# refresh-bio/LZ-ANI

Measured on AMD Instinct MI355X. Metric: genome-pairs/sec + achieved HBM GB/s, 10k×40kbp all2all at 1/2/4/8 GPUs, higher is better.
Workload: dtype u32 (2-bit packed symbols, 64-bit lane masks; f64 only in the anchor/seed arbitration)

## Files before the change

### lz-ani_amd/csrc/lzani_core.h

```cpp
#pragma once
#include <stdint.h>
#include <type_traits>

#if defined(__HIPCC__)
#include <hip/hip_runtime.h>
#define LZ_HD __host__ __device__ __forceinline__
#else
#define LZ_HD inline
#endif

#if defined(__HIP_DEVICE_COMPILE__)
extern __device__ int g_guard_trip;
#define LZ_GUARD_TRIP(code) (g_guard_trip = (code))
#else
#define LZ_GUARD_TRIP(code) ((void)(code))
#endif

namespace lzani {

typedef uint64_t u64;
typedef uint32_t u32;

struct Params {
    int mal, msl, mrd, mqd, reg, aw, am, ar;
};

struct TextView {
    const u64* t2;
    const u64* nm;
    int len;
    int L, rc0;
    bool nfree;
};

enum { NO_RC = 0x40000000 };
LZ_HD TextView ref_view(const u64* t2, const u64* nm, int L, int mrd, bool nfree)
{ return TextView{t2, nm, 2 * L + 3 * mrd, L, L + 2 * mrd, nfree}; }
LZ_HD TextView qry_view(const u64* t2, const u64* nm, int L, int mrd, bool nfree)
{ return TextView{t2, nm, L + mrd, L, NO_RC, nfree}; }

LZ_HD bool pos_valid(const TextView& t, int p)
{
    const u32 a = (u32)p, b = (u32)(p - t.rc0);
    return (a < b ? a : b) < (u32)t.L;
}
LZ_HD int run_end(const TextView& t, int p)
{
    if (p < t.L) return (t.rc0 == t.L) ? t.rc0 + t.L : t.L;
    return (p >= t.rc0 && p < t.rc0 + t.L) ? t.rc0 + t.L : p;
}

struct IndexView {
    const u32* dirz;
    const u32* ent;
    int kb;
    int dirbits;
    int posbits;
    u32 tagmask;
    const u32* bk;
    const u32* tw;
};
enum : u32 { BK_EMPTY = 0xFFFFFFFFu, BK_OVERFLOW = 0xFFFFFFFEu, TW_OVERFLOW = 0x808080FFu };
enum { IDX_SORT_MAX = 32 };

LZ_HD u64 lowmask(int n) { return n >= 64 ? ~0ULL : (n <= 0 ? 0ULL : ((1ULL << n) - 1ULL)); }

LZ_HD int popc64(u64 x)
{
#if defined(__HIP_DEVICE_COMPILE__)
    return __popcll(x);
#else
    return __builtin_popcountll(x);
#endif
}
LZ_HD int ctz64(u64 x)
{
#if defined(__HIP_DEVICE_COMPILE__)
    return __ffsll((unsigned long long)x) - 1;
#else
    return __builtin_ctzll(x);
#endif
}
LZ_HD int clz64(u64 x)
{
#if defined(__HIP_DEVICE_COMPILE__)
    return __clzll((long long)x);
#else
    return __builtin_clzll(x);
#endif
}
LZ_HD u64 brev64(u64 x)
{
#if defined(__HIP_DEVICE_COMPILE__)
    return __brevll(x);
#else
    u64 r = 0;
    for (int k = 0; k < 64; ++k) r |= ((x >> k) & 1ULL) << (63 - k);
    return r;
#endif
}
LZ_HD int imin(int a, int b) { return a < b ? a : b; }
LZ_HD int imax(int a, int b) { return a > b ? a : b; }
LZ_HD int iabs(int a) { return a < 0 ? -a : a; }

LZ_HD u64 win2(const u64* t2, int p)
{
    const u32 w = (u32)p >> 5;
    const int s = (p & 31) * 2;
    u64 lo = t2[w];
    if (s == 0) return lo;
    return (lo >> s) | (t2[w + 1] << (64 - s));
}
LZ_HD u64 winN(const u64* nm, int p)
{
    const u32 w = (u32)p >> 6;
    const int s = p & 63;
    u64 lo = nm[w];
    if (s == 0) return lo;
    return (lo >> s) | (nm[w + 1] << (64 - s));
}
typedef u32 __attribute__((may_alias)) u32a;
LZ_HD int sym_at(const TextView& t, int p)
{
    return (int)((reinterpret_cast<const u32a*>(t.t2)[(u32)p >> 4] >> ((p & 15) * 2)) & 3u);
}
LZ_HD int isN_at(const TextView& t, int p) { return (int)((t.nm[(u32)p >> 6] >> (p & 63)) & 1ULL); }

LZ_HD int sym_match(const TextView& R, int rp, const TextView& Q, int qp)
{
    if (R.nfree && Q.nfree) {
        const bool vr = pos_valid(R, rp), vq = pos_valid(Q, qp);
        const int a = sym_at(R, vr ? rp : 0), b = sym_at(Q, vq ? qp : 0);
        return (int)(vr & vq & (a == b));
    }
    if (rp < 0 || rp >= R.len || qp < 0 || qp >= Q.len) return 0;
    if (isN_at(R, rp) | isN_at(Q, qp)) return 0;
    return sym_at(R, rp) == sym_at(Q, qp);
}

LZ_HD int equal_len(const TextView& R, int rp, const TextView& Q, int qp, int start)
{
    if (R.nfree && Q.nfree) {
        int bound = imin(run_end(R, rp) - rp, run_end(Q, qp) - qp);
        int n = start;
        while (n < bound) {
            u64 x = win2(R.t2, rp + n) ^ win2(Q.t2, qp + n);
            u64 d = (x | (x >> 1)) & 0x5555555555555555ULL;
            if (d) { n += ctz64(d) >> 1; break; }
            n += 32;
        }
        n = imin(n, bound);
        return n > start ? n : start;
    }
    int bound = imin(R.len - rp, Q.len - qp);
    int n = start;
    int guard = 0;
    while (n < bound) {
        if (++guard > (1 << 26)) { LZ_GUARD_TRIP(1); break; }
        u64 x = win2(R.t2, rp + n) ^ win2(Q.t2, qp + n);
        u64 d = (x | (x >> 1)) & 0x5555555555555555ULL;
        u32 nn = (u32)(winN(R.nm, rp + n) | winN(Q.nm, qp + n));
        int fd = d ? (ctz64(d) >> 1) : 32;
        int fn = nn ? ctz64((u64)nn) : 32;
        int f = imin(fd, fn);
        if (f < 32) { n += f; return n < bound ? n : (bound > start ? bound : start); }
        n += 32;
    }
    return n < bound ? n : (bound > start ? bound : start);
}

LZ_HD bool kmer_at(const TextView& t, int p, int k, u64& key)
{
    if (p < 0 || p + k > t.len) return false;
    if (winN(t.nm, p) & lowmask(k)) return false;
    key = win2(t.t2, p) & lowmask(2 * k);
    if (k >= 32 && (key & 2)) return false;
    return true;
}

LZ_HD u64 mix_key(u64 key, int kb)
{
    if (kb <= 32) {
        u32 m = kb >= 32 ? 0xFFFFFFFFu : ((1u << kb) - 1u);
        u32 x = (u32)key;
        x = (x * 0x9E3779B1u) & m;
        x ^= x >> ((kb + 1) >> 1);
        x = (x * 0x85EBCA6Bu) & m;
        x ^= x >> ((kb + 1) >> 1);
        x = (x * 0xC2B2AE35u) & m;
        return x;
    }
    u64 m = lowmask(kb);
    u64 x = key;
    x = (x * 0x9E3779B97F4A7C15ULL) & m;
    x ^= x >> ((kb + 1) >> 1);
    x = (x * 0xD6E8FEB86659FD93ULL) & m;
    x ^= x >> ((kb + 1) >> 1);
    x = (x * 0xC2B2AE3D27D4EB4FULL) & m;
    return x;
}
LZ_HD u32 kml_from_syms(u32 syms, int mal)
{
    return (u32)mix_key((u64)(syms & (u32)lowmask(2 * mal)), 2 * mal);
}
LZ_HD bool kmer_valid_n(const TextView& t, int p, int k, u64 nwin)
{
    return p >= 0 && p + k <= t.len && !(nwin & lowmask(k));
}
LZ_HD bool kmer_valid_nfree_head(int L, int mrd, int p, int k)
{
    return p + k <= (mrd == 0 ? 2 * L : L);
}
LZ_HD void key_slot(const IndexView& I, u64 key, u32& bucket, u32& tag)
{
    u64 h = mix_key(key, I.kb);
    int tb = I.kb - I.dirbits;
    bucket = (u32)(h >> tb);
    tag = (u32)(h & lowmask(tb)) & I.tagmask;
}

LZ_HD void anchor_lookup(const Params& P, const TextView& R, const TextView& Q, const IndexView& I,
                         u64 h, int qp, int& ap, int& al)
{
    ap = 0; al = 0;
    int tb = I.kb - I.dirbits;
    u32 b = (u32)(h >> tb);
    u32 tag = (u32)(h & lowmask(tb)) & I.tagmask;
    u32 s = I.dirz[b], e = I.dirz[b + 1];
    u32 pm = (u32)lowmask(I.posbits);
    if (e - s > (u32)R.len || e < s) { LZ_GUARD_TRIP(2); return; }
    for (u32 j = s; j < e; ++j) {
        u32 en = I.ent[j];
        if ((en >> I.posbits) != tag) continue;
        int p = (int)(en & pm);
        int m = equal_len(R, p, Q, qp, 0);
        if (m >= P.mal && (m > al || (m == al && p < ap))) { al = m; ap = p; }
    }
}

LZ_HD void best_anchor(const Params& P, const TextView& R, const TextView& Q, const IndexView& I,
                       int qp, int& ap, int& al)
{
    ap = 0; al = 0;
    u64 key;
    if (!kmer_at(Q, qp, P.mal, key)) return;
    anchor_lookup(P, R, Q, I, mix_key(key, I.kb), qp, ap, al);
}

LZ_HD void seed_consider(int p, int m, int ref_pred, int& sp, int& sl)
{
    if (m >= sl) {
        if (m == sl) { if (iabs(p - ref_pred) < iabs(sp - ref_pred)) sp = p; }
        else { sl = m; sp = p; }
    }
}

LZ_HD double pow_not_chance(int len, u32 e)
{
    if (len >= 27) return 1.0;
    double base = 1.0 - __builtin_ldexp(1.0, -2 * len);
    double r = 1.0;
    while (e) {
        if (e & 1u) r *= base;
        base *= base;
        e >>= 1;
    }
    return r;
}

LZ_HD void arbitrate(const Params& P, int T, int lit, int ap, int al, int& sp, int& sl)
{
    if (!ap) return;
    if (!sp) { sp = ap; sl = al; return; }
    if (sp == ap && sl == al) return;
    u32 ea = (u32)(int)(2 * ((u64)T + 1 - (u64)(int64_t)al));
    u32 ec = (u32)(lit + P.mrd + 1 - sl);
    double anchor_prob = pow_not_chance(al, ea);
    double close_prob = pow_not_chance(sl, ec);
    if (anchor_prob > close_prob) { sp = ap; sl = al; }
}

LZ_HD void seed_search_window(const Params& P, const TextView& R, const TextView& Q,
                              int qp, int r_end, int lit, int& sp, int& sl)
{
    sp = 0; sl = 0;
    u64 qk;
    if (!kmer_at(Q, qp, P.msl, qk)) return;
    int ref_pred = r_end + lit;
    int hi = imin(ref_pred + P.mrd, R.len - P.msl + 1);
    const int step = 33 - P.msl;
    const u64 km = lowmask(2 * P.msl), nk = lowmask(P.msl);
    for (int p0 = r_end; p0 < hi; p0 += step) {
        u64 w2 = win2(R.t2, p0), wn = winN(R.nm, p0);
        int cnt = imin(step, hi - p0);
        for (int o = 0; o < cnt; ++o) {
            if (((w2 >> (2 * o)) & km) != qk || ((wn >> o) & nk)) continue;
            seed_consider(p0 + o, equal_len(R, p0 + o, Q, qp, P.msl), ref_pred, sp, sl);
        }
    }
}

LZ_HD void eval_step(const Params& P, const TextView& R, const TextView& Q, const IndexView& I,
                     int qp, bool trk, int r_end, int lit, int& bp, int& bl)
{
    int ap, al;
    best_anchor(P, R, Q, I, qp, ap, al);
    if (!trk) { bp = ap; bl = al; return; }
    int sp, sl;
    seed_search_window(P, R, Q, qp, r_end, lit, sp, sl);
    arbitrate(P, R.len, lit, ap, al, sp, sl);
    bp = sp; bl = sl;
}

struct Regions {
    int cl, clit, nl;
    int tm, tl, tc;
    int reg;
    LZ_HD void init(int r) { cl = clit = nl = tm = tl = tc = 0; reg = r; }
    LZ_HD void finalize()
    {
        if (cl && cl + clit >= reg) { tm += cl; tl += clit; ++tc; }
        cl = clit = nl = 0;
    }
    LZ_HD void discard() { cl = clit = nl = 0; }
    LZ_HD void seg(u64 M, int n)
    {
        if (M) {
            int hi = 63 - clz64(M);
            int c = popc64(M);
            cl += c;
            clit += nl + (hi + 1 - c);
            nl = n - 1 - hi;
        } else nl += n;
    }
    LZ_HD void seg_match_run(int n) { if (n > 0) { cl += n; clit += nl; nl = 0; } }
};

struct RegionCoords {
    int ref_start, ref_end, seq_start, seq_end, nm, nmm, buf;
    bool fresh;
    LZ_HD void clear() { ref_start = ref_end = seq_start = seq_end = -1; nm = nmm = buf = 0; fresh = true; }
    LZ_HD int length() const { return seq_end - seq_start; }
    LZ_HD void touch(int dp, int off, int len)
    {
        if (seq_start < 0 || dp < seq_start) seq_start = dp;
        if (seq_end < 0 || dp + len > seq_end) seq_end = dp + len;
        if (ref_start < 0 || off < ref_start) ref_start = off;
        if (ref_end < 0 || off + len > ref_end) ref_end = off + len;
    }
    LZ_HD void match(int dp, int off, int len)
    {
        if (fresh) { clear(); fresh = false; }
        else { ref_end += buf; seq_end += buf; nmm += buf; }
        buf = 0;
        touch(dp, off, len);
        nm += len;
    }
    LZ_HD void lit(int len) { buf += len; }
};

struct ExtMasks { u64 brk, qual; };

LZ_HD void ext_lane(u64 prevB, u64 B, int j, int n, int aw, int am, int ar, bool& brk, bool& qual)
{
    u64 W = (B << (63 - j)) | ((prevB >> 1) >> j);
    int a = ar < 1 ? 1 : ar;
    bool in = j < n;
    brk = in && popc64(W >> (64 - aw)) > am;
    qual = in && (W >> (64 - a)) == 0;
}

LZ_HD u64 compress_even(u64 x)
{
    x &= 0x5555555555555555ULL;
    x = (x | (x >> 1)) & 0x3333333333333333ULL;
    x = (x | (x >> 2)) & 0x0F0F0F0F0F0F0F0FULL;
    x = (x | (x >> 4)) & 0x00FF00FF00FF00FFULL;
    x = (x | (x >> 8)) & 0x0000FFFF0000FFFFULL;
    x = (x | (x >> 16)) & 0x00000000FFFFFFFFULL;
    return x;
}
LZ_HD u64 bits_below(int n) { return lowmask(n < 0 ? 0 : n); }
LZ_HD u64 bits_range(int a, int b) { return bits_below(b) & ~bits_below(a); }
LZ_HD u64 valid_bits(const TextView& t, int p0)
{
    u64 v = bits_range(-p0, t.L - p0);
    if (t.rc0 != NO_RC) v |= bits_range(t.rc0 - p0, t.rc0 + t.L - p0);
    return v;
}
LZ_HD u64 win2f(const u64* t2, int p)
{
    const u32 w = (u32)p >> 5;
    const int s = (p & 31) * 2;
    return (t2[w] >> s) | ((t2[w + 1] << 1) << (63 - s));
}
LZ_HD u64 winNf(const u64* nm, int p)
{
    const u32 w = (u32)p >> 6;
    const int s = p & 63;
    return (nm[w] >> s) | ((nm[w + 1] << 1) << (63 - s));
}
LZ_HD u32 lane_mism32(const TextView& R, const TextView& Q, int q0, int r0)
{
    const u64 x = win2f(R.t2, r0) ^ win2f(Q.t2, q0);
    const u32 mm = (u32)compress_even(x | (x >> 1));
    u32 valid;
    if (R.nfree && Q.nfree) valid = (u32)(valid_bits(R, r0) & valid_bits(Q, q0));
    else valid = (u32)(~(winNf(R.nm, r0) | winNf(Q.nm, q0)) & bits_below(R.len - r0) & bits_below(Q.len - q0));
    return mm | ~valid;
}
LZ_HD u32 win16f(const u64* t2, int p)
{
    const u32* t32 = reinterpret_cast<const u32*>(t2);
    const u32 w = (u32)p >> 4;
    const u32 s = ((u32)p & 15u) * 2u;
    const u32 d0 = t32[w], d1 = t32[w + 1];
#if defined(__HIP_DEVICE_COMPILE__)
    return __builtin_amdgcn_alignbit(d1, d0, s);
#else
    return (u32)((((u64)d1 << 32) | d0) >> s);
#endif
}
LZ_HD u32 compress_even16(u32 x)
{
    x &= 0x55555555u;
    x = (x | (x >> 1)) & 0x33333333u;
    x = (x | (x >> 2)) & 0x0F0F0F0Fu;
    x = (x | (x >> 4)) & 0x00FF00FFu;
    x = (x | (x >> 8)) & 0x0000FFFFu;
    return x;
}
LZ_HD int clamp16(int n) { return imax(0, imin(n, 16)); }
LZ_HD u32 bits_range16(int a, int b)
{
    const int l = clamp16(a), h = imax(clamp16(b), l);
    return (1u << h) - (1u << l);
}
LZ_HD u32 valid_bits16(const TextView& t, int p0)
{
    u32 v = bits_range16(-p0, t.L - p0);
    if (t.rc0 != NO_RC) v |= bits_range16(t.rc0 - p0, t.rc0 + t.L - p0);
    return v;
}
LZ_HD u32 lane_mism16(const TextView& R, const TextView& Q, int q0, int r0)
{
    const u32 x = win16f(R.t2, r0) ^ win16f(Q.t2, q0);
    const u32 mm = compress_even16(x | (x >> 1));
    u32 valid;
    if (R.nfree && Q.nfree) valid = valid_bits16(R, r0) & valid_bits16(Q, q0);
    else valid = (u32)(~(winNf(R.nm, r0) | winNf(Q.nm, q0)) & bits_below(R.len - r0) & bits_below(Q.len - q0)) & 0xFFFFu;
    return mm | ~valid;
}
LZ_HD u32 brev32(u32 x)
{
#if defined(__HIP_DEVICE_COMPILE__)
    return __brev(x);
#else
    u32 r = 0;
    for (int k = 0; k < 32; ++k) r |= ((x >> k) & 1u) << (31 - k);
    return r;
#endif
}
LZ_HD int popc32(u32 x) { return popc64((u64)x); }

enum : u32 { EXT_REC_NONE = 0x3FFFFFFFu, EXT_REC_FWDK = 0x20000000u, EXT_REC_BRKB = 0x40000000u, EXT_REC_NULLF = 0x80000000u };
LZ_HD u32 ext_rec_none(int aw) { return aw <= 15 ? 0x00007FFFu : (u32)EXT_REC_NONE; }
LZ_HD u32 ext_qual32(u32 B, int ar)
{
    const int a = ar < 1 ? 1 : ar;
    const u32 Z = ~B;
    u32 acc = Z;
    for (int k = 1; k < a && k < 32; ++k) acc &= (Z << k) | (u32)lowmask(k);
    return acc;
}
LZ_HD u32 ext_record_bwd(const Params& P, u32 Bb)
{
    const u32 wm = (u32)lowmask(P.aw);
    const u32 qb = ext_qual32(Bb, P.ar) & wm;
    if (popc32(Bb & wm) <= P.am) return qb;
    if (P.aw > 15) return qb | EXT_REC_BRKB;
    u32 x = Bb & wm;
    for (int k = 0; k < P.am; ++k) x &= x - 1u;
    const u32 q = qb & (u32)lowmask((int)__builtin_ctz(x) + 1);
    const int b = q ? 32 - (int)__builtin_clz(q) : 0;
    return (u32)b | ((u32)(b - popc32(Bb & (u32)lowmask(b))) << 4) | EXT_REC_BRKB;
}
LZ_HD u32 ext_record_fwd(const Params& P, u32 Bf)
{
    const u32 wm = (u32)lowmask(P.aw);
    if (popc32(Bf & wm) <= P.am) return 0u;
    u32 x = Bf & wm;
    for (int k = 0; k < P.am; ++k) x &= x - 1u;
    const u32 qf = ext_qual32(Bf, P.ar) & (u32)lowmask((int)__builtin_ctz(x) + 1);
    if (qf == 0) return EXT_REC_NULLF | (P.aw <= 15 ? (u32)EXT_REC_FWDK : 0u);
    if (P.aw > 15) return 0u;
    const int e = 32 - (int)__builtin_clz(qf);
    return EXT_REC_FWDK | ((u32)e << 24) | ((u32)popc32(Bf & (u32)lowmask(e)) << 20);
}
LZ_HD u32 null_ext_record(const Params& P, const TextView& R, const TextView& Q, int qp, int pos, int al, bool narrow = true)
{
    if (P.aw > 30) return EXT_REC_NONE;
    u32 rec = ext_rec_none(P.aw);
    if (qp >= 32 && pos >= 32)
        rec = ext_record_bwd(P, (narrow && P.aw <= 15) ? (brev32(lane_mism16(R, Q, qp - 16, pos - 16)) >> 16) | 0xFFFF0000u
                                                       : brev32(lane_mism32(R, Q, qp - 32, pos - 32)));
    const int fq = qp + al, fr = pos + al;
    if (imin(Q.len - fq, R.len - fr) >= P.aw)
        rec |= ext_record_fwd(P, (narrow && P.aw <= 15) ? lane_mism16(R, Q, fq, fr) : lane_mism32(R, Q, fq, fr));
    return rec;
}

struct TextWords5 { u32 m, a, b, c, d; };
LZ_HD u32 funnel32(u32 hi, u32 lo, u32 s)
{
// ... 554 lines not shown
```

### lz-ani_amd/csrc/lzani_kernels_index.h

```cpp
#pragma once
#include "lzani_block.h"

namespace lzani {

__global__ void k_kmers(GenomeTab G, u32* __restrict__ kmL, u32* __restrict__ kmS, int mal, int msl, int mrd, int Tmax)
{
    u32 g = blockIdx.y;
    int p = blockIdx.x * blockDim.x + threadIdx.x;
    int T = ref_text_len(G.L[g], mrd);
    if (p >= Tmax || p >= T) return;
    u64 o = G.nmoff[g];
    TextView R = ref_view(G.t2 + 2 * o, G.nm + o, G.L[g], mrd, false);
    u64 key;
    u32 a = KM_INVALID, b = KM_INVALID;
    if (kmer_at(R, p, mal, key)) a = kml_from_syms((u32)key, mal);
    if (kmer_at(R, p, msl, key)) {
        b = (u32)key;
        if (msl == 8 || msl == 9) {
            u32 h = (b * 0x9E3779B1u) >> 18;
            h = h == 0x3FFFu ? 0x3FFEu : h;
            b |= h << (2 * msl);
        }
    }
    kmL[64 * o + p] = a;
    kmS[64 * o + p] = b;
}

__global__ void __launch_bounds__(256) k_join_keys(GenomeTab G, const u64* __restrict__ koff, unsigned long long* __restrict__ keys,
                                                   u32* __restrict__ valid_cnt, int shift_g, int posbits, int Lmax, u32 g_base)
{
    enum { PER_THREAD = 16 };
    __shared__ u32 s_cnt;
    const u32 g = blockIdx.y;
    const int L = G.L[g];
    if (threadIdx.x == 0) s_cnt = 0;
    __syncthreads();
    const u32* km = G.kmL + 64 * G.nmoff[g];
    unsigned long long* out = keys + koff[g];
    u32 mine = 0;
    for (int k = 0; k < PER_THREAD; ++k) {
        const int p = (blockIdx.x * PER_THREAD + k) * 256 + threadIdx.x;
        if (p >= L) break;
        const u32 h = km[p];
        const bool ok = h != KM_INVALID;
        out[p] = ok ? ((unsigned long long)(g_base + g) << shift_g) | ((unsigned long long)h << posbits) | (unsigned long long)p : ~0ULL;
        mine += ok;
    }
    for (int d = 32; d >= 1; d >>= 1) mine += __shfl_xor(mine, d);
    if ((threadIdx.x & 63) == 0 && mine) atomicAdd(&s_cnt, mine);
    __syncthreads();
    if (threadIdx.x == 0 && s_cnt) atomicAdd(&valid_cnt[g], s_cnt);
    (void)Lmax;
}

__global__ void k_pack(const uint8_t* __restrict__ codes, const u64* __restrict__ codeoff,
                       u64* __restrict__ t2, u64* __restrict__ nm, const u64* __restrict__ nmoff,
                       const int* __restrict__ Ls, int* __restrict__ hasN, int mrd, u32 n)
{
    u32 g = blockIdx.y;
    if (g >= n) return;
    int L = Ls[g];
    int T = ref_text_len(L, mrd);
    size_t nblk = text_wordsN(T);
    size_t blk = (size_t)blockIdx.x * blockDim.x + threadIdx.x;
    if (blk >= nblk) return;
    const uint8_t* c = codes + codeoff[g];
    u64 w0 = 0, w1 = 0, nw = 0;
    int rc0 = L + 2 * mrd;
    for (int j = 0; j < 64; ++j) {
        long p = (long)blk * 64 + j;
        int s = 4;
        if (p < L) { int v = c[p]; s = v < 4 ? v : 4; if (v >= 4) hasN[g] = 1; }
        else if (p >= rc0 && p < rc0 + L) { int v = c[L - 1 - (p - rc0)]; s = v < 4 ? 3 - v : 4; }
        if (s < 4) {
            if (j < 32) w0 |= (u64)s << (2 * j);
            else w1 |= (u64)s << (2 * (j - 32));
        } else nw |= 1ULL << j;
    }
    size_t o = nmoff[g] + blk;
    nm[o] = nw;
    t2[2 * o] = w0;
    t2[2 * o + 1] = w1;
}

struct IdxArgs {
    GenomeTab G;
    const u32* ref_ids;
    u32* dirz;
    u32* ent;
    u64 dir_stride, ent_stride;
    int mal, mrd;
    IndexGeom geo;
    const u32* todo;
};

__device__ __forceinline__ bool idx_slot_key(const IdxArgs& a, u32 slot, int p, u32& bucket, u32& entry)
{
    u32 g = a.ref_ids[slot];
    int T = ref_text_len(a.G.L[g], a.mrd);
    if (p + a.mal > T) return false;
    u64 o = a.G.nmoff[g];
    u64 h;
    if (a.G.kmL) {
        u32 v = a.G.kmL[64 * o + p];
        if (v == KM_INVALID) return false;
        h = (u64)v;
    } else {
        TextView R = ref_view(a.G.t2 + 2 * o, a.G.nm + o, a.G.L[g], a.mrd, false);
        u64 key;
        if (!kmer_at(R, p, a.mal, key)) return false;
        h = mix_key(key, a.geo.kb);
    }
    int tb = a.geo.kb - a.geo.dirbits;
    bucket = (u32)(h >> tb);
    u32 tag = (u32)(h & lowmask(tb)) & a.geo.tagmask;
    entry = (tag << a.geo.posbits) | (u32)p;
    return true;
}

__global__ void __launch_bounds__(256) k_idx_keys(IdxArgs a, unsigned long long* __restrict__ keys, u32* __restrict__ cnt,
                                                  int Tmax, int shift_slot)
{
    enum { PER_THREAD = 16 };
    __shared__ u32 s_cnt;
    const u32 slot = blockIdx.y;
    const u32 g = a.ref_ids[slot];
    const int T = ref_text_len(a.G.L[g], a.mrd);
    if (threadIdx.x == 0) s_cnt = 0;
    __syncthreads();
    const u32* km = a.G.kmL + 64 * a.G.nmoff[g];
    unsigned long long* out = keys + (u64)slot * (u64)Tmax;
    u32 mine = 0;
    for (int k = 0; k < PER_THREAD; ++k) {
        const int p = (blockIdx.x * PER_THREAD + k) * 256 + threadIdx.x;
        if (p >= Tmax) break;
        const u32 h = p < T ? km[p] : KM_INVALID;
        const bool ok = h != KM_INVALID;
        out[p] = ok ? ((unsigned long long)h << a.geo.posbits) | (unsigned long long)p : ~0ULL;
        mine += ok;
    }
    (void)shift_slot;
    block_sum(mine, &s_cnt);
    if (threadIdx.x == 0 && s_cnt) atomicAdd(&cnt[slot], s_cnt);
}

__global__ void k_idx_base(const u32* __restrict__ cnt, u64* __restrict__ base, u32 rows, u32 group, u64 Tmax)
{
    for (u32 s = blockIdx.x * blockDim.x + threadIdx.x; s < rows; s += gridDim.x * blockDim.x) {
        const u32 g0 = s / group * group;
        u64 at = (u64)g0 * Tmax;
        for (u32 t = g0; t < s; ++t) at += cnt[t];
        base[s] = at;
    }
}

__global__ void __launch_bounds__(256) k_idx_from_sorted(IdxArgs a, const unsigned long long* __restrict__ sorted,
                                                         const u32* __restrict__ cnt, const u64* __restrict__ base,
                                                         u32* __restrict__ bk, u32* __restrict__ tw, u64 bk_stride, u64 tw_stride)
{
    const u32 slot = blockIdx.y;
    const u32 n = cnt[slot], nb = 1u << a.geo.dirbits;
    const int tb = a.geo.kb - a.geo.dirbits, posbits = a.geo.posbits;
    const u32 hmask = (u32)lowmask(a.geo.kb), pmask = (u32)lowmask(posbits), tagm = (u32)lowmask(tb) & a.geo.tagmask;
    u32* dirz = a.dirz + slot * a.dir_stride;
    u32* ent = a.ent + slot * a.ent_stride;
    uint4* bks = bk ? reinterpret_cast<uint4*>(bk + slot * bk_stride) : nullptr;
    u32* tws = tw ? tw + slot * tw_stride : nullptr;
    const uint4 empty4 = {BK_EMPTY, BK_EMPTY, BK_EMPTY, BK_EMPTY};
    if (n == 0) {
        for (u32 b = blockIdx.x * blockDim.x + threadIdx.x; b <= nb; b += gridDim.x * blockDim.x) {
            dirz[b] = 0;
            if (b < nb) { if (bks) bks[b] = empty4; if (tws) tws[b] = 0; }
        }
        return;
    }
    const unsigned long long* S = sorted + base[slot];
    for (u32 k = blockIdx.x * blockDim.x + threadIdx.x; k < n; k += gridDim.x * blockDim.x) {
        const unsigned long long e = S[k];
        const u32 h = ((u32)(e >> posbits)) & hmask, b = h >> tb;
        const u32 en = ((h & tagm) << posbits) | ((u32)e & pmask);
        ent[k] = en;
        const long long pb = k ? (long long)((((u32)(S[k - 1] >> posbits)) & hmask) >> tb) : -1;
        if ((long long)b != pb) {
            for (long long bb = pb + 1; bb <= (long long)b; ++bb) dirz[bb] = k;
            for (long long bb = pb + 1; bb < (long long)b; ++bb) { if (bks) bks[bb] = empty4; if (tws) tws[bb] = 0; }
            if (bks) {
                u32 o[4] = {en, BK_EMPTY, BK_EMPTY, BK_EMPTY};
                u32 w = 0x80u | (en >> posbits);
                u32 m = 1;
                for (; m < 5 && k + m < n; ++m) {
                    const unsigned long long e2 = S[k + m];
                    const u32 h2 = ((u32)(e2 >> posbits)) & hmask;
                    if ((h2 >> tb) != b) break;
                    if (m < 4) { o[m] = ((h2 & tagm) << posbits) | ((u32)e2 & pmask); w |= (0x80u | (o[m] >> posbits)) << (8 * m); }
                }
                if (m > 4) { o[3] = BK_OVERFLOW; w = TW_OVERFLOW; }
                bks[b] = uint4{o[0], o[1], o[2], o[3]};
                if (tws) tws[b] = w;
            }
        }
        if (k == n - 1) {
            for (long long bb = (long long)b + 1; bb <= (long long)nb; ++bb) dirz[bb] = n;
            for (long long bb = (long long)b + 1; bb < (long long)nb; ++bb) { if (bks) bks[bb] = empty4; if (tws) tws[bb] = 0; }
        }
    }
}

__global__ void k_idx_filter(IdxArgs a, u32* __restrict__ fl, u64 fl_stride, u32 fmask, int Tmax)
{
    const u32 slot = blockIdx.y;
    const u32 g = a.ref_ids[slot];
    const int T = ref_text_len(a.G.L[g], a.mrd);
    const u64 o = a.G.nmoff[g];
    for (int p = blockIdx.x * blockDim.x + threadIdx.x; p + a.mal <= T && p < Tmax; p += gridDim.x * blockDim.x) {
        const u32 v = a.G.kmL[64 * o + p];
        if (v != KM_INVALID) atomicOr(&fl[slot * fl_stride + ((v & fmask) >> 5)], 1u << (v & 31));
    }
}

__global__ void k_idx_count(IdxArgs a, int Tmax)
{
    u32 slot = blockIdx.y;
    if (a.todo && !a.todo[slot]) return;
    for (int p = blockIdx.x * blockDim.x + threadIdx.x; p < Tmax; p += gridDim.x * blockDim.x) {
        u32 b, e;
        if (idx_slot_key(a, slot, p, b, e)) atomicAdd(&a.dirz[slot * a.dir_stride + 1 + b], 1u);
    }
}

__global__ void k_idx_zero(u32* dirz, u64 dir_stride, u32 nb, const u32* todo)
{
    u32 slot = blockIdx.y;
    if (!todo[slot]) return;
    for (u32 b = blockIdx.x * blockDim.x + threadIdx.x; b <= nb; b += gridDim.x * blockDim.x) dirz[slot * dir_stride + b] = 0;
}

__global__ void __launch_bounds__(1024) k_idx_scan(u32* dirz, u64 dir_stride, u32 nb, const u32* todo)
{
    __shared__ u32 wsum[16];
    __shared__ u32 carry_s;
    if (todo && !todo[blockIdx.x]) return;
    u32* cnt = dirz + (u64)blockIdx.x * dir_stride + 1;
    if (threadIdx.x == 0) carry_s = 0;
    __syncthreads();
    for (u32 base = 0; base < nb; base += 1024) {
        const u32 idx = base + threadIdx.x;
        const u32 before = block_scan_step<u32>(idx < nb ? cnt[idx] : 0, wsum, &carry_s);
        if (idx < nb) cnt[idx] = before;
    }
}

__global__ void k_idx_fill(IdxArgs a, int Tmax)
{
    u32 slot = blockIdx.y;
    if (a.todo && !a.todo[slot]) return;
    for (int p = blockIdx.x * blockDim.x + threadIdx.x; p < Tmax; p += gridDim.x * blockDim.x) {
        u32 b, e;
        if (idx_slot_key(a, slot, p, b, e)) {
            u32 at = atomicAdd(&a.dirz[slot * a.dir_stride + 1 + b], 1u);
            a.ent[slot * a.ent_stride + at] = e;
        }
    }
}

#ifndef LZANI_IDX_RANGE
#define LZANI_IDX_RANGE 16384
#define LZANI_IDX_STAGE 24576
#endif
enum { IDX_RANGE = LZANI_IDX_RANGE, IDX_STAGE = LZANI_IDX_STAGE };

__global__ void __launch_bounds__(1024) k_idx_build(IdxArgs a, u32* __restrict__ bk, u32* __restrict__ tw,
                                                    u64 bk_stride, u64 tw_stride, u32* __restrict__ status)
{
    extern __shared__ u32 lds[];
    u32* cnt = lds;
    u32* stage = lds + IDX_RANGE / 2;
    __shared__ u32 wsum[16];
    __shared__ u32 carry_s, ovf_s;
    const u32 slot = blockIdx.x, tid = threadIdx.x;
    const int lane = tid & 63, wv = tid >> 6;
    const u32 g = a.ref_ids[slot];
    const int T = ref_text_len(a.G.L[g], a.mrd);
    const u32* km = a.G.kmL + 64 * a.G.nmoff[g];
    const u32 nb = 1u << a.geo.dirbits;
    const u32 rb = nb < (u32)IDX_RANGE ? nb : (u32)IDX_RANGE, rw = rb >> 1;
    const int tb = a.geo.kb - a.geo.dirbits, posbits = a.geo.posbits;
    const u32 tagm = (u32)lowmask(tb) & a.geo.tagmask;
    u32* dirz = a.dirz + slot * a.dir_stride;
    u32* ent = a.ent + slot * a.ent_stride;
    u32* bks = bk ? bk + slot * bk_stride : nullptr;
    u32* tws = tw ? tw + slot * tw_stride : nullptr;
    enum { U = 8 };
    if (tid == 0) ovf_s = 0;
    u32 base = 0;
    for (u32 r0 = 0; r0 < nb; r0 += rb) {
        for (u32 k = tid; k < rw; k += 1024) cnt[k] = 0;
        if (tid == 0) carry_s = 0;
        __syncthreads();
        for (int p0 = (int)tid; p0 < T; p0 += U * 1024) {
            u32 v[U];
#pragma unroll
            for (int k = 0; k < U; ++k) { const int p = p0 + k * 1024; v[k] = p < T ? km[p] : KM_INVALID; }
#pragma unroll
            for (int k = 0; k < U; ++k) {
                const u32 b = (v[k] >> tb) - r0;
                if (v[k] == KM_INVALID || b >= rb) continue;
                const u32 sh = (b & 1) * 16;
                const u32 old = atomicAdd(&cnt[b >> 1], 1u << sh);
                if (((old >> sh) & 0xFFFFu) == 0xFFFFu) ovf_s = 1;
            }
        }
        __syncthreads();
        for (u32 w0 = 0; w0 < rw; w0 += 1024) {
            const u32 idx = w0 + tid;
            const u32 w = idx < rw ? cnt[idx] : 0;
            const u32 c0 = w & 0xFFFFu, c1 = w >> 16;
            const u32 v = c0 + c1;
            u32 x = v;
            for (int d = 1; d < 64; d <<= 1) {
                u32 y = __shfl_up(x, d);
// ... 114 lines not shown
```

### lz-ani_amd/csrc/lzani_kernels_pairs.h

```cpp
#pragma once

namespace lzani {

enum { SEED_BM_BITS = 14, SEED_BM_WORDS = 1 << (SEED_BM_BITS - 5), NQUEUES = 8 };
enum { AQ_CAP = 64, AQ_MAXCHUNKS = 32, AQ_LANE_CAP = 32, AQ_LDS_CAND = 128,
       SEED_PAD = 96,
       SEED_LDS_WORDS = SEED_BM_WORDS + SEED_PAD };
static_assert(2 * AQ_LDS_CAND <= SEED_BM_WORDS, "the candidate buffers of refill live in the seed bitmap");
enum : u32 { AQ_COMPLEX = 0x80000000u, AQ_LONG = 0x40000000u, AQ_POS = 0x3FFFFFFFu };
enum { AQ_NONE = 0x7FFFFFFF };

__device__ __forceinline__ u64 wballot(bool b) { return __builtin_amdgcn_ballot_w64(b); }
__device__ __forceinline__ u32 rep4(u32 b) { return __builtin_amdgcn_perm(b, b, 0u); }

#if defined(LZANI_RTC)
#define LZ_RTC_PARAMS Params{LZANI_P_MAL, LZANI_P_MSL, LZANI_P_MRD, LZANI_P_MQD, LZANI_P_REG, LZANI_P_AW, LZANI_P_AM, LZANI_P_AR}
#else
#define LZ_RTC_PARAMS Params{11, 7, 40, 40, 35, 15, 7, 3}
#endif
LZ_HD constexpr Params folded_params(int defp)
{
    return defp == 2 ? Params{15, 9, 40, 40, 60, 15, 7, 3} : defp == 9 ? LZ_RTC_PARAMS : Params{11, 7, 40, 40, 35, 15, 7, 3};
}
LZ_HD constexpr bool chain_params_ok(const Params& p)
{
    return p.mal >= 1 && p.mal <= 15 && p.msl >= 1 && p.msl <= 9 && p.mqd >= 0 && p.mqd <= 62 && p.mrd >= 1 &&
           p.mqd + p.mrd >= 64 && p.mqd + p.mrd <= 127 && p.aw >= 2 && p.aw <= 15 && p.ar <= p.aw && p.am >= 0 && p.reg >= 0 && p.reg < (1 << 20);
}
LZ_HD constexpr int chain_of(int defp, bool nfree)
{
    return defp == 1 ? (nfree ? 3 : 1) : defp == 2 ? 2 : defp == 9 ? (chain_params_ok(folded_params(9)) ? (nfree ? 10 : 9) : 0) : 0;
}
template <int CHAIN> struct ChainP {
    static constexpr Params P = folded_params(CHAIN == 2 ? 2 : CHAIN >= 9 ? 9 : 1);
    static constexpr bool NF = CHAIN == 3 || CHAIN == 10;
    enum { MAL = P.mal, MSL = P.msl, MRD = P.mrd, MQD = P.mqd, REG = P.reg, AW = P.aw, AM = P.am > 16 ? 16 : P.am, AR = P.ar < 1 ? 1 : P.ar,
           NT = MQD + 1, WIN = MQD + MRD };
};

#ifndef LZANI_STRETCH_DENSE
#define LZANI_STRETCH_DENSE 0
#endif
template <bool FAST, bool BK = false, bool JOIN = false, int CHAIN = 0, bool LFLT = false, bool SPLITW = false>
struct DevWave {
    static constexpr bool NULL_CHAIN = CHAIN != 0;
    const Params& P;
    TextView R, Q;
    IndexView I;
    int lane;
    u32* bitmap;
    const u32* rkS;
    const u32* qkL;
    const u32* qkS;
    lzani_region* reg_out;
    unsigned long long* reg_count;
    unsigned long long reg_cap, pair_e;
    int iend = 0;
    int scan_pos = 0, q_head = 0, q_cnt = 0;
    int last_src = -1;
    int stop_i = 0x7FFFFFFF;
    __device__ __forceinline__ void split_limit(int at) { stop_i = at; }
    bool split_taint = false;
    __device__ __forceinline__ void split_taint_set(bool t) { split_taint = t; }
    static __device__ __forceinline__ int uniform(int v) { return __builtin_amdgcn_readfirstlane(v); }
    enum { SPLIT_MARGIN = 256 };
    u32 a_ext = EXT_REC_NONE;
    unsigned long long* cand_bits = nullptr;
    int a_pos = AQ_NONE, a_len = 0;
    u32 a_ref = 0;
#ifdef LZANI_CHAIN_STATS
    unsigned st[8] = {0, 0, 0, 0, 0, 0, 0, 0};
    unsigned sw[8] = {0, 0, 0, 0, 0, 0, 0, 0};
    unsigned sr[4] = {0, 0, 0, 0};
    unsigned long long stc[4] = {0, 0, 0, 0}, stc_t0 = 0;
    int stc_open = -2;
#define LZ_CHAIN_SLOTS(X) \
    X(0, "chain_calls") X(1, "commits") X(2, "exit_nothing") X(3, "exit_seed") X(4, "exit_not_plain") X(5, "exit_event") \
    X(6, "events_general") X(7, "refills") \
    X(8, "cycles after exit_nothing") X(9, "cycles after round_done") X(10, "cycles after exit_event") X(11, "cycles inside the chain") \
    X(12, "not null: close") X(13, "not null: region kept or none open") X(14, "not null: no forward record") X(15, "not null: backward side") \
    X(16, "exit_seed: anchor's own step") X(17, "exit_seed: no window position") X(18, "exit_seed: several") X(19, "exit_seed: text end") \
    X(20, "exit_seed: long seed") X(21, "exit_seed: other") X(22, "event known, commit left") X(23, "-")
    template <class Acc> __device__ __forceinline__ void flush_chain_stats(Acc* g, int ln) const
    {
        for (int k = 0; k < 8; ++k) atomicAdd(&g[k], ln == 0 ? (unsigned long long)st[k] : 0ULL);
        for (int k = 0; k < 4; ++k) atomicAdd(&g[8 + k], ln == 0 ? stc[k] : 0ULL);
        for (int k = 0; k < 4; ++k) atomicAdd(&g[12 + k], ln == 0 ? (unsigned long long)sr[k] : 0ULL);
        for (int k = 0; k < 8; ++k) atomicAdd(&g[16 + k], ln == 0 ? (unsigned long long)sw[k] : 0ULL);
    }
    __device__ __forceinline__ void cycles_mark(int code)
    {
        unsigned long long t;
        asm volatile("s_memtime %0\n\ts_waitcnt lgkmcnt(0)" : "=s"(t) :: "memory");
        if (stc_open == 0) stc[0] += t - stc_t0; else if (stc_open == 1) stc[1] += t - stc_t0; else if (stc_open == 2) stc[2] += t - stc_t0; else if (stc_open == 3) stc[3] += t - stc_t0;
        stc_open = code < 0 ? 3 : code;
        stc_t0 = t;
    }
#endif
#ifdef LZANI_PATH_STATS
    unsigned ps[24] = {0};
    unsigned pw[12] = {0};
#define LZ_PATH_SLOTS(X) \
    X(0, "find_event calls") X(1, "fe: seed straight from the chain's round") X(2, "fe: common call, plain candidate") X(3, "fe: light rounds") \
    X(4, "fe: light round hit") X(5, "fe: light round without a hit") X(6, "fe: merge loop hit") X(7, "fe: jump to a plain candidate") \
    X(8, "stretch calls") X(9, "stretch: not applicable") X(10, "stretch: no seed step") X(11, "stretch: anchor before the seed") \
    X(12, "stretch: seed event") X(13, "stretch: ... with the masks") X(14, "stretch: sum of seed steps") \
    X(15, "refills") X(16, "chain: nothing") X(17, "chain: round done") X(18, "chain: event found") X(19, "chain: seed event known") \
    X(20, "events") X(21, "close events") X(22, "extension chunks") X(23, "stretch chain: events committed") \
    X(24, "-") X(25, "text end") X(26, "no seed step") X(27, "several window positions") X(28, "seed bounds") X(29, "match of 64+") \
    X(30, "anchor before the seed") X(31, "tag in two slots / overflow") X(32, "anchor elsewhere") X(33, "extension runs on") \
    X(34, "-") X(35, "-")
    template <class Acc> __device__ __forceinline__ void flush_path_stats(Acc* g, int ln) const
    {
        for (int k = 0; k < 24; ++k) atomicAdd(&g[k], ln == 0 ? (unsigned long long)ps[k] : 0ULL);
        for (int k = 0; k < 12; ++k) atomicAdd(&g[24 + k], ln == 0 ? (unsigned long long)pw[k] : 0ULL);
    }
#define LZ_PS(k) (ps[k] += 1)
#define LZ_PSN(k, n) (ps[k] += (unsigned)(n))
#else
#define LZ_PS(k) ((void)0)
#define LZ_PSN(k, n) ((void)0)
#endif
#ifdef LZANI_PHASE_TIME
    unsigned long long pt_chain = 0, pt_refill = 0;
    static __device__ __forceinline__ unsigned long long pt_now()
    {
        unsigned long long t;
        asm volatile("s_memtime %0\n\ts_waitcnt lgkmcnt(0)" : "=s"(t) :: "memory");
        return t;
    }
#endif
    bool refill_only = false;
    int restart_at = -1;
    bool round_no_seed = false;
    bool pre_round = false;
    u64 pre_seed = 0;
    u32 pre_rk0 = KM_INVALID, pre_rk1 = KM_INVALID, pre_qk = KM_INVALID;
    const u32* flt = nullptr;
    u32 fmask = 31;
    __device__ __forceinline__ void emit_region(const RegionCoords& c) const
    {
        unsigned long long old, saved;
        const unsigned long long one = 1ULL;
        asm volatile("s_mov_b64 %[sv], exec\n\t"
                     "s_mov_b64 exec, 1\n\t"
                     "global_atomic_add_x2 %[old], %[addr], %[one], off sc0\n\t"
                     "s_waitcnt vmcnt(0)\n\t"
                     "s_mov_b64 exec, %[sv]"
                     : [old] "=&v"(old), [sv] "=&s"(saved)
                     : [addr] "v"(reg_count), [one] "v"(one)
                     : "memory");
        const u32 lo = __builtin_amdgcn_readfirstlane((u32)old), hi = __builtin_amdgcn_readfirstlane((u32)(old >> 32));
        const unsigned long long slot = ((unsigned long long)hi << 32) | lo;
        if (slot < reg_cap) {
            lzani_region* o = reg_out + slot;
            o->pair = pair_e;
            o->ref_start = c.ref_start; o->ref_end = c.ref_end; o->seq_start = c.seq_start; o->seq_end = c.seq_end;
            o->num_matches = c.nm; o->num_mismatches = c.nmm;
        }
    }
#ifdef LZANI_STAMPS
    mutable unsigned long long t0;
    mutable unsigned long long acc[8];
    mutable int cur;
    __device__ __forceinline__ void stamp(int k) const
    {
        unsigned long long t;
        asm volatile("s_memtime %0\n\ts_waitcnt lgkmcnt(0)" : "=s"(t) :: "memory");
        acc[cur] += t - t0; cur = k; t0 = t;
    }
#else
    __device__ __forceinline__ void stamp(int) const {}
#endif

    struct SymReq { u32 wr, wq; int sr, sq; bool ok; };
    __device__ __forceinline__ SymReq sym_request(int rp, int qp) const
    {
        const bool vr = pos_valid(R, rp), vq = pos_valid(Q, qp);
        const int a = vr ? rp : 0, b = vq ? qp : 0;
        SymReq x;
        x.wr = reinterpret_cast<const u32a*>(R.t2)[(u32)a >> 4];
        x.wq = reinterpret_cast<const u32a*>(Q.t2)[(u32)b >> 4];
        x.sr = (a & 15) * 2; x.sq = (b & 15) * 2; x.ok = vr & vq;
        return x;
    }
    static __device__ __forceinline__ bool sym_differs(const SymReq& x)
    {
        return !(x.ok & ((((x.wr >> x.sr) ^ (x.wq >> x.sq)) & 3u) == 0));
    }
    __device__ __forceinline__ bool lane_mismatch(int rp, int qp) const
    {
        if (R.nfree && Q.nfree) {
            SymReq x = sym_request(rp, qp);
            asm volatile("" : "+v"(x.wr), "+v"(x.wq));
            return sym_differs(x);
        }
        return !sym_match(R, rp, Q, qp);
    }
    __device__ __forceinline__ u64 mism_fwd(int q0, int r0, int n) const
    {
        return wballot((lane < n) & lane_mismatch(r0 + lane, q0 + lane));
    }
    __device__ __forceinline__ u64 mism_bwd(int q0, int r0, int n) const
    {
        return wballot((lane < n) & lane_mismatch(r0 - 1 - lane, q0 - 1 - lane));
    }
    __device__ __forceinline__ void mism2(int qa, int ra, int da, int na, int qb, int rb, int db, int nb, u64& A, u64& B) const
    {
        const int rpa = ra + da * lane, qpa = qa + da * lane, rpb = rb + db * lane, qpb = qb + db * lane;
        bool ma, mb;
        if (R.nfree && Q.nfree) {
            SymReq x = sym_request(rpa, qpa), y = sym_request(rpb, qpb);
            asm volatile("" : "+v"(x.wr), "+v"(x.wq), "+v"(y.wr), "+v"(y.wq));
            ma = sym_differs(x); mb = sym_differs(y);
        } else {
            ma = !sym_match(R, rpa, Q, qpa);
            mb = !sym_match(R, rpb, Q, qpb);
        }
        A = wballot((lane < na) & ma);
        B = wballot((lane < nb) & mb);
    }
    static constexpr bool HAS_MISM3 = true;
    __device__ __forceinline__ void mism3(int qa, int ra, int na, int qb, int rb, int nb, int qc, int rc, int nc, u64& A, u64& B, u64& C) const
    {
        bool ma, mb, mc;
        if (R.nfree && Q.nfree) {
            SymReq x = sym_request(ra + lane, qa + lane), y = sym_request(rb + lane, qb + lane), z = sym_request(rc + lane, qc + lane);
            asm volatile("" : "+v"(x.wr), "+v"(x.wq), "+v"(y.wr), "+v"(y.wq), "+v"(z.wr), "+v"(z.wq));
            ma = sym_differs(x); mb = sym_differs(y); mc = sym_differs(z);
        } else {
            ma = !sym_match(R, ra + lane, Q, qa + lane);
            mb = !sym_match(R, rb + lane, Q, qb + lane);
            mc = !sym_match(R, rc + lane, Q, qc + lane);
        }
        A = wballot((lane < na) & ma);
        B = wballot((lane < nb) & mb);
        C = wballot((lane < nc) & mc);
    }
    __device__ __forceinline__ u32 bm_hash(u32 k) const
    {
        return P.msl <= 7 ? k : P.msl <= 9 ? k >> (2 * P.msl) : (k * 0x9E3779B1u) >> (32 - SEED_BM_BITS);
    }
    __device__ __forceinline__ bool seed_prefilter(u32 rk0, u32 rk1, u32 qk) const
    {
        const u32 scratch = (u32)lane;
        const u32 b0 = bm_hash(rk0), b1 = bm_hash(rk1), bq = bm_hash(qk);
        const bool v0 = rk0 != KM_INVALID, v1 = rk1 != KM_INVALID, vq = qk != KM_INVALID;
        const u32 w0 = v0 ? b0 >> 5 : scratch, w1 = v1 ? b1 >> 5 : scratch, wq = vq ? bq >> 5 : scratch;
        atomicOr(&bitmap[w0], v0 ? 1u << (b0 & 31) : 0u);
        atomicOr(&bitmap[w1], v1 ? 1u << (b1 & 31) : 0u);
        __builtin_amdgcn_fence(__ATOMIC_ACQ_REL, "wavefront");
        __builtin_amdgcn_wave_barrier();
        const bool hit = vq & ((bitmap[wq] >> (bq & 31)) & 1u);
        __builtin_amdgcn_fence(__ATOMIC_ACQ_REL, "wavefront");
        __builtin_amdgcn_wave_barrier();
        bitmap[w0] = 0;
        bitmap[w1] = 0;
        return hit;
    }
    __device__ __forceinline__ void seed_candidates(u32 qkl, int lim, u32 rk0, u32 rk1, u64& d0, u64& d1) const
    {
        d0 = wballot(rk0 == qkl) & lowmask(lim);
        d1 = wballot(rk1 == qkl) & lowmask(lim - 64);
    }

    __device__ __forceinline__ u64 bcast64(u64 v, int l) const
    {
        const u32 lo = (u32)__builtin_amdgcn_readlane((int)(u32)v, l), hi = (u32)__builtin_amdgcn_readlane((int)(u32)(v >> 32), l);
        return ((u64)hi << 32) | lo;
    }
    __device__ __forceinline__ int wave_equal_len(int rp, int qp, int start) const
    {
        const int bound = imin(R.len - rp, Q.len - qp);
        int n = start;
        while (n < bound) {
            u64 B = mism_fwd(qp + n, rp + n, imin(64, bound - n));
            if (B) { n += ctz64(B); break; }
            n += 64;
        }
        n = imin(n, bound);
        return n > start ? n : start;
    }

    __device__ __forceinline__ bool find_event_generic(int i, int n, bool trk, int r_end, int lit,
                                                       int& ev_lane, int& bpos, int& blen) const
    {
        int bp = 0, bl = 0;
        if (lane < n)
            eval_step(P, R, Q, I, i + lane, trk && (lit + lane <= P.mqd), r_end, lit + lane, bp, bl);
        u64 hit = wballot(lane < n && bl >= P.msl);
        if (!hit) { ev_lane = n; return false; }
        ev_lane = ctz64(hit);
        bpos = __builtin_amdgcn_readlane(bp, ev_lane);
        blen = __builtin_amdgcn_readlane(bl, ev_lane);
        return true;
    }

    __device__ __forceinline__ void walk_bucket(u32 b, u32 tag, int qp, int& ap, int& al) const
    {
        const u32 pm = (u32)lowmask(I.posbits);
        u32 s = I.dirz[b], e = I.dirz[b + 1];
        if (e - s > (u32)R.len || e < s) { LZ_GUARD_TRIP(2); e = s; }
        for (u32 j = s; j < e; ++j) {
            const u32 x = (u32)__builtin_amdgcn_readfirstlane((int)I.ent[j]);
            if ((x >> I.posbits) != tag) continue;
            const int p = (int)(x & pm);
            const int m = wave_equal_len(p, qp, 0);
            if (m >= P.mal && (m > al || (m == al && p < ap))) { al = m; ap = p; }
        }
    }

    __device__ __forceinline__ void anchor_by_wave(u32 hql, int qp, int& ap, int& al) const
    {
        const int tb = I.kb - I.dirbits;
        const u32 pm = (u32)lowmask(I.posbits), tag = hql & I.tagmask;
        typedef u32 u32x4 __attribute__((ext_vector_type(4)));
        u32x4 bq;
        const u64 baddr = (u64)(I.bk + 4 * (u64)(hql >> tb));
        const u64 bsgpr = ((u64)(u32)__builtin_amdgcn_readfirstlane((int)(u32)(baddr >> 32)) << 32) |
                          (u32)__builtin_amdgcn_readfirstlane((int)(u32)baddr);
        asm volatile("s_load_dwordx4 %0, %1, 0x0\n\ts_waitcnt lgkmcnt(0)" : "=s"(bq) : "s"(bsgpr) : "memory");
        const u32 en[4] = {bq.x, bq.y, bq.z, bq.w};
        if (__builtin_expect(en[3] == BK_OVERFLOW, 0)) {
            walk_bucket(hql >> tb, tag, qp, ap, al);
        } else {
#pragma unroll
            for (int k = 0; k < 4; ++k) {
                if ((en[k] >> I.posbits) != tag) continue;
                const int p = (int)(en[k] & pm);
                const int m = wave_equal_len(p, qp, 0);
                if (m >= P.mal && m > al) { al = m; ap = p; }
            }
        }
    }

    __device__ __forceinline__ bool find_event_round(int i, int n, bool trk, int r_end, int lit,
                                                     int& ev_lane, int& bpos, int& blen) const
    {
        n = imin(n, 64);
        ev_lane = n;
        const int nt = trk ? imin(n, P.mqd - lit + 1) : 0;
        const int W = nt > 0 ? imin(lit + nt - 1 + P.mrd, R.len - P.msl + 1 - r_end) : 0;
        const int tb = I.kb - I.dirbits;
        if (__builtin_expect(!FAST || W > 128 || (!BK && I.tagmask != (u32)lowmask(tb)), 0))
            return find_event_generic(i, n, trk, r_end, lit, ev_lane, bpos, blen);

        u32 hq = qkL[(u32)(i + lane)], rk0 = KM_INVALID, rk1 = KM_INVALID, qk = KM_INVALID;
        hq = lane < n ? hq : KM_INVALID;
        if (W > 0) {
            const int w0 = imin(lane, W - 1), w1 = imin(lane + 64, W - 1);
            qk = qkS[(u32)(i + lane)];
            rk0 = rkS[(u32)(r_end + w0)];
            rk1 = rkS[(u32)(r_end + w1)];
            qk = lane < nt ? qk : KM_INVALID;
            rk0 = lane < W ? rk0 : KM_INVALID;
            rk1 = lane + 64 < W ? rk1 : KM_INVALID;
        }
        u32 ac = 0;
        uint4 bkv = {BK_EMPTY, BK_EMPTY, BK_EMPTY, BK_EMPTY};
        bool viadir = !BK && I.bk == nullptr;
        if constexpr (BK) {
            const bool valid = hq != KM_INVALID;
            const u32 w = I.tw[valid ? hq >> tb : 0u];
            const u32 x = w ^ rep4(0x80u | (hq & I.tagmask));
            ac = (u32)(valid & ((((x - 0x01010101u) & ~x & 0x80808080u) != 0) | (w == TW_OVERFLOW)));
        } else if (hq != KM_INVALID) {
            const u32 b = hq >> tb, tag = hq & I.tagmask;
            if (I.bk) {
                bkv = reinterpret_cast<const uint4*>(I.bk)[b];
                viadir = bkv.w == BK_OVERFLOW;
                if (!viadir)
                    ac = (u32)((bkv.x >> I.posbits) == tag) + (u32)((bkv.y >> I.posbits) == tag) +
                         (u32)((bkv.z >> I.posbits) == tag) + (u32)((bkv.w >> I.posbits) == tag);
            }
            if (viadir) {
                u32 s = I.dirz[b], e = I.dirz[b + 1];
                if (e - s > (u32)R.len || e < s) { LZ_GUARD_TRIP(2); e = s; }
                for (u32 j = s; j < e; ++j) ac += (I.ent[j] >> I.posbits) == tag;
            }
        }
        stamp(2);
        bool shit = false;
        if (W > 0) shit = seed_prefilter(rk0, rk1, qk);
        u64 todo = wballot(ac != 0 || shit);
        stamp(7);
        const u32 pm = (u32)lowmask(I.posbits);
        while (todo) {
            const int l = ctz64(todo);
            todo &= todo - 1;
            const int qp = i + l;
            int ap = 0, al = 0;
            const u32 cnt = __builtin_amdgcn_readlane(ac, l);
            if (BK && cnt) {
                anchor_by_wave((u32)__builtin_amdgcn_readlane((int)hq, l), qp, ap, al);
            } else if (cnt) {
                const u32 hql = (u32)__builtin_amdgcn_readlane((int)hq, l), tag = hql & I.tagmask;
                if (__builtin_amdgcn_readlane((int)viadir, l)) {
                    walk_bucket(hql >> tb, tag, qp, ap, al);
                } else {
                    const u32 en[4] = {(u32)__builtin_amdgcn_readlane((int)bkv.x, l), (u32)__builtin_amdgcn_readlane((int)bkv.y, l),
                                       (u32)__builtin_amdgcn_readlane((int)bkv.z, l), (u32)__builtin_amdgcn_readlane((int)bkv.w, l)};
#pragma unroll
                    for (int k = 0; k < 4; ++k) {
                        if ((en[k] >> I.posbits) != tag) continue;
                        const int p = (int)(en[k] & pm);
                        const int m = wave_equal_len(p, qp, 0);
                        if (m >= P.mal && m > al) { al = m; ap = p; }
                    }
                }
            }
            int bp = ap, bl = al;
            if (l < nt) {
                int sp = 0, sl = 0;
                const int ref_pred = r_end + lit + l;
                u64 d0 = 0, d1 = 0;
                const u32 qkl = (u32)__builtin_amdgcn_readlane((int)qk, l);
                if (qkl != KM_INVALID) seed_candidates(qkl, lit + l + P.mrd, rk0, rk1, d0, d1);
                while (d0 | d1) {
                    int idx;
                    if (d0) { idx = ctz64(d0); d0 &= d0 - 1; }
                    else { idx = 64 + ctz64(d1); d1 &= d1 - 1; }
                    seed_consider(r_end + idx, wave_equal_len(r_end + idx, qp, P.msl), ref_pred, sp, sl);
                }
                arbitrate(P, R.len, lit + l, ap, al, sp, sl);
                bp = sp; bl = sl;
            }
            if (__builtin_expect(bl >= P.msl, 1)) { ev_lane = l; bpos = bp; blen = bl; return true; }
        }
        return false;
    }
    static __device__ __forceinline__ int wave_incl_scan(int v)
    {
        v += __builtin_amdgcn_update_dpp(0, v, 0x111, 0xF, 0xF, false);
        v += __builtin_amdgcn_update_dpp(0, v, 0x112, 0xF, 0xF, false);
        v += __builtin_amdgcn_update_dpp(0, v, 0x114, 0xF, 0xF, false);
        v += __builtin_amdgcn_update_dpp(0, v, 0x118, 0xF, 0xF, false);
        v += __builtin_amdgcn_update_dpp(0, v, 0x142, 0xA, 0xF, false);
        v += __builtin_amdgcn_update_dpp(0, v, 0x143, 0xC, 0xF, false);
        return v;
    }
    __device__ __forceinline__ void lds_order() const
    {
        __builtin_amdgcn_fence(__ATOMIC_ACQ_REL, "wavefront");
        __builtin_amdgcn_wave_barrier();
    }
    __device__ __forceinline__ void refill(int from)
    {
#ifdef LZANI_CHAIN_STATS
        st[7] += 1;
#endif
#ifdef LZANI_STAMPS
        const int stamp_sv = cur;
        stamp(2);
#endif
#ifdef LZANI_PHASE_TIME
        const unsigned long long pt_r0 = pt_now();
#endif
        LZ_PS(15);
        u32* const cq = bitmap;
        const int tb = I.kb - I.dirbits;
        scan_pos = imax(scan_pos, from);
        int ncand = 0;
        if (JOIN && scan_pos < iend) {
            const u32 w0 = (u32)scan_pos >> 6;
            const int p_lo = (int)((w0 + (u32)lane) << 6), p_hi = p_lo + 4096;
            unsigned long long x = cand_bits[p_lo < iend ? w0 + (u32)lane : w0];
            unsigned long long x2 = cand_bits[p_hi < iend ? w0 + 64u + (u32)lane : w0];
            x &= ~lowmask(scan_pos - p_lo) & lowmask(iend - p_lo);
            x2 = p_hi < iend ? x2 & lowmask(iend - p_hi) : 0ULL;
            int blocks = 1, base = 0;
            for (;;) {
                const int cnt = popc64(x);
                const int incl = wave_incl_scan(cnt);
                int at = base + incl - cnt;
                ncand = base + __builtin_amdgcn_readlane(incl, 63);
                int p0 = blocks == 1 ? p_lo : p_hi;
                while (wballot((x != 0) & (at <= AQ_CAP)) != 0) {
                    const bool has = (x != 0) & (at <= AQ_CAP);
                    const u32 lo = (u32)x, hi = (u32)(x >> 32);
                    const int b = lo ? (int)__builtin_ctz(lo) : 32 + (int)__builtin_ctz(hi | 0x80000000u);
                    cq[has ? at : AQ_LDS_CAND - 1] = (u32)(p0 + b);
                    x &= x - 1;
                    at += 1;
                }
                if (blocks == 2 || ncand >= AQ_CAP || (int)((w0 + 64u) << 6) >= iend) break;
                blocks = 2; base = ncand; x = x2;
            }
            scan_pos = imin((int)((w0 + 64u * (u32)blocks) << 6), iend);
        }
        for (int turn = 0; !JOIN && turn < AQ_MAXCHUNKS / 4 && scan_pos < iend && ncand < AQ_CAP; ++turn) {
            u32 hq[4], w[4];
            bool valid[4];
#pragma unroll
            for (int c = 0; c < 4; ++c) hq[c] = qkL[(u32)imin(scan_pos + 64 * c + lane, iend + 63)];
            asm volatile("" : "+v"(hq[0]), "+v"(hq[1]), "+v"(hq[2]), "+v"(hq[3]));
#pragma unroll
            for (int c = 0; c < 4; ++c) {
                valid[c] = (scan_pos + 64 * c + lane < iend) & (hq[c] != KM_INVALID);
                if (LFLT) valid[c] &= (bool)((flt[(hq[c] & fmask) >> 5] >> (hq[c] & 31u)) & 1u);
                w[c] = I.tw[valid[c] ? hq[c] >> tb : 0u];
            }
            asm volatile("" : "+v"(w[0]), "+v"(w[1]), "+v"(w[2]), "+v"(w[3]));
#ifdef LZANI_PROBE2X
            {
                u32 d[4];
#pragma unroll
                for (int c = 0; c < 4; ++c) d[c] = I.tw[valid[c] ? ((hq[c] * 0x9E3779B1u) >> (32 - I.dirbits)) : 0u];
                asm volatile("" :: "v"(d[0]), "v"(d[1]), "v"(d[2]), "v"(d[3]));
            }
#endif
#pragma unroll
            for (int c = 0; c < 4; ++c) {
                if (scan_pos >= iend || ncand >= AQ_CAP) break;
                const int p = scan_pos + lane;
                const u32 x = w[c] ^ rep4(0x80u | (hq[c] & I.tagmask));
                const u32 z = (x - 0x01010101u) & ~x & 0x80808080u;
                const bool ovf = w[c] == TW_OVERFLOW;
                const bool cnd = valid[c] & ((z != 0) | ovf);
                const u64 bal = wballot(cnd);
                {
                    const int at = cnd ? ncand + (int)__builtin_amdgcn_mbcnt_hi((u32)(bal >> 32), __builtin_amdgcn_mbcnt_lo((u32)bal, 0u)) : AQ_LDS_CAND - 1;
                    const bool cplx = ovf | ((z & (z - 1)) != 0);
                    cq[at] = (u32)p;
                    cq[AQ_LDS_CAND + at] = cplx ? (u32)AQ_COMPLEX : 4u * (hq[c] >> tb) + ((u32)__builtin_ctz(z | 0x80000000u) >> 3);
                    ncand += popc64(bal);
                }
                scan_pos = imin(scan_pos + 64, iend);
            }
        }
        lds_order();
        q_head = 0;
        q_cnt = imin(ncand, AQ_CAP);
        if (__builtin_expect(ncand > AQ_CAP, 0))
            scan_pos = (int)__builtin_amdgcn_readfirstlane(cq[AQ_CAP]);
        const bool live = lane < q_cnt;
        const int qp = live ? (int)cq[lane] : 0;
        u32 slot = live ? cq[AQ_LDS_CAND + lane] : (u32)AQ_COMPLEX;
        lds_order();
#pragma unroll
        for (int k = 0; k < 2 * AQ_LDS_CAND; k += 64) cq[k + lane] = 0;
        lds_order();
        bool simple, dead = false;
        int pos;
        const u32* const pq = reinterpret_cast<const u32*>(Q.t2) + ((u32)qp >> 4);
        const u32 sq = ((u32)qp & 15u) * 2u;
        const u32 q0 = pq[0], q1 = pq[1];
        const u32 qlo = __builtin_amdgcn_alignbit(q1, q0, sq);
        u64 qn = 0;
        bool qvalid = true;
        if (JOIN) {
            const TextView QR = ref_view(Q.t2, Q.nm, Q.L, P.mrd, Q.nfree);
            if (R.nfree && Q.nfree) qvalid = kmer_valid_nfree_head(Q.L, P.mrd, qp, P.mal);
            else { qn = winN(Q.nm, qp); qvalid = kmer_valid_n(QR, qp, P.mal, qn); }
        }
        if (JOIN) {
            const u32 hq = kml_from_syms(qlo, P.mal);
            const bool ok = live & qvalid;
            const uint4 bkv = reinterpret_cast<const uint4*>(I.bk)[ok ? hq >> tb : 0u];
            const u32 tag = hq & I.tagmask;
            const bool m0 = (bkv.x >> I.posbits) == tag, m1 = (bkv.y >> I.posbits) == tag, m2 = (bkv.z >> I.posbits) == tag,
                       m3 = (bkv.w >> I.posbits) == tag;
            const int cnt = (int)m0 + (int)m1 + (int)m2 + (int)m3;
            const bool ovf = bkv.w == BK_OVERFLOW;
            simple = ok & !ovf & (cnt == 1);
            dead = !ok | (!ovf & (cnt == 0));
            const u32 en = m0 ? bkv.x : m1 ? bkv.y : m2 ? bkv.z : bkv.w;
            pos = simple ? (int)(en & (u32)lowmask(I.posbits)) : 0;
        } else {
            simple = !(slot & AQ_COMPLEX);
            pos = simple ? (int)(I.bk[simple ? slot : 0u] & (u32)lowmask(I.posbits)) : 0;
        }
        int qp2 = qp;
        asm volatile("" : "+v"(qp2));
        ResolveDiff df = resolve_diff(text_words5(R.t2, pos), pos, text_words5(Q.t2, qp2), qp);
        asm volatile("" : "+v"(df.back), "+v"(df.d0), "+v"(df.d1), "+v"(df.d2));
        int same = diff_same32(df);
        int bound;
        if (R.nfree && Q.nfree) bound = imin(run_end(R, pos) - pos, run_end(Q, qp) - qp);
        else {
            bound = imin(R.len - pos, Q.len - qp);
            if (!JOIN) qn = winN(Q.nm, qp);
            const u32 nn = (u32)(winN(R.nm, pos) | qn);
            same = imin(same, nn ? (int)__builtin_ctz(nn) : AQ_LANE_CAP);
        }
        const bool lng = (same == AQ_LANE_CAP) & (bound > AQ_LANE_CAP);
        a_pos = live ? qp : (int)AQ_NONE;
        a_ref = simple ? ((u32)pos | (lng ? (u32)AQ_LONG : 0u)) : (u32)AQ_COMPLEX;
        const int al0 = simple ? imin(same, bound) : 0;
        const bool plain = simple & !lng & (al0 >= P.mal) & (al0 >= P.msl) & (pos != 0);
        a_len = plain ? al0 : -1 - al0;
        a_ext = ext_rec_none(P.aw);
        if (R.nfree && Q.nfree && P.aw <= 15) a_ext = (simple & !lng) ? null_ext_record_diff(P, R, Q, df, qp, pos, al0) : a_ext;
        else if (simple & !lng) a_ext = null_ext_record(P, R, Q, qp, pos, al0);
        const bool kept = live & !dead & !(simple & !lng & (al0 < P.mal));
        const u64 keep = wballot(kept);
        if (keep != lowmask(q_cnt)) {
            const int to = 4 * (kept ? (int)__builtin_amdgcn_mbcnt_hi((u32)(keep >> 32), __builtin_amdgcn_mbcnt_lo((u32)keep, 0u)) : 63);
            q_cnt = popc64(keep);
            const int mp = __builtin_amdgcn_ds_permute(to, a_pos), ml = __builtin_amdgcn_ds_permute(to, a_len);
            const int mr = __builtin_amdgcn_ds_permute(to, (int)a_ref), mx = __builtin_amdgcn_ds_permute(to, (int)a_ext);
            a_pos = lane < q_cnt ? mp : (int)AQ_NONE;
            a_len = ml; a_ref = (u32)mr; a_ext = (u32)mx;
        }
        if constexpr (CHAIN) chain_classes();
#ifdef LZANI_PHASE_TIME
        asm volatile("s_waitcnt vmcnt(0) lgkmcnt(0)" ::: "memory");
        pt_refill += pt_now() - pt_r0;
#endif
#ifdef LZANI_STAMPS
        stamp(stamp_sv);
#endif
    }
    __device__ __forceinline__ int len_at(int k) const
    {
        const int v = __builtin_amdgcn_readlane(a_len, k);
        return CHAIN ? (int)(signed char)(v & 0xFF) : v;
    }
    __device__ __forceinline__ void chain_classes()
    {
        typedef ChainP<CHAIN> CP;
        enum { MQD = CP::MQD, MRD = CP::MRD, MSL = CP::MSL, REG = CP::REG, AW = CP::AW, NT = CP::NT, WIN = CP::WIN };
        constexpr bool nf = CP::NF;
        int ilim = imin(imin(scan_pos, iend) - NT, nf ? Q.L - MSL + 1 - 64 : iend);
        const int rlim = R.len - MSL + 1 - WIN;
        if constexpr (SPLITW) ilim = imin(ilim, stop_i - (int)SPLIT_MARGIN);
        const int len = a_len;
        const bool plain = len > 0;
        const u32 rec = a_ext;
        const int pos = (int)(a_ref & AQ_POS);
        const int t2 = len + (int)((rec >> 24) & 31u);
        const int end = a_pos + t2, rend = pos + t2;
        const bool both = (rec & (EXT_REC_FWDK | EXT_REC_BRKB)) == (u32)(EXT_REC_FWDK | EXT_REC_BRKB);
        const bool cap = plain & both & (imin(a_pos, pos) >= AW);
        const bool rwin = !nf | (rend + WIN <= R.L - MSL + 1) | ((rend >= R.rc0) & (rend + WIN <= R.rc0 + R.L - MSL + 1));
        const bool pred = plain & both & (end <= ilim) & (rend <= rlim) & rwin & (t2 + (int)(rec & 15u) < REG);
        const int mine = (int)((u32)pos | (cap ? 0x80000000u : 0u));
        int succ = 64, s_pos = 0, s_u = 0;
#pragma unroll
        for (int d = 3; d >= 1; --d) {
            const int l = lane + d;
            const int p = __builtin_amdgcn_ds_bpermute(4 * l, a_pos), u = __builtin_amdgcn_ds_bpermute(4 * l, mine);
            const bool ok = (l < 64) & (p >= end);
            succ = ok ? l : succ; s_pos = ok ? p : s_pos; s_u = ok ? u : s_u;
        }
        const int gap = s_pos - end;
        const bool distant = (gap > MQD) | (iabs((s_u & 0x7FFFFFFF) - (rend + gap)) > MRD);
        bool go = pred & (succ < q_cnt) & (s_u < 0) & distant;
        if constexpr (SPLITW) go &= s_pos <= ilim;
        a_len = (len & 0xFF) | (succ << 8) | (go ? 0x8000 : 0) | (cap ? 0x10000 : 0) | ((t2 & 0xFF) << 17);
    }
    __device__ __forceinline__ bool ext_record(u32& x) const
    {
        if (last_src < 0) return false;
        x = (u32)__builtin_amdgcn_readlane((int)a_ext, last_src);
        return true;
    }
    __device__ __forceinline__ void note_src(int k, int ap, int al, int bpos, int blen)
    {
        const u32 ref = (u32)__builtin_amdgcn_readlane((int)a_ref, k);
        last_src = (!(ref & (AQ_COMPLEX | AQ_LONG)) && al >= P.mal && bpos == ap && blen == al) ? k : -1;
    }
    __device__ __forceinline__ void drop_before(int pos)
    {
        const u64 m = wballot((lane >= q_head) & (a_pos >= pos));
        q_head = m ? ctz64(m) : 64;
    }
    __device__ __forceinline__ void anchor_of(int k, int qp, int& ap, int& al) const
    {
        const u32 ref = (u32)__builtin_amdgcn_readlane((int)a_ref, k);
        ap = 0; al = 0;
        if (__builtin_expect((ref & AQ_COMPLEX) != 0, 0)) {
            anchor_by_wave((u32)__builtin_amdgcn_readfirstlane((int)qkL[(u32)qp]), qp, ap, al);
            return;
        }
        ap = (int)(ref & AQ_POS);
        al = len_at(k);
        al = al < 0 ? -1 - al : al;
        if (__builtin_expect((ref & AQ_LONG) != 0, 0)) al = wave_equal_len(ap, qp, AQ_LANE_CAP);
        if (__builtin_expect(al < P.mal, 0)) { ap = 0; al = 0; }
    }

    __device__ __forceinline__ u64 detect_steps(int i, int nt, int from = 0) const
    {
        if (JOIN) {
            const int sh = i & 63;
            const unsigned long long wd = cand_bits[((u32)i >> 6) + (u32)imin(lane, 1)];
            return ((bcast64(wd, 0) >> sh) | ((bcast64(wd, 1) << 1) << (63 - sh))) & lowmask(nt) & ~lowmask(from);
        }
        const int tb = I.kb - I.dirbits;
        const u32 hq = qkL[(u32)(i + lane)];
        const bool valid = (lane >= from) & (lane < nt) & (hq != KM_INVALID);
        const u32 w = I.tw[valid ? hq >> tb : 0u];
        const u32 x = w ^ rep4(0x80u | (hq & I.tagmask));
        const u32 z = (x - 0x01010101u) & ~x & 0x80808080u;
        return wballot(valid & ((z != 0) | (w == TW_OVERFLOW)));
    }

    __device__ __forceinline__ u64 track_round(int i, int nt, int r_end, int lit, u32& rk0, u32& rk1, u32& qk) const
    {
        rk0 = rk1 = qk = KM_INVALID;
        const int W = imin(lit + nt - 1 + P.mrd, R.len - P.msl + 1 - r_end);
        if (W <= 0) return 0;
        const int w0 = imin(lane, W - 1), w1 = imin(lane + 64, W - 1);
#ifdef LZANI_PRIO
        __builtin_amdgcn_s_setprio(LZANI_PRIO);
#endif
        qk = qkS[(u32)(i + lane)];
        rk0 = rkS[(u32)(r_end + w0)];
        rk1 = rkS[(u32)(r_end + w1)];
#ifdef LZANI_PRIO
        asm volatile("" : "+v"(qk), "+v"(rk0), "+v"(rk1));
        __builtin_amdgcn_s_setprio(0);
#endif
        qk = lane < nt ? qk : KM_INVALID;
        rk0 = lane < W ? rk0 : KM_INVALID;
        rk1 = lane + 64 < W ? rk1 : KM_INVALID;
        return wballot(seed_prefilter(rk0, rk1, qk));
    }


    static __device__ __forceinline__ const u32* uniform_ptr(const u32* p)
    {
        const u64 a = (u64)p;
        const u32 lo = (u32)__builtin_amdgcn_readfirstlane((int)(u32)a), hi = (u32)__builtin_amdgcn_readfirstlane((int)(u32)(a >> 32));
        return (const u32*)(((u64)hi << 32) | lo);
    }
    __device__ __forceinline__ bool chain_covers(int i) const { return scan_pos >= i; }
    __device__ __forceinline__ int null_chain(int& i, int& r_end, int& prev_rs, int& prev_re, int& pre_lit, int& last_cl,
                                              int& last_clit, int& adv, int& bpos, int& blen, int open_cl, int open_clit,
                                              int& add_tm, int& add_tl, int& add_tc)
    {
        static_assert(!CHAIN || (FAST && BK), "the null chain reads the anchor queue");
        typedef ChainP<CHAIN> CP;
        enum { MQD = CP::MQD, MRD = CP::MRD, MSL = CP::MSL, REG = CP::REG, AW = CP::AW, AM = CP::AM, AR = CP::AR, NT = CP::NT, WIN = CP::WIN };
        static_assert(!CHAIN || chain_params_ok(CP::P), "the null chain is not written for these parameters");
        const int ilim_q = imin(scan_pos, iend) - NT;
        const int ilim = SPLITW ? imin(ilim_q, stop_i - (int)SPLIT_MARGIN) : ilim_q;
        const int rlim = R.len - MSL + 1 - WIN;
        const u32 ldsb = (u32)(size_t)bitmap;
        const u32 zero = 0, one = 1;
        const u32* const qks = uniform_ptr(qkS);
        const u32* const rks = uniform_ptr(rkS);
        int code, ap, rec, t0, t1, t2, kb, kc, qh = q_head;
        u64 m, seed;
#if defined(LZANI_STAMPS) || defined(LZANI_PATH_STATS)
        constexpr bool unify = true;
#else
        constexpr bool unify = SPLITW;
#endif
        int qc_u = q_cnt, ilim_u = ilim, rlim_u = rlim;
        [[maybe_unused]] const int tnt_u = SPLITW ? __builtin_amdgcn_readfirstlane((int)split_taint) : 0;
        if constexpr (unify) {
            i = __builtin_amdgcn_readfirstlane(i); r_end = __builtin_amdgcn_readfirstlane(r_end); qh = __builtin_amdgcn_readfirstlane(qh);
            prev_rs = __builtin_amdgcn_readfirstlane(prev_rs); prev_re = __builtin_amdgcn_readfirstlane(prev_re);
            pre_lit = __builtin_amdgcn_readfirstlane(pre_lit);
            qc_u = __builtin_amdgcn_readfirstlane(q_cnt); ilim_u = __builtin_amdgcn_readfirstlane(ilim); rlim_u = __builtin_amdgcn_readfirstlane(rlim);
        }
        u32 rk0, rk1, qk, a0, a1, aq, t, bq, w1, dumv, qkb, rk0b, rk1b;
#ifdef LZANI_CHAIN_STATS
        int ncnt = 0;
#define LZ_NC_COUNT "s_add_i32 %[ncnt], %[ncnt], 1\n\t"
        int why = 0;
#define LZ_NC_COUNT_OPERAND [ncnt] "+s"(ncnt), [why] "+s"(why),
#define LZ_NC_WHY(n) "s_mov_b32 %[why], " #n "\n\t"
#else
#define LZ_NC_COUNT
#define LZ_NC_COUNT_OPERAND
#define LZ_NC_WHY(n)
#endif
#if defined(LZANI_EXP) && LZANI_EXP == 4
#define LZ_NC_NOSEED "s_cmp_lg_u32 0, 0\n\t"
#else
#define LZ_NC_NOSEED
#endif
#define LZ_NC_LOADS_X(I, R, QK, K0, K1) \
            "v_add_lshl_u32 %[a0], %[lane], %[" I "], 2\n\t" \
            "v_add_lshl_u32 %[a1], %[lane], %[" R "], 2\n\t" \
            "v_add_lshl_u32 %[aq], %[w1], %[" R "], 2\n\t" \
            "global_load_dword %[" QK "], %[a0], %[qks]\n\t" \
            "global_load_dword %[" K0 "], %[a1], %[rks]\n\t" \
            "global_load_dword %[" K1 "], %[aq], %[rks]\n\t"
#define LZ_NC_LOADS_F LZ_NC_LOADS_X("i", "rend", "qk", "rk0", "rk1")
#define LZ_NC_WORD7(A, T, K) \
            "v_lshrrev_b32_e32 %[" A "], 5, %[" K "]\n\t" \
            "v_lshlrev_b32_e32 %[" T "], %[" K "], %[one]\n\t" \
            "v_min_u32_e32 %[" A "], %[dumv], %[" A "]\n\t" \
            "v_lshl_add_u32 %[" A "], %[" A "], 2, %[ldsb]\n\t"
#define LZ_NC_WORD7N(A, T, K) \
            "v_lshrrev_b32_e32 %[" A "], 5, %[" K "]\n\t" \
            "v_lshlrev_b32_e32 %[" T "], %[" K "], %[one]\n\t" \
            "v_lshl_add_u32 %[" A "], %[" A "], 2, %[ldsb]\n\t"
#define LZ_NC_WORD9(A, T, K) \
            "v_lshrrev_b32_e32 %[" A "], 23, %[" K "]\n\t" \
            "v_lshrrev_b32_e32 %[" T "], 18, %[" K "]\n\t" \
            "v_lshlrev_b32_e32 %[" T "], %[" T "], %[one]\n\t" \
            "v_lshl_add_u32 %[" A "], %[" A "], 2, %[ldsb]\n\t"
#define LZ_NC_WORD8(A, T, K)                 \
            "v_bfe_u32 %[" A "], %[" K "], %[KS5], 9\n\t" \
            "v_lshrrev_b32_e32 %[" T "], %[KS], %[" K "]\n\t" \
            "v_lshlrev_b32_e32 %[" T "], %[" T "], %[one]\n\t" \
            "v_lshl_add_u32 %[" A "], %[" A "], 2, %[ldsb]\n\t"
#define LZ_NC_ROUND_X(WORD, WAIT, QK, K0, K1) \
            WAIT "\n\t" \
            WORD("a0", "t", K0) \
            "ds_or_b32 %[a0], %[t]\n\t" \
            WORD("a1", "bq", K1) \
            "ds_or_b32 %[a1], %[bq]\n\t" \
            WORD("aq", "t", QK) \
            "ds_read_b32 %[aq], %[aq]\n\t" \
            "ds_write_b32 %[a0], %[zero]\n\t" \
            "ds_write_b32 %[a1], %[zero]\n\t" \
            "s_waitcnt lgkmcnt(2)\n\t" \
            "v_and_b32_e32 %[aq], %[aq], %[t]\n\t" \
            "v_cmp_ne_u32_e64 %[seed], 0, %[aq]\n\t"
#define LZ_NC_ROUND_F(WORD) LZ_NC_ROUND_X(WORD, "s_waitcnt vmcnt(0)", "qk", "rk0", "rk1")
#define LZ_NC_FTURN(WORDF, P, N, IC, IN, RN, CQ, C0, C1, NQ, N0, N1, SFX) \
            "Lnc_fturn" SFX "_%=:\n\t" \
            "s_bitcmp0_b32 %[" P "], 15\n\t" \
            "s_cbranch_scc1 Lnc_fnogo" SFX "_%=\n\t" \
            "s_bfe_u32 %[qh], %[" P "], 0x70008\n\t"         \
            "v_readlane_b32 %[" N "], %[alen], %[qh]\n\t"    \
            "v_readlane_b32 %[ap], %[apos], %[qh]\n\t" \
            "v_readlane_b32 %[bpos], %[aref], %[qh]\n\t" \
            "s_bfe_u32 %[t0], %[" N "], 0x80011\n\t" \
            "s_sub_i32 %[gap], %[ap], %[" IC "]\n\t" \
            "s_add_i32 %[" IN "], %[ap], %[t0]\n\t" \
            "s_add_i32 %[" RN "], %[bpos], %[t0]\n\t" \
            LZ_NC_LOADS_X(IN, RN, NQ, N0, N1) \
            LZ_NC_ROUND_X(WORDF, "s_waitcnt vmcnt(3)", CQ, C0, C1) \
            LZ_NC_SEEDS \
            "s_cbranch_scc1 Lnc_frec" SFX "_%=\n\t"          \
            "s_mov_b32 %[t2], %[qh]\n\t" \
            LZ_NC_COUNT
#define LZ_NC_FIX \
            "s_bfm_b64 %[m2], %[NT], 0\n\t" \
            "s_and_b64 %[seed], %[seed], %[m2]\n\t" \
            "v_cmp_gt_u32_e64 %[m2], %[NR1], %[lane]\n\t" \
            "v_cmp_gt_u32_e32 vcc, %[NT], %[lane]\n\t" \
            "s_nop 1\n\t" \
            "v_cndmask_b32_e64 %[rk1], -1, %[rk1], %[m2]\n\t" \
            "v_cndmask_b32_e32 %[qk], -1, %[qk], vcc\n\t" \
            "v_cmp_ne_u32_e32 vcc, -1, %[qk]\n\t"           \
            "s_and_b64 %[seed], %[seed], vcc\n\t" \
            "s_and_b64 %[m], %[m], vcc\n"
#define LZ_NC_SEEDS \
            "s_add_i32 %[t0], %[gap], 1\n\t" \
            "s_min_u32 %[t0], %[t0], %[NT]\n\t" \
            "s_bfm_b64 %[m], %[t0], 0\n\t" \
            "s_and_b64 %[m], %[m], %[seed]\n\t" LZ_NC_NOSEED
#define LZ_NC_COMMIT \
            "s_sub_i32 %[plit], %[t1], %[kb]\n\t"            \
            "s_sub_i32 %[prs], %[ap], %[kb]\n\t"             \
            "s_bfe_u32 %[t0], %[rec], 0x50018\n\t"           \
            "s_bfe_u32 %[lastlit], %[rec], 0x40014\n\t"      \
            "s_add_i32 %[t2], %[blen], %[t0]\n\t" \
            "s_sub_i32 %[lastb], %[t2], %[lastlit]\n\t"      \
            "s_add_i32 %[lastb], %[lastb], %[kc]\n\t" \
            "s_add_i32 %[lastlit], %[lastlit], %[kb]\n\t"    \
            "s_sub_i32 %[lastlit], %[lastlit], %[kc]\n\t" \
            "s_add_i32 %[i], %[ap], %[t2]\n\t" \
            "s_add_i32 %[rend], %[bpos], %[t2]\n\t" \
            "s_mov_b32 %[pre], %[i]\n\t" \
            "s_add_i32 %[qh], %[qh], 1\n\t" \
            LZ_NC_COUNT
        int gap, cls, fok;
        u64 m2;
        const u32* const rt2 = uniform_ptr(reinterpret_cast<const u32*>(R.t2));
        const u32* const qt2 = uniform_ptr(reinterpret_cast<const u32*>(Q.t2));
        const int qend = __builtin_amdgcn_readfirstlane((R.nfree && Q.nfree) ? iend : -(1 << 30));
        const int ocl_u = __builtin_amdgcn_readfirstlane(open_cl), oclit_u = __builtin_amdgcn_readfirstlane(open_clit);
#ifdef LZANI_CHAIN_PRIO
#define LZ_NC_PRIO_ON "s_setprio 2\n\t"
#define LZ_NC_PRIO_OFF "s_setprio 0\n\t"
#else
#define LZ_NC_PRIO_ON
#define LZ_NC_PRIO_OFF
#endif
#define LZ_NC_SPLITCHK \
            "v_readlane_b32 %[t0], %[apos], %[qh]\n\t" \
            "s_cmp_gt_i32 %[t0], %[ilim]\n\t" \
            "s_cbranch_scc1 Lnc_end_%=\n\t"
#define LZ_NC_SPLITGEN \
            "s_cmp_lg_u32 %[tnt], 0\n\t" \
            "s_cbranch_scc1 Lnc_chk_%=\n\t"
#define LZ_NC_SPLITIN , [tnt] "s"(tnt_u)
#define LZ_NC_ASM(WORD, WORDF) LZ_NC_ASM_X(WORD, WORDF, "", "", )
#define LZ_NC_ASM_X(WORD, WORDF, SPLCHK, SPLGEN, SPLIN) \
        asm volatile( \
            LZ_NC_PRIO_ON \
            "s_mov_b32 %[code], 0\n\t" \
            "s_mov_b32 %[lastb], 0\n\t" \
            "s_mov_b32 %[lastlit], 0\n\t" \
            "s_mov_b32 %[atm], 0\n\t" \
            "s_mov_b32 %[atl], 0\n\t" \
            "s_mov_b32 %[atc], 0\n\t" \
            "s_mov_b64 %[m2], -1\n\t"                       \
             \
             \
            "v_add_u32_e32 %[w1], 64, %[lane]\n\t" \
            "v_subrev_u32_e32 %[dumv], %[WIN], %[w1]\n\t" \
            "v_min_u32_e32 %[w1], %[w1], %[dumv]\n\t" \
            "v_add_u32_e32 %[dumv], %[wdum], %[lane]\n\t"   \
            "s_nop 3\n" \
            "Lnc_top_%=:\n\t" \
             \
            "s_cmp_ge_i32 %[qh], %[qc]\n\t" \
            "s_cbranch_scc1 Lnc_end_%=\n\t" \
            "v_readlane_b32 %[t0], %[apos], %[qh]\n\t" \
            "s_cmp_ge_i32 %[t0], %[i]\n\t" \
            "s_cbranch_scc1 Lnc_nodrop_%=\n\t" \
            "v_cmp_le_i32_e32 vcc, %[qh], %[lane]\n\t" \
            "v_cmp_le_i32_e64 %[m], %[i], %[apos]\n\t" \
            "s_and_b64 %[m], %[m], vcc\n\t" \
            "s_ff1_i32_b64 %[qh], %[m]\n\t" \
            "s_min_u32 %[qh], %[qh], 64\n\t" \
            "s_cmp_ge_i32 %[qh], %[qc]\n\t" \
            "s_cbranch_scc1 Lnc_end_%=\n" \
            "Lnc_nodrop_%=:\n\t" \
            "s_cmp_gt_i32 %[i], %[ilim]\n\t" \
            "s_cbranch_scc1 Lnc_end_%=\n\t" \
            "s_cmp_gt_i32 %[rend], %[rlim]\n\t" \
            "s_cbranch_scc1 Lnc_end_%=\n\t" \
            SPLCHK \
            LZ_NC_LOADS_F \
             \
             \
            "v_readlane_b32 %[blen], %[alen], %[qh]\n\t" \
            "v_readlane_b32 %[ap], %[apos], %[qh]\n\t" \
            "v_readlane_b32 %[bpos], %[aref], %[qh]\n\t" \
            "v_readlane_b32 %[rec], %[aext], %[qh]\n\t" \
            "s_mov_b32 %[t2], 0\n\t" \
            "s_mov_b32 %[cls], 0\n\t"                         \
            "s_bfe_u32 %[code], %[blen], 0x10010\n\t"        \
            "s_sext_i32_i8 %[blen], %[blen]\n\t"             \
            "s_sub_i32 %[gap], %[ap], %[i]\n\t" \
            "s_cmp_lt_i32 %[blen], 1\n\t" \
            "s_cbranch_scc1 Lnc_chk_%=\n\t" \
            "s_cmp_le_i32 %[gap], %[MQD]\n\t" \
            "s_cbranch_scc1 Lnc_close_%=\n" \
            "Lnc_distant_%=:\n\t" \
            "s_cmp_lt_i32 %[prs], 0\n\t" \
            "s_cbranch_scc1 Lnc_kept_%=\n\t" \
            "s_sub_i32 %[t1], %[pre], %[prs]\n\t" \
            "s_cmp_ge_i32 %[t1], %[REG]\n\t" \
            "s_cbranch_scc1 Lnc_kept_%=\n\t" \
            "s_sub_i32 %[t1], %[ap], %[prs]\n\t" \
            "s_add_i32 %[t1], %[t1], %[plit]\n"              \
            "Lnc_avail_%=:\n\t" \
             \
             \
            "s_cmp_eq_u32 %[code], 0\n\t" \
            "s_cbranch_scc1 Lnc_gen_%=\n\t" \
            "s_cmp_lt_i32 %[t1], %[AW]\n\t" \
            "s_cbranch_scc1 Lnc_gen_%=\n\t" \
            "s_and_b32 %[kb], %[rec], 15\n\t" \
            "s_bfe_u32 %[kc], %[rec], 0x40004\n\t" \
            "s_mov_b32 %[fok], 1\n\t" \
            "s_branch Lnc_ok_%=\n" \
            "Lnc_gen_%=:\n\t" \
            SPLGEN \
            "s_bitcmp0_b32 %[rec], 29\n\t"                   \
            "s_cbranch_scc1 Lnc_chk_%=\n\t" \
            "s_min_i32 %[t0], %[t1], %[ap]\n\t" \
            "s_min_i32 %[t0], %[t0], %[bpos]\n\t"            \
            "s_mov_b32 %[kb], 0\n\t"                           \
            "s_mov_b32 %[kc], 0\n\t" \
            "s_mov_b32 %[fok], 0\n\t" \
            "s_cmp_lt_i32 %[t0], 1\n\t" \
            "s_cbranch_scc1 Lnc_ok_%=\n\t" \
            "s_bitcmp1_b32 %[rec], 30\n\t" \
            "s_cbranch_scc1 Lnc_brkb_%=\n\t" \
            "s_min_i32 %[code], %[t0], %[AW]\n\t"            \
            "s_bfm_b32 %[code], %[code], 0\n\t"              \
            "s_and_b32 %[code], %[code], %[rec]\n\t" \
            "s_cbranch_scc1 Lnc_chk_%=\n\t" \
            "s_cmp_le_i32 %[t0], %[AW]\n\t" \
            "s_cbranch_scc1 Lnc_ok_%=\n\t" \
            "s_branch Lnc_chk_%=\n" \
            "Lnc_brkb_%=:\n\t"                                \
            "s_cmp_lt_i32 %[t0], %[AW]\n\t"                  \
            "s_cbranch_scc1 Lnc_chk_%=\n\t" \
            "s_and_b32 %[kb], %[rec], 15\n\t" \
            "s_bfe_u32 %[kc], %[rec], 0x40004\n\t" \
            "s_mov_b32 %[fok], 1\n"                           \
            "Lnc_ok_%=:\n\t" \
            "s_mov_b32 %[t2], 1\n" \
            "Lnc_chk_%=:\n\t" \
            LZ_NC_ROUND_F(WORD) \
            "s_mov_b32 %[code], 1\n\t" \
            LZ_NC_SEEDS \
            "s_cbranch_scc1 Lnc_sseed_%=\n"                  \
            "Lnc_noseed_%=:\n\t" \
            "s_cmp_lt_i32 %[blen], 1\n\t" \
            "s_cbranch_scc1 Lnc_npl_%=\n\t"                  \
            "s_mov_b32 %[code], 2\n\t" \
            "s_cmp_eq_u32 %[t2], 0\n\t" \
            "s_cbranch_scc1 Lnc_end_%=\n\t"                  \
            "s_cmp_eq_u32 %[cls], 0\n\t" \
            "s_cbranch_scc1 Lnc_commit_%=\n\t" \
             \
             \
             \
            "s_cmp_lg_u32 %[lastb], 0\n\t" \
            "s_cselect_b32 %[t0], %[lastb], %[ocl]\n\t" \
            "s_cselect_b32 %[t2], %[lastlit], %[oclit]\n\t" \
            "s_cmp_eq_u32 %[t0], 0\n\t" \
            "s_cbranch_scc1 Lnc_commit_%=\n\t" \
            "s_add_i32 %[t2], %[t2], %[t0]\n\t" \
            "s_cmp_lt_i32 %[t2], %[REG]\n\t" \
            "s_cbranch_scc1 Lnc_commit_%=\n\t" \
            "s_sub_i32 %[t2], %[t2], %[t0]\n\t" \
            "s_add_i32 %[atm], %[atm], %[t0]\n\t" \
            "s_add_i32 %[atl], %[atl], %[t2]\n\t" \
            "s_add_i32 %[atc], %[atc], 1\n" \
            "Lnc_commit_%=:\n\t" \
            LZ_NC_COMMIT \
            "s_mov_b32 %[code], 0\n\t" \
            "s_cmp_eq_u32 %[fok], 0\n\t" \
            "s_cbranch_scc1 Lnc_top_%=\n" \
             \
             \
             \
            "Lnc_fast_%=:\n\t" \
             \
             \
             \
             \
            "s_sub_i32 %[fok], %[prs], %[plit]\n\t" \
            "s_sub_i32 %[t2], %[qh], 1\n\t"                 \
            "v_readlane_b32 %[cls], %[alen], %[t2]\n"       \
            "Lnc_fstart_%=:\n\t" \
            LZ_NC_LOADS_F \
             \
             \
             \
             \
             \
            LZ_NC_FTURN(WORDF, "cls", "blen", "i", "t1", "kb", "qk", "rk0", "rk1", "qkb", "rk0b", "rk1b", "") \
            LZ_NC_FTURN(WORDF, "blen", "cls", "t1", "i", "rend", "qkb", "rk0b", "rk1b", "qk", "rk0", "rk1", "2") \
            "s_branch Lnc_fturn_%=\n" \
            "Lnc_fnogo2_%=:\n\t" \
            "s_mov_b32 %[i], %[t1]\n\t" \
            "s_mov_b32 %[rend], %[kb]\n\t" \
            "s_mov_b32 %[cls], %[blen]\n\t" \
            "s_branch Lnc_fnogo_%=\n" \
            "Lnc_frec2_%=:\n\t" \
            "s_mov_b32 %[i], %[t1]\n\t" \
            "s_mov_b32 %[rend], %[kb]\n\t" \
            "s_mov_b32 %[t0], %[cls]\n\t" \
            "s_mov_b32 %[cls], %[blen]\n\t" \
            "s_mov_b32 %[blen], %[t0]\n\t" \
            "s_waitcnt vmcnt(0)\n\t"                         \
            "v_mov_b32_e32 %[qk], %[qkb]\n\t" \
            "v_mov_b32_e32 %[rk0], %[rk0b]\n\t" \
            "v_mov_b32_e32 %[rk1], %[rk1b]\n\t" \
            "s_branch Lnc_frec_%=\n" \
             \
            "Lnc_fcont_%=:\n\t" \
            "s_bfe_u32 %[t0], %[blen], 0x80011\n\t" \
            "s_add_i32 %[i], %[ap], %[t0]\n\t" \
            "s_add_i32 %[rend], %[bpos], %[t0]\n\t" \
            "s_mov_b32 %[t2], %[qh]\n\t" \
            "s_mov_b32 %[cls], %[blen]\n\t" \
            LZ_NC_COUNT \
            "s_branch Lnc_fstart_%=\n" \
            "Lnc_fnogo_%=:\n\t"                             \
            "s_add_i32 %[qh], %[t2], 1\n" \
             \
            "Lnc_frec_%=:\n\t" \
            "v_readlane_b32 %[t0], %[apos], %[t2]\n\t" \
            "v_readlane_b32 %[t1], %[alen], %[t2]\n\t" \
            "v_readlane_b32 %[kc], %[aext], %[t2]\n\t" \
            "s_sext_i32_i8 %[t1], %[t1]\n\t" \
            "s_and_b32 %[kb], %[kc], 15\n\t" \
            "s_sub_i32 %[prs], %[t0], %[kb]\n\t" \
            "s_sub_i32 %[plit], %[t0], %[fok]\n\t" \
            "s_sub_i32 %[plit], %[plit], %[kb]\n\t" \
            "s_bfe_u32 %[lastlit], %[kc], 0x40014\n\t" \
            "s_bfe_u32 %[t0], %[kc], 0x50018\n\t" \
            "s_add_i32 %[t1], %[t1], %[t0]\n\t" \
            "s_sub_i32 %[lastb], %[t1], %[lastlit]\n\t" \
            "s_bfe_u32 %[t0], %[kc], 0x40004\n\t" \
            "s_add_i32 %[lastb], %[lastb], %[t0]\n\t" \
            "s_add_i32 %[lastlit], %[lastlit], %[kb]\n\t" \
            "s_sub_i32 %[lastlit], %[lastlit], %[t0]\n\t" \
            "s_mov_b32 %[pre], %[i]\n\t" \
            "s_bitcmp0_b32 %[cls], 15\n\t" \
            "s_cbranch_scc1 Lnc_top_%=\n"                    \
            "Lnc_fseed_%=:\n\t"                              \
            "s_mov_b32 %[code], 1\n\t" \
            LZ_NC_FIX \
            "s_cmp_eq_u64 %[m], 0\n\t"                       \
            "s_cbranch_scc1 Lnc_snone_%=\n" \
             \
             \
             \
             \
             \
             \
            "Lnc_seedev_%=:\n\t" \
            "s_ff1_i32_b64 %[t0], %[m]\n"                    \
            "Lnc_sdl_%=:\n\t" \
            "v_readlane_b32 %[t1], %[qk], %[t0]\n\t"         \
            "s_add_i32 %[t2], %[t0], %[MRD]\n\t"             \
            "s_sub_i32 %[kc], %[t2], 64\n\t" \
            "s_max_i32 %[kc], %[kc], 0\n\t" \
            "s_min_u32 %[kb], %[t2], 64\n\t" \
            "s_sub_i32 %[kb], 64, %[kb]\n\t"                 \
            "v_cmp_eq_u32_e32 vcc, %[t1], %[rk1]\n\t" \
            "s_bfm_b64 %[m2], %[kc], 0\n\t" \
            "s_and_b64 %[m2], %[m2], vcc\n\t" \
            "v_cmp_eq_u32_e32 vcc, %[t1], %[rk0]\n\t" \
            "s_bcnt1_i32_b64 %[kc], %[m2]\n\t" \
            "s_lshl_b64 vcc, vcc, %[kb]\n\t" \
            "s_bcnt1_i32_b64 %[t1], vcc\n\t" \
            "s_add_i32 %[t2], %[t1], %[kc]\n\t" \
            LZ_NC_WHY(2) \
            "s_cmp_eq_u32 %[t2], 0\n\t" \
            "s_cbranch_scc1 Lnc_sfalse_%=\n\t"               \
            "s_cmp_lg_u32 %[t2], 1\n\t" \
            "s_cbranch_scc1 Lnc_end_%=\n\t"                  \
            "s_ff1_i32_b64 %[t2], vcc\n\t" \
            "s_sub_i32 %[t2], %[t2], %[kb]\n\t" \
            "s_ff1_i32_b64 %[kc], %[m2]\n\t" \
            "s_add_i32 %[kc], %[kc], 64\n\t" \
            "s_cmp_lg_u32 %[t1], 0\n\t" \
            "s_cselect_b32 %[t2], %[t2], %[kc]\n\t"          \
            "s_add_i32 %[rec], %[rend], %[t2]\n\t"           \
            "s_add_i32 %[cls], %[i], %[t0]\n\t"              \
             \
             \
             \
             \
            LZ_NC_WHY(1) \
            "s_cmp_lg_u32 %[t0], %[gap]\n\t" \
            "s_cbranch_scc1 Lnc_snoq_%=\n\t" \
            "s_cmp_lt_i32 %[blen], 1\n\t" \
            "s_cbranch_scc1 Lnc_end_%=\n\t" \
            "s_cmp_lg_u32 %[bpos], %[rec]\n\t" \
            "s_cbranch_scc1 Lnc_end_%=\n" \
            "Lnc_snoq_%=:\n\t" \
             \
             \
             \
            "s_sub_i32 %[t1], %[qend], %[CQ64]\n\t" \
            LZ_NC_WHY(3) \
            "s_cmp_gt_i32 %[cls], %[t1]\n\t" \
            "s_cbranch_scc1 Lnc_end_%=\n\t" \
            "s_sub_i32 %[t1], %[rlim], %[C41M]\n\t" \
            "s_lshr_b32 %[t1], %[t1], 1\n\t" \
            "s_add_i32 %[t2], %[rec], %[MSL64]\n\t" \
            "s_cmp_le_i32 %[t2], %[t1]\n\t" \
            "s_cbranch_scc1 Lnc_sok_%=\n\t" \
            "s_add_i32 %[kb], %[t1], %[C2MRD]\n\t"                 \
            "s_cmp_lt_i32 %[rec], %[kb]\n\t" \
            "s_cbranch_scc1 Lnc_end_%=\n\t"                  \
            "s_add_i32 %[kb], %[kb], %[t1]\n\t" \
            "s_cmp_gt_i32 %[t2], %[kb]\n\t" \
            "s_cbranch_scc1 Lnc_end_%=\n" \
            "Lnc_sok_%=:\n\t" \
            "s_add_i32 %[t1], %[rec], %[MSL]\n\t" \
            "s_add_i32 %[t2], %[cls], %[MSL]\n\t" \
            "v_add_u32_e32 %[a0], %[t1], %[lane]\n\t" \
            "v_add_u32_e32 %[a1], %[t2], %[lane]\n\t" \
            "v_lshrrev_b32_e32 %[aq], 4, %[a0]\n\t" \
            "v_lshrrev_b32_e32 %[t], 4, %[a1]\n\t" \
            "v_lshlrev_b32_e32 %[aq], 2, %[aq]\n\t" \
            "v_lshlrev_b32_e32 %[t], 2, %[t]\n\t" \
            "global_load_dword %[aq], %[aq], %[rt2]\n\t" \
            "global_load_dword %[t], %[t], %[qt2]\n\t" \
            "v_and_b32_e32 %[a0], 15, %[a0]\n\t" \
            "v_and_b32_e32 %[a1], 15, %[a1]\n\t" \
            "v_lshlrev_b32_e32 %[a0], 1, %[a0]\n\t" \
            "v_lshlrev_b32_e32 %[a1], 1, %[a1]\n\t" \
            "s_waitcnt vmcnt(0)\n\t" \
            "v_lshrrev_b32_e32 %[aq], %[a0], %[aq]\n\t" \
            "v_lshrrev_b32_e32 %[t], %[a1], %[t]\n\t" \
            "v_xor_b32_e32 %[aq], %[aq], %[t]\n\t" \
            "v_and_b32_e32 %[aq], 3, %[aq]\n\t" \
            "v_cmp_ne_u32_e64 %[m], 0, %[aq]\n\t" \
            "s_nop 0\n\t" \
            LZ_NC_WHY(4) \
            "s_cmp_eq_u64 %[m], 0\n\t" \
            "s_cbranch_scc1 Lnc_end_%=\n\t"                  \
            "s_ff1_i32_b64 %[blen], %[m]\n\t" \
            "s_add_i32 %[blen], %[blen], %[MSL]\n\t" \
            "s_mov_b32 %[ap], %[t0]\n\t" \
            "s_mov_b32 %[bpos], %[rec]\n\t" \
            LZ_NC_WHY(5) \
            "s_mov_b32 %[code], 4\n\t"                       \
             \
             \
             \
             \
             \
             \
            "s_add_i32 %[t1], %[cls], %[blen]\n\t" \
            "s_add_i32 %[t2], %[t1], 64\n\t" \
            "s_sub_i32 %[kb], %[qend], %[C40M]\n\t"               \
            "s_cmp_gt_i32 %[t2], %[kb]\n\t" \
            "s_cbranch_scc1 Lnc_end_%=\n\t" \
            "s_add_i32 %[fok], %[rec], %[blen]\n\t" \
            "s_add_i32 %[t2], %[fok], 64\n\t"                \
            "s_sub_i32 %[kb], %[rlim], %[C41M]\n\t" \
            "s_lshr_b32 %[kb], %[kb], 1\n\t"                 \
            "s_cmp_le_i32 %[t2], %[kb]\n\t" \
            "s_cbranch_scc1 Lnc_hull_%=\n\t" \
            "s_add_i32 %[kc], %[kb], %[C2MRD]\n\t"                 \
            "s_cmp_lt_i32 %[rend], %[kc]\n\t" \
            "s_cbranch_scc1 Lnc_end_%=\n\t" \
            "s_add_i32 %[kc], %[kc], %[kb]\n\t" \
            "s_cmp_gt_i32 %[t2], %[kc]\n\t" \
            "s_cbranch_scc1 Lnc_end_%=\n" \
            "Lnc_hull_%=:\n\t" \
             \
            "s_sub_i32 %[kb], %[fok], %[rend]\n\t" \
            "s_min_i32 %[kb], %[kb], %[t0]\n\t"              \
            "s_sub_i32 %[kc], %[t0], %[kb]\n\t" \
            "s_sub_i32 %[gap], %[fok], %[kb]\n\t"            \
            "s_add_i32 %[kc], %[kc], %[i]\n\t"               \
             \
            "v_add_u32_e32 %[rk0], %[rend], %[lane]\n\t" \
            "v_add_u32_e32 %[rk1], %[i], %[lane]\n\t" \
            "v_add_u32_e32 %[qk], %[gap], %[lane]\n\t" \
            "v_add_u32_e32 %[a0], %[kc], %[lane]\n\t" \
            "v_add_u32_e32 %[a1], %[fok], %[lane]\n\t" \
            "v_add_u32_e32 %[aq], %[t1], %[lane]\n\t" \
            "v_lshrrev_b32_e32 %[rk0], 4, %[rk0]\n\t" \
            "v_lshrrev_b32_e32 %[rk1], 4, %[rk1]\n\t" \
            "v_lshrrev_b32_e32 %[qk], 4, %[qk]\n\t" \
            "v_lshrrev_b32_e32 %[a0], 4, %[a0]\n\t" \
            "v_lshrrev_b32_e32 %[a1], 4, %[a1]\n\t" \
            "v_lshrrev_b32_e32 %[aq], 4, %[aq]\n\t" \
            "v_lshlrev_b32_e32 %[rk0], 2, %[rk0]\n\t" \
            "v_lshlrev_b32_e32 %[rk1], 2, %[rk1]\n\t" \
            "v_lshlrev_b32_e32 %[qk], 2, %[qk]\n\t" \
            "v_lshlrev_b32_e32 %[a0], 2, %[a0]\n\t" \
            "v_lshlrev_b32_e32 %[a1], 2, %[a1]\n\t" \
            "v_lshlrev_b32_e32 %[aq], 2, %[aq]\n\t" \
            "s_nop 0\n\t" \
            "global_load_dword %[rk0], %[rk0], %[rt2]\n\t" \
            "global_load_dword %[rk1], %[rk1], %[qt2]\n\t" \
            "global_load_dword %[qk], %[qk], %[rt2]\n\t" \
            "global_load_dword %[a0], %[a0], %[qt2]\n\t" \
            "global_load_dword %[a1], %[a1], %[rt2]\n\t" \
            "global_load_dword %[aq], %[aq], %[qt2]\n\t" \
            "s_bfm_b64 %[seed], %[kb], 0\n\t"                \
            "s_waitcnt vmcnt(0)\n\t" \
             \
            "v_add_u32_e32 %[t], %[rend], %[lane]\n\t" \
            "v_add_u32_e32 %[bq], %[i], %[lane]\n\t" \
            "v_lshlrev_b32_e32 %[t], 1, %[t]\n\t" \
            "v_lshlrev_b32_e32 %[bq], 1, %[bq]\n\t" \
            "v_and_b32_e32 %[t], 30, %[t]\n\t" \
            "v_and_b32_e32 %[bq], 30, %[bq]\n\t" \
            "v_lshrrev_b32_e32 %[rk0], %[t], %[rk0]\n\t" \
            "v_lshrrev_b32_e32 %[rk1], %[bq], %[rk1]\n\t" \
            "v_xor_b32_e32 %[rk0], %[rk0], %[rk1]\n\t" \
            "v_and_b32_e32 %[rk0], 3, %[rk0]\n\t" \
            "v_cmp_eq_u32_e64 %[m], 0, %[rk0]\n\t" \
             \
            "v_add_u32_e32 %[t], %[gap], %[lane]\n\t" \
            "v_add_u32_e32 %[bq], %[kc], %[lane]\n\t" \
            "v_lshlrev_b32_e32 %[t], 1, %[t]\n\t" \
            "v_lshlrev_b32_e32 %[bq], 1, %[bq]\n\t" \
            "v_and_b32_e32 %[t], 30, %[t]\n\t" \
            "v_and_b32_e32 %[bq], 30, %[bq]\n\t" \
            "v_lshrrev_b32_e32 %[qk], %[t], %[qk]\n\t" \
            "v_lshrrev_b32_e32 %[a0], %[bq], %[a0]\n\t" \
            "v_xor_b32_e32 %[qk], %[qk], %[a0]\n\t" \
            "v_and_b32_e32 %[qk], 3, %[qk]\n\t" \
            "v_cmp_eq_u32_e64 %[m2], 0, %[qk]\n\t" \
             \
            "v_add_u32_e32 %[t], %[fok], %[lane]\n\t" \
            "v_add_u32_e32 %[bq], %[t1], %[lane]\n\t" \
            "v_lshlrev_b32_e32 %[t], 1, %[t]\n\t" \
            "v_lshlrev_b32_e32 %[bq], 1, %[bq]\n\t" \
            "v_and_b32_e32 %[t], 30, %[t]\n\t" \
            "v_and_b32_e32 %[bq], 30, %[bq]\n\t" \
            "v_lshrrev_b32_e32 %[a1], %[t], %[a1]\n\t" \
            "v_lshrrev_b32_e32 %[aq], %[bq], %[aq]\n\t" \
            "v_xor_b32_e32 %[a1], %[a1], %[aq]\n\t" \
            "v_and_b32_e32 %[a1], 3, %[a1]\n\t" \
            "v_cmp_ne_u32_e32 vcc, 0, %[a1]\n\t" \
            "s_and_b64 %[m], %[m], %[seed]\n\t"              \
            "s_and_b64 %[m2], %[m2], %[seed]\n\t"            \
            "s_mov_b64 %[seed], vcc\n\t"                     \
             \
            "s_bcnt1_i32_b64 %[t2], %[m2]\n\t" \
            "s_mov_b64 vcc, %[m]\n\t" \
            "s_nop 0\n\t" \
            "v_mbcnt_lo_u32_b32 %[t], vcc_lo, 0\n\t" \
            "v_mbcnt_hi_u32_b32 %[t], vcc_hi, %[t]\n\t" \
            "s_mov_b64 vcc, %[m2]\n\t" \
            "s_nop 0\n\t" \
            "v_mbcnt_lo_u32_b32 %[bq], vcc_lo, 0\n\t" \
            "v_mbcnt_hi_u32_b32 %[bq], vcc_hi, %[bq]\n\t" \
            "v_add_u32_e32 %[t], %[t2], %[t]\n\t" \
            "v_sub_u32_e32 %[t], %[t], %[bq]\n\t" \
            "v_cmp_ge_u32_e32 vcc, %[kb], %[lane]\n\t" \
            "s_nop 1\n\t" \
            "v_cndmask_b32_e32 %[t], 0, %[t], vcc\n\t"       \
            "s_nop 1\n\t" \
            "v_max_u32_dpp %[t], %[t], %[t] row_shr:1 row_mask:0xf bank_mask:0xf bound_ctrl:0\n\t" \
            "s_nop 1\n\t" \
            "v_max_u32_dpp %[t], %[t], %[t] row_shr:2 row_mask:0xf bank_mask:0xf bound_ctrl:0\n\t" \
            "s_nop 1\n\t" \
            "v_max_u32_dpp %[t], %[t], %[t] row_shr:4 row_mask:0xf bank_mask:0xf bound_ctrl:0\n\t" \
            "s_nop 1\n\t" \
            "v_max_u32_dpp %[t], %[t], %[t] row_shr:8 row_mask:0xf bank_mask:0xf bound_ctrl:0\n\t" \
            "s_nop 1\n\t" \
            "v_max_u32_dpp %[t], %[t], %[t] row_bcast:15 row_mask:0xa bank_mask:0xf\n\t" \
            "s_nop 1\n\t" \
            "v_max_u32_dpp %[t], %[t], %[t] row_bcast:31 row_mask:0xc bank_mask:0xf\n\t" \
            "s_nop 1\n\t" \
            "v_readlane_b32 %[t2], %[t], 63\n\t"             \
             \
             \
             \
            "s_mov_b64 vcc, %[seed]\n\t" \
            "s_lshl_b32 %[gap], vcc_lo, %[AW1]\n\t" \
            "s_lshr_b32 %[kb], vcc_lo, %[AW1C]\n\t" \
            "s_lshl_b32 %[kc], vcc_hi, %[AW1]\n\t" \
            "s_or_b32 %[kc], %[kc], %[kb]\n\t" \
            "s_lshr_b32 %[kb], vcc_hi, %[AW1C]\n\t" \
            "v_mov_b32_e32 %[rk0], %[gap]\n\t" \
            "v_mov_b32_e32 %[rk1], %[kc]\n\t" \
            "v_mov_b32_e32 %[qk], %[kb]\n\t" \
            "v_cmp_gt_u32_e32 vcc, 32, %[lane]\n\t" \
            "v_alignbit_b32 %[a0], %[rk1], %[rk0], %[lane]\n\t" \
            "v_alignbit_b32 %[a1], %[qk], %[rk1], %[lane]\n\t" \
            "v_cndmask_b32_e32 %[a0], %[a1], %[a0], vcc\n\t" \
            "v_and_b32_e32 %[a0], %[AWM], %[a0]\n\t" \
            "v_bcnt_u32_b32 %[a1], %[a0], 0\n\t" \
            "v_and_b32_e32 %[a0], %[ARM], %[a0]\n\t" \
            "v_cmp_lt_u32_e32 vcc, %[AM], %[a1]\n\t"             \
            "v_cmp_eq_u32_e64 %[m], 0, %[a0]\n\t"            \
            "s_nop 0\n\t" \
            "s_cmp_eq_u64 vcc, 0\n\t" \
            "s_cbranch_scc1 Lnc_end_%=\n\t"                  \
            "s_ff1_i32_b64 %[kb], vcc\n\t" \
            "s_cmp_ge_u32 %[kb], 63\n\t" \
            "s_cbranch_scc1 Lnc_end_%=\n\t" \
            "s_add_i32 %[kb], %[kb], 1\n\t" \
            "s_bfm_b64 %[m2], %[kb], 0\n\t" \
            "s_and_b64 %[m], %[m], %[m2]\n\t"                \
            "s_mov_b32 %[kb], 0\n\t"                          \
            "s_mov_b32 %[kc], 0\n\t"                          \
            "s_cbranch_scc0 Lnc_sext_%=\n\t" \
            "s_flbit_i32_b64 %[kb], %[m]\n\t" \
            "s_sub_i32 %[kb], 64, %[kb]\n\t"                 \
            "s_bfm_b64 %[m2], %[kb], 0\n\t" \
            "s_and_b64 %[m2], %[m2], %[seed]\n\t" \
            "s_bcnt1_i32_b64 %[kc], %[m2]\n"                  \
            "Lnc_sext_%=:\n\t" \
             \
            "s_cmp_lg_u32 %[lastb], 0\n\t" \
            "s_cselect_b32 %[gap], %[lastb], %[ocl]\n\t" \
            "s_cselect_b32 %[rec], %[lastlit], %[oclit]\n\t" \
            "s_add_i32 %[gap], %[gap], %[t2]\n\t"            \
            "s_add_i32 %[gap], %[gap], %[blen]\n\t" \
            "s_add_i32 %[gap], %[gap], %[kb]\n\t" \
            "s_sub_i32 %[lastb], %[gap], %[kc]\n\t"          \
            "s_add_i32 %[rec], %[rec], %[t0]\n\t" \
            "s_sub_i32 %[rec], %[rec], %[t2]\n\t" \
            "s_add_i32 %[lastlit], %[rec], %[kc]\n\t"        \
            "s_add_i32 %[i], %[t1], %[kb]\n\t" \
            "s_add_i32 %[rend], %[fok], %[kb]\n\t" \
            "s_mov_b32 %[pre], %[i]\n\t" \
            "s_mov_b32 %[code], 0\n\t" \
            "s_mov_b64 %[m2], -1\n\t" \
            LZ_NC_COUNT \
            "s_branch Lnc_top_%=\n" \
             \
             \
            "Lnc_sfalse_%=:\n\t" \
            "s_bitset0_b64 %[m], %[t0]\n\t" \
            "s_cmp_eq_u64 %[m], 0\n\t" \
            "s_cbranch_scc1 Lnc_snone_%=\n\t" \
            "s_ff1_i32_b64 %[t0], %[m]\n\t" \
            "s_branch Lnc_sdl_%=\n" \
            "Lnc_snone_%=:\n\t" \
            "s_mov_b32 %[code], 0\n\t" \
            "s_mov_b64 %[m2], -1\n\t" \
            "s_bitcmp1_b32 %[cls], 15\n\t" \
            "s_cbranch_scc1 Lnc_fcont_%=\n\t" \
            "s_mov_b64 %[m2], 0\n\t" \
            "s_branch Lnc_top_%=\n" \
            "Lnc_sseed_%=:\n\t"                             \
            "s_cmp_eq_u64 %[m2], 0\n\t" \
            "s_mov_b64 %[m2], -1\n\t" \
            "s_cbranch_scc1 Lnc_noseed_%=\n\t" \
            "s_branch Lnc_fseed_%=\n" \
            "Lnc_kept_%=:\n\t"                               \
            "s_mov_b32 %[cls], 1\n\t"                         \
            "s_mov_b32 %[t1], %[gap]\n\t" \
            "s_branch Lnc_avail_%=\n" \
            "Lnc_close_%=:\n\t"                              \
            "s_add_i32 %[t1], %[rend], %[gap]\n\t" \
            "s_sub_i32 %[t1], %[bpos], %[t1]\n\t" \
            "s_abs_i32 %[t1], %[t1]\n\t" \
            "s_cmp_le_i32 %[t1], %[MRD]\n\t" \
            "s_cbranch_scc1 Lnc_chk_%=\n\t" \
            "s_branch Lnc_distant_%=\n" \
            "Lnc_npl_%=:\n\t" \
            LZ_NC_FIX \
            "Lnc_end_%=:\n\t" \
            "s_waitcnt vmcnt(0) lgkmcnt(0)\n\t" \
            LZ_NC_PRIO_OFF \
            "s_nop 4" \
            : LZ_NC_COUNT_OPERAND [i] "+s"(i), [rend] "+s"(r_end), [qh] "+s"(qh), [prs] "+s"(prev_rs), [pre] "+s"(prev_re), [plit] "+s"(pre_lit), \
              [code] "=&s"(code), [ap] "=&s"(ap), [bpos] "=&s"(bpos), [blen] "=&s"(blen), [lastb] "=&s"(last_cl), [lastlit] "=&s"(last_clit), [rec] "=&s"(rec), \
              [t0] "=&s"(t0), [t1] "=&s"(t1), [t2] "=&s"(t2), [kb] "=&s"(kb), [kc] "=&s"(kc), [m] "=&s"(m), [seed] "=&s"(seed), \
              [gap] "=&s"(gap), [cls] "=&s"(cls), [fok] "=&s"(fok), [atm] "=&s"(add_tm), [atl] "=&s"(add_tl), [atc] "=&s"(add_tc), [m2] "=&s"(m2), \
              [rk0] "=&v"(rk0), [rk1] "=&v"(rk1), [qk] "=&v"(qk), [a0] "=&v"(a0), [a1] "=&v"(a1), [aq] "=&v"(aq), [t] "=&v"(t), [bq] "=&v"(bq), [w1] "=&v"(w1), [dumv] "=&v"(dumv), [qkb] "=&v"(qkb), [rk0b] "=&v"(rk0b), [rk1b] "=&v"(rk1b) \
            : [qc] "s"(qc_u), [ilim] "s"(ilim_u), [rlim] "s"(rlim_u), [qks] "s"(qks), [rks] "s"(rks), [ocl] "s"(ocl_u), [oclit] "s"(oclit_u), \
              [rt2] "s"(rt2), [qt2] "s"(qt2), [qend] "s"(qend), [wdum] "s"((int)SEED_BM_WORDS) SPLIN, \
              [apos] "v"(a_pos), [alen] "v"(a_len), [aref] "v"(a_ref), [aext] "v"(a_ext), [lane] "v"(lane), \
              [ldsb] "v"(ldsb), [zero] "v"(zero), [one] "v"(one), \
              [MQD] "n"(MQD), [MRD] "n"(MRD), [REG] "n"(REG), [AW] "n"(AW), [NT] "n"(NT), [WIN] "s"((int)WIN), [NR1] "n"(WIN - 64), [MSL] "n"(MSL), [MSL64] "n"(MSL + 64), [C41M] "n"(3 * MRD + 1 - WIN - MSL), [C40M] "n"(MRD - MSL), [CQ64] "n"(MRD + 64), [C2MRD] "n"(2 * MRD), \
              [AW1] "n"(AW - 1), [AW1C] "n"(33 - AW), [AWM] "n"((1 << AW) - 1), [ARM] "n"(((1 << AR) - 1) << (AW - AR)), [AM] "n"(AM), [KS5] "n"(2 * MSL + 5), [KS] "n"(2 * MSL) \
            : "vcc", "scc", "memory");
#ifdef LZANI_PHASE_TIME
        const unsigned long long pt_t0 = pt_now();
#endif
        if constexpr (SPLITW) {
            if constexpr (MSL == 9) { LZ_NC_ASM_X(LZ_NC_WORD9, LZ_NC_WORD9, LZ_NC_SPLITCHK, LZ_NC_SPLITGEN, LZ_NC_SPLITIN) }
            else if constexpr (MSL == 8) { LZ_NC_ASM_X(LZ_NC_WORD8, LZ_NC_WORD8, LZ_NC_SPLITCHK, LZ_NC_SPLITGEN, LZ_NC_SPLITIN) }
            else if constexpr (CP::NF) { LZ_NC_ASM_X(LZ_NC_WORD7, LZ_NC_WORD7N, LZ_NC_SPLITCHK, LZ_NC_SPLITGEN, LZ_NC_SPLITIN) }
            else { LZ_NC_ASM_X(LZ_NC_WORD7, LZ_NC_WORD7, LZ_NC_SPLITCHK, LZ_NC_SPLITGEN, LZ_NC_SPLITIN) }
        } else
        if constexpr (MSL == 9) { LZ_NC_ASM(LZ_NC_WORD9, LZ_NC_WORD9) }
        else if constexpr (MSL == 8) { LZ_NC_ASM(LZ_NC_WORD8, LZ_NC_WORD8) }
        else if constexpr (CP::NF) { LZ_NC_ASM(LZ_NC_WORD7, LZ_NC_WORD7N) }
        else { LZ_NC_ASM(LZ_NC_WORD7, LZ_NC_WORD7) }
#ifdef LZANI_PHASE_TIME
        pt_chain += pt_now() - pt_t0;
#endif
        q_head = qh;
        if constexpr (JOIN) {
            if (code == 0 && scan_pos >= i && scan_pos < iend && (qh >= q_cnt || (i > ilim_q && restart_at != i))) refill_only = true;
        }
        pre_round = code == 1;
        if (code == 0) LZ_PS(16); else if (code == 1) LZ_PS(17); else if (code == 2) LZ_PS(18); else LZ_PS(19);
        pre_seed = seed; pre_rk0 = rk0; pre_rk1 = rk1; pre_qk = qk;
        if (code == 2) { adv = ap - i; last_src = q_head++; }
        if (code == 4) { adv = ap; last_src = -1; }
#ifdef LZANI_CHAIN_STATS
        st[0] += 1; st[1] += ncnt; st[2] += code == 0; st[3] += code == 1 && seed != 0; st[4] += code == 1 && seed == 0; st[5] += code == 2;
        if (code == 2) {
            const int g2 = ap - i;
            const bool close = g2 <= MQD && iabs(bpos - (r_end + g2)) <= MRD;
            const bool kept = prev_rs < 0 || prev_re - prev_rs >= REG;
            const bool nofwd = !((u32)rec & EXT_REC_FWDK);
            sr[0] += close; sr[1] += !close && kept; sr[2] += !close && !kept && nofwd; sr[3] += !close && !kept && !nofwd;
        }
        if (code == 1 && seed != 0) {
            sw[0] += why == 1; sw[2] += why == 2; sw[3] += why == 3; sw[4] += why == 4; sw[5] += why == 0;
        }
        if (code == 4) sw[6] += 1;
#endif
        return code;
    }

    static constexpr bool HAS_STRETCH_CHAIN = CHAIN != 0 && (ChainP<CHAIN>::MQD <= ChainP<CHAIN>::MRD) &&
                                              (!JOIN || ChainP<CHAIN>::MAL >= 13 || LZANI_STRETCH_DENSE);
    __device__ __forceinline__ int stretch_chain(int& i, int& r_end, int& cl, int& clit, int& kind, u64& Bf, int& adv, u32& hqa)
    {
        typedef ChainP<CHAIN> CP;
        enum { MQD = CP::MQD, MRD = CP::MRD, MSL = CP::MSL, AW = CP::AW, AM = CP::AM, AR = CP::AR, NT = CP::NT, WIN = CP::WIN };
        const int ilim = SPLITW ? imin(iend - NT, stop_i - (int)SPLIT_MARGIN) : iend - NT, rlim = R.len - MSL + 1 - WIN;
        const u32 ldsb = (u32)(size_t)bitmap;
        const u32 zero = 0, one = 1;
        const u32* const qks = uniform_ptr(qkS);
        const u32* const rks = uniform_ptr(rkS);
        const u32* const qkl = uniform_ptr(qkL);
        const u32* const rt2 = uniform_ptr(reinterpret_cast<const u32*>(R.t2));
        const u32* const qt2 = uniform_ptr(reinterpret_cast<const u32*>(Q.t2));
        const u32* const twp = uniform_ptr(I.tw);
        const u32* const bkp = uniform_ptr(I.bk);
        const int qend = __builtin_amdgcn_readfirstlane((R.nfree && Q.nfree) ? iend : -(1 << 30));
        const int tbits = __builtin_amdgcn_readfirstlane(I.kb - I.dirbits), pbits = __builtin_amdgcn_readfirstlane(I.posbits);
        const u32 tagm = (u32)__builtin_amdgcn_readfirstlane((int)I.tagmask);
        int ncm, t0, t1, t2, kb, kc, gap, rec, cls, fok, blen, anc, aent;
        u64 m, seed, m2, pmk;
        u32 rk0, rk1, qk, hq, a0, a1, aq, t, bq, w1, dumv;
        [[maybe_unused]] u64 cwa, cwb;
        [[maybe_unused]] u32 e0, e1, e2, e3, tagl;
        [[maybe_unused]] const unsigned long long* const cbp = JOIN ? reinterpret_cast<const unsigned long long*>(uniform_ptr(reinterpret_cast<const u32*>(cand_bits))) : nullptr;
#if defined(LZANI_STAMPS) || defined(LZANI_PATH_STATS)
        constexpr bool unify = true;
#else
        constexpr bool unify = SPLITW;
#endif
        int ilim_u = ilim, rlim_u = rlim;
        if constexpr (unify) {
            i = __builtin_amdgcn_readfirstlane(i); r_end = __builtin_amdgcn_readfirstlane(r_end);
            cl = __builtin_amdgcn_readfirstlane(cl); clit = __builtin_amdgcn_readfirstlane(clit);
            ilim_u = __builtin_amdgcn_readfirstlane(ilim); rlim_u = __builtin_amdgcn_readfirstlane(rlim);
        }
#ifdef LZANI_PATH_STATS
        int why = 0;
#define LZ_SC_WHY(n) "s_mov_b32 %[why], " #n "\n\t"
#define LZ_SC_WHY_OPERAND [why] "=&s"(why),
#else
#define LZ_SC_WHY(n)
#define LZ_SC_WHY_OPERAND
#endif
#define LZ_SC_P_CANDLOAD
#define LZ_SC_P_TWADDR \
            "v_lshrrev_b32_e32 %[bq], %[TB], %[hq]\n\t"      \
            "v_cmp_ge_u32_e32 vcc, %[t0], %[lane]\n\t"
#define LZ_SC_P_TWADDR2 \
            "v_lshlrev_b32_e32 %[bq], 2, %[bq]\n\t" \
            "v_cndmask_b32_e32 %[bq], 0, %[bq], vcc\n\t"
#define LZ_SC_P_TWLOAD \
            "s_mov_b64 %[pmk], vcc\n\t" \
            "s_nop 0\n\t" \
            "global_load_dword %[bq], %[bq], %[twp]\n\t"
#define LZ_SC_P_VWAIT "s_waitcnt vmcnt(0)\n\t"
#define LZ_SC_P_TWSWAR \
            "v_and_b32_e32 %[a0], %[TAGM], %[hq]\n\t" \
            "v_or_b32_e32 %[a0], 0x80, %[a0]\n\t" \
            "v_perm_b32 %[a0], %[a0], %[a0], %[zero]\n\t" \
            "v_xor_b32_e32 %[a0], %[a0], %[bq]\n\t"          \
            "v_subrev_u32_e32 %[a1], 0x01010101, %[a0]\n\t" \
            "v_not_b32_e32 %[a0], %[a0]\n\t" \
            "v_and_b32_e32 %[a1], %[a1], %[a0]\n\t" \
            "v_and_b32_e32 %[a1], 0x80808080, %[a1]\n\t"
#define LZ_SC_P_CANDMASK \
            "v_cmp_ne_u32_e32 vcc, 0, %[a1]\n\t" \
            "s_mov_b64 %[m2], vcc\n\t" \
            "v_cmp_eq_u32_e32 vcc, 0x808080ff, %[bq]\n\t"    \
            "s_or_b64 %[m2], %[m2], vcc\n\t" \
            "s_and_b64 %[m2], %[m2], %[pmk]\n\t"
#define LZ_SC_P_ANCENTRY \
             \
            "v_readlane_b32 %[kc], %[a1], %[t0]\n\t"         \
            "v_readlane_b32 %[t1], %[bq], %[t0]\n\t"         \
            "v_readlane_b32 %[t2], %[hq], %[t0]\n\t" \
            "s_cmp_eq_u32 %[t1], 0x808080ff\n\t" \
            LZ_SC_WHY(7) "s_cbranch_scc1 Lsc_end_%=\n\t" \
            "s_sub_u32 %[t1], %[kc], 1\n\t" \
            "s_and_b32 %[t1], %[t1], %[kc]\n\t" \
            "s_cmp_lg_u32 %[t1], 0\n\t" \
            "s_cbranch_scc1 Lsc_end_%=\n\t"                  \
            "s_ff1_i32_b32 %[kc], %[kc]\n\t" \
            "s_lshr_b32 %[kc], %[kc], 3\n\t"                 \
            "s_lshr_b32 %[t2], %[t2], %[TB]\n\t" \
            "s_lshl_b32 %[t2], %[t2], 2\n\t" \
            "s_add_u32 %[t2], %[t2], %[kc]\n\t" \
            "s_lshl_b32 %[t2], %[t2], 2\n\t" \
            "s_load_dword %[aent], %[bkp], %[t2]\n\t" \
            "s_mov_b32 %[anc], 1\n"
#define LZ_SC_P_ANCCHECK \
            "s_bfm_b32 %[anc], %[PB], 0\n\t" \
            "s_and_b32 %[aent], %[aent], %[anc]\n\t" \
            LZ_SC_WHY(8) "s_cmp_lg_u32 %[aent], %[rec]\n\t" \
            "s_cbranch_scc1 Lsc_end_%=\n"
#define LZ_SC_P_XOUT
#define LZ_SC_P_XIN , [twp] "s"(twp)
#define LZ_SC_J_CANDLOAD \
            "s_lshr_b32 %[t1], %[i], 6\n\t" \
            "s_lshl_b32 %[t1], %[t1], 3\n\t" \
            "s_add_u32 %[t2], %[t1], 8\n\t" \
            "s_waitcnt lgkmcnt(0)\n\t" \
            "s_load_dwordx2 %[cwa], %[cbp], %[t1]\n\t" \
            "s_load_dwordx2 %[cwb], %[cbp], %[t2]\n\t"
#define LZ_SC_J_TWADDR
#define LZ_SC_J_TWADDR2
#define LZ_SC_J_TWLOAD
#define LZ_SC_J_VWAIT "s_waitcnt vmcnt(0) lgkmcnt(0)\n\t"
#define LZ_SC_J_TWSWAR
#define LZ_SC_J_CANDMASK \
            "s_and_b32 %[t1], %[i], 63\n\t" \
            "s_lshr_b64 %[m2], %[cwa], %[t1]\n\t" \
            "s_sub_i32 %[t1], 63, %[t1]\n\t" \
            "s_lshl_b64 %[pmk], %[cwb], 1\n\t" \
            "s_lshl_b64 %[pmk], %[pmk], %[t1]\n\t" \
            "s_or_b64 %[m2], %[m2], %[pmk]\n\t"              \
            "s_add_i32 %[t1], %[t0], 1\n\t" \
            "s_bfm_b64 %[pmk], %[t1], 0\n\t" \
            "s_and_b64 %[m2], %[m2], %[pmk]\n\t"
#define LZ_SC_J_ANCENTRY \
            "v_readlane_b32 %[t2], %[hq], %[t0]\n\t" \
            "s_lshr_b32 %[t1], %[t2], %[TB]\n\t" \
            "s_lshl_b32 %[t1], %[t1], 4\n\t" \
            "s_and_b32 %[tagl], %[t2], %[TAGM]\n\t"          \
            "s_load_dword %[e0], %[bkp], %[t1]\n\t" \
            "s_add_u32 %[t2], %[t1], 4\n\t" \
            "s_load_dword %[e1], %[bkp], %[t2]\n\t" \
            "s_add_u32 %[anc], %[t1], 8\n\t" \
            "s_load_dword %[e2], %[bkp], %[anc]\n\t" \
            "s_add_u32 %[aent], %[t1], 12\n\t" \
            "s_load_dword %[e3], %[bkp], %[aent]\n\t" \
            "s_mov_b32 %[anc], 1\n"
#define LZ_SC_J_ANCCHECK \
             \
            "s_cmp_eq_u32 %[e3], 0xfffffffe\n\t" \
            LZ_SC_WHY(7) "s_cbranch_scc1 Lsc_end_%=\n\t" \
            "s_mov_b32 %[anc], 0\n\t" \
            "s_mov_b32 %[aent], 0\n\t" \
            "s_lshr_b32 %[t2], %[e0], %[PB]\n\t" \
            "s_cmp_eq_u32 %[t2], %[tagl]\n\t" \
            "s_cselect_b32 %[aent], %[e0], %[aent]\n\t" \
            "s_addc_u32 %[anc], %[anc], 0\n\t" \
            "s_lshr_b32 %[t2], %[e1], %[PB]\n\t" \
            "s_cmp_eq_u32 %[t2], %[tagl]\n\t" \
            "s_cselect_b32 %[aent], %[e1], %[aent]\n\t" \
            "s_addc_u32 %[anc], %[anc], 0\n\t" \
            "s_lshr_b32 %[t2], %[e2], %[PB]\n\t" \
            "s_cmp_eq_u32 %[t2], %[tagl]\n\t" \
            "s_cselect_b32 %[aent], %[e2], %[aent]\n\t" \
            "s_addc_u32 %[anc], %[anc], 0\n\t" \
            "s_lshr_b32 %[t2], %[e3], %[PB]\n\t" \
            "s_cmp_eq_u32 %[t2], %[tagl]\n\t" \
            "s_cselect_b32 %[aent], %[e3], %[aent]\n\t" \
            "s_addc_u32 %[anc], %[anc], 0\n\t" \
            "s_cmp_lg_u32 %[anc], 1\n\t" \
            "s_cbranch_scc1 Lsc_end_%=\n\t" \
            "s_bfm_b32 %[anc], %[PB], 0\n\t" \
            "s_and_b32 %[aent], %[aent], %[anc]\n\t" \
            LZ_SC_WHY(8) "s_cmp_lg_u32 %[aent], %[rec]\n\t" \
            "s_cbranch_scc1 Lsc_end_%=\n"
#define LZ_SC_J_XOUT , [cwa] "=&s"(cwa), [cwb] "=&s"(cwb), [e0] "=&s"(e0), [e1] "=&s"(e1), [e2] "=&s"(e2), [e3] "=&s"(e3), [tagl] "=&s"(tagl)
#define LZ_SC_J_XIN , [cbp] "s"(cbp)
#define LZ_SC_CAT(F, X) LZ_SC_##F##_##X
#define LZ_SC_ASM(WORD, F) \
        asm volatile( \
            "s_mov_b32 %[ncm], 0\n\t" "s_mov_b32 %[kind], 0\n\t" LZ_SC_WHY(10) \
            "v_add_u32_e32 %[w1], 64, %[lane]\n\t" \
            "v_subrev_u32_e32 %[dumv], %[WIN], %[w1]\n\t" \
            "v_min_u32_e32 %[w1], %[w1], %[dumv]\n\t" \
            "v_add_u32_e32 %[dumv], %[wdum], %[lane]\n\t" \
            "s_nop 3\n" \
            "Lsc_top_%=:\n\t" \
            LZ_SC_WHY(1) "s_cmp_gt_i32 %[i], %[ilim]\n\t" \
            "s_cbranch_scc1 Lsc_end_%=\n\t" \
            LZ_SC_WHY(1) "s_cmp_gt_i32 %[rend], %[rlim]\n\t" \
            "s_cbranch_scc1 Lsc_end_%=\n\t" \
            LZ_NC_LOADS_F \
            "global_load_dword %[hq], %[a0], %[qkl]\n\t"     \
            "s_mov_b32 %[gap], %[NT]\n\t"                    \
            LZ_NC_ROUND_F(WORD) \
            LZ_NC_SEEDS \
            LZ_SC_WHY(2) "s_cbranch_scc0 Lsc_noseed_%=\n\t"               \
            LZ_NC_FIX \
            LZ_SC_WHY(2) "s_cmp_eq_u64 %[m], 0\n\t" \
            "s_cbranch_scc1 Lsc_noseed_%=\n\t" \
            LZ_SC_CAT(F, CANDLOAD) \
            "s_ff1_i32_b64 %[t0], %[m]\n"                    \
            "Lsc_sdl_%=:\n\t" \
            "v_readlane_b32 %[t1], %[qk], %[t0]\n\t"         \
            "s_add_i32 %[t2], %[t0], %[MRD]\n\t"             \
            "s_sub_i32 %[kc], %[t2], 64\n\t" \
            "s_max_i32 %[kc], %[kc], 0\n\t" \
            "s_min_u32 %[kb], %[t2], 64\n\t" \
            "s_sub_i32 %[kb], 64, %[kb]\n\t" \
            "v_cmp_eq_u32_e32 vcc, %[t1], %[rk1]\n\t" \
            "s_bfm_b64 %[m2], %[kc], 0\n\t" \
            "s_and_b64 %[m2], %[m2], vcc\n\t" \
            "v_cmp_eq_u32_e32 vcc, %[t1], %[rk0]\n\t" \
            "s_bcnt1_i32_b64 %[kc], %[m2]\n\t" \
            "s_lshl_b64 vcc, vcc, %[kb]\n\t" \
            "s_bcnt1_i32_b64 %[t1], vcc\n\t" \
            "s_add_i32 %[t2], %[t1], %[kc]\n\t" \
            "s_cmp_eq_u32 %[t2], 0\n\t" \
            "s_cbranch_scc1 Lsc_sfalse_%=\n\t"               \
            "s_cmp_lg_u32 %[t2], 1\n\t" \
            LZ_SC_WHY(3) "s_cbranch_scc1 Lsc_end_%=\n\t"                  \
            "s_ff1_i32_b64 %[t2], vcc\n\t" \
            "s_sub_i32 %[t2], %[t2], %[kb]\n\t" \
            "s_ff1_i32_b64 %[kc], %[m2]\n\t" \
            "s_add_i32 %[kc], %[kc], 64\n\t" \
            "s_cmp_lg_u32 %[t1], 0\n\t" \
            "s_cselect_b32 %[t2], %[t2], %[kc]\n\t"          \
            "s_add_i32 %[rec], %[rend], %[t2]\n\t"           \
            "s_add_i32 %[cls], %[i], %[t0]\n\t"              \
             \
            "s_sub_i32 %[t1], %[qend], %[CQ64]\n\t" \
            LZ_SC_WHY(4) "s_cmp_gt_i32 %[cls], %[t1]\n\t" \
            "s_cbranch_scc1 Lsc_end_%=\n\t" \
            "s_sub_i32 %[t1], %[rlim], %[C41M]\n\t" \
            "s_lshr_b32 %[t1], %[t1], 1\n\t"                 \
            "s_add_i32 %[t2], %[rec], %[MSL64]\n\t" \
            "s_cmp_le_i32 %[t2], %[t1]\n\t" \
            "s_cbranch_scc1 Lsc_sok_%=\n\t" \
            "s_add_i32 %[kb], %[t1], %[C2MRD]\n\t"           \
            "s_cmp_lt_i32 %[rec], %[kb]\n\t" \
            "s_cbranch_scc1 Lsc_end_%=\n\t" \
            "s_add_i32 %[kb], %[kb], %[t1]\n\t" \
            "s_cmp_gt_i32 %[t2], %[kb]\n\t" \
            "s_cbranch_scc1 Lsc_end_%=\n" \
            "Lsc_sok_%=:\n\t" \
             \
            "s_add_i32 %[t1], %[rec], %[MSL]\n\t" \
            "s_add_i32 %[t2], %[cls], %[MSL]\n\t" \
            "v_add_u32_e32 %[a0], %[t1], %[lane]\n\t" \
            "v_add_u32_e32 %[a1], %[t2], %[lane]\n\t" \
            "v_lshrrev_b32_e32 %[aq], 4, %[a0]\n\t" \
            "v_lshrrev_b32_e32 %[t], 4, %[a1]\n\t" \
            LZ_SC_CAT(F, TWADDR) \
            "v_lshlrev_b32_e32 %[aq], 2, %[aq]\n\t" \
            "v_lshlrev_b32_e32 %[t], 2, %[t]\n\t" \
            LZ_SC_CAT(F, TWADDR2) \
            "global_load_dword %[aq], %[aq], %[rt2]\n\t" \
            "global_load_dword %[t], %[t], %[qt2]\n\t" \
            LZ_SC_CAT(F, TWLOAD) \
            "v_and_b32_e32 %[a0], 15, %[a0]\n\t" \
            "v_and_b32_e32 %[a1], 15, %[a1]\n\t" \
            "v_lshlrev_b32_e32 %[a0], 1, %[a0]\n\t" \
            "v_lshlrev_b32_e32 %[a1], 1, %[a1]\n\t" \
            LZ_SC_CAT(F, VWAIT) \
            "v_lshrrev_b32_e32 %[aq], %[a0], %[aq]\n\t" \
            "v_lshrrev_b32_e32 %[t], %[a1], %[t]\n\t" \
            "v_xor_b32_e32 %[aq], %[aq], %[t]\n\t" \
            "v_and_b32_e32 %[aq], 3, %[aq]\n\t" \
            "v_cmp_ne_u32_e64 %[m], 0, %[aq]\n\t" \
            LZ_SC_CAT(F, TWSWAR) \
            "s_cmp_eq_u64 %[m], 0\n\t" \
            LZ_SC_WHY(5) "s_cbranch_scc1 Lsc_end_%=\n\t"                  \
            "s_ff1_i32_b64 %[blen], %[m]\n\t" \
            "s_add_i32 %[blen], %[blen], %[MSL]\n\t" \
            LZ_SC_CAT(F, CANDMASK) \
            "s_bfm_b64 %[seed], %[t0], 0\n\t" \
            "s_and_b64 %[seed], %[seed], %[m2]\n\t" \
            "s_cmp_lg_u64 %[seed], 0\n\t" \
            LZ_SC_WHY(6) "s_cbranch_scc1 Lsc_anchor_%=\n\t"               \
            "s_mov_b32 %[anc], 0\n\t" \
            "s_cmp_eq_u64 %[m2], 0\n\t" \
            "s_cbranch_scc1 Lsc_noanc_%=\n\t" \
            LZ_SC_CAT(F, ANCENTRY) \
            "Lsc_noanc_%=:\n\t" \
             \
            "s_add_i32 %[t1], %[cls], %[blen]\n\t" \
            "s_add_i32 %[t2], %[t1], 64\n\t" \
            "s_sub_i32 %[kb], %[qend], %[C40M]\n\t"          \
            "s_cmp_gt_i32 %[t2], %[kb]\n\t" \
            "s_cbranch_scc1 Lsc_end_%=\n\t" \
            "s_add_i32 %[fok], %[rec], %[blen]\n\t" \
            "s_add_i32 %[t2], %[fok], 64\n\t"                \
            "s_sub_i32 %[kb], %[rlim], %[C41M]\n\t" \
            "s_lshr_b32 %[kb], %[kb], 1\n\t"                 \
            "s_cmp_le_i32 %[t2], %[kb]\n\t" \
            "s_cbranch_scc1 Lsc_hull_%=\n\t" \
            "s_add_i32 %[kc], %[kb], %[C2MRD]\n\t"           \
            "s_cmp_lt_i32 %[rend], %[kc]\n\t" \
            "s_cbranch_scc1 Lsc_end_%=\n\t" \
            "s_add_i32 %[kc], %[kc], %[kb]\n\t" \
            "s_cmp_gt_i32 %[t2], %[kc]\n\t" \
            "s_cbranch_scc1 Lsc_end_%=\n" \
            "Lsc_hull_%=:\n\t" \
            "s_sub_i32 %[kb], %[fok], %[rend]\n\t" \
            "s_min_i32 %[kb], %[kb], %[t0]\n\t"              \
            "s_sub_i32 %[kc], %[t0], %[kb]\n\t" \
            "s_sub_i32 %[gap], %[fok], %[kb]\n\t"            \
            "s_add_i32 %[kc], %[kc], %[i]\n\t"               \
            "v_add_u32_e32 %[rk0], %[rend], %[lane]\n\t" \
            "v_add_u32_e32 %[rk1], %[i], %[lane]\n\t" \
            "v_add_u32_e32 %[qk], %[gap], %[lane]\n\t" \
            "v_add_u32_e32 %[a0], %[kc], %[lane]\n\t" \
            "v_add_u32_e32 %[a1], %[fok], %[lane]\n\t" \
            "v_add_u32_e32 %[aq], %[t1], %[lane]\n\t" \
            "v_lshrrev_b32_e32 %[rk0], 4, %[rk0]\n\t" \
            "v_lshrrev_b32_e32 %[rk1], 4, %[rk1]\n\t" \
            "v_lshrrev_b32_e32 %[qk], 4, %[qk]\n\t" \
            "v_lshrrev_b32_e32 %[a0], 4, %[a0]\n\t" \
            "v_lshrrev_b32_e32 %[a1], 4, %[a1]\n\t" \
            "v_lshrrev_b32_e32 %[aq], 4, %[aq]\n\t" \
            "v_lshlrev_b32_e32 %[rk0], 2, %[rk0]\n\t" \
            "v_lshlrev_b32_e32 %[rk1], 2, %[rk1]\n\t" \
            "v_lshlrev_b32_e32 %[qk], 2, %[qk]\n\t" \
            "v_lshlrev_b32_e32 %[a0], 2, %[a0]\n\t" \
            "v_lshlrev_b32_e32 %[a1], 2, %[a1]\n\t" \
            "v_lshlrev_b32_e32 %[aq], 2, %[aq]\n\t" \
            "s_nop 0\n\t" \
            "global_load_dword %[rk0], %[rk0], %[rt2]\n\t" \
            "global_load_dword %[rk1], %[rk1], %[qt2]\n\t" \
            "global_load_dword %[qk], %[qk], %[rt2]\n\t" \
            "global_load_dword %[a0], %[a0], %[qt2]\n\t" \
            "global_load_dword %[a1], %[a1], %[rt2]\n\t" \
            "global_load_dword %[aq], %[aq], %[qt2]\n\t" \
            "s_bfm_b64 %[seed], %[kb], 0\n\t"                \
            "s_waitcnt vmcnt(0) lgkmcnt(0)\n\t" \
             \
            "s_cmp_eq_u32 %[anc], 0\n\t" \
            "s_cbranch_scc1 Lsc_anok_%=\n\t" \
            LZ_SC_CAT(F, ANCCHECK) \
            "Lsc_anok_%=:\n\t" \
             \
            "v_add_u32_e32 %[t], %[rend], %[lane]\n\t" \
            "v_add_u32_e32 %[bq], %[i], %[lane]\n\t" \
            "v_lshlrev_b32_e32 %[t], 1, %[t]\n\t" \
            "v_lshlrev_b32_e32 %[bq], 1, %[bq]\n\t" \
            "v_and_b32_e32 %[t], 30, %[t]\n\t" \
            "v_and_b32_e32 %[bq], 30, %[bq]\n\t" \
            "v_lshrrev_b32_e32 %[rk0], %[t], %[rk0]\n\t" \
            "v_lshrrev_b32_e32 %[rk1], %[bq], %[rk1]\n\t" \
            "v_xor_b32_e32 %[rk0], %[rk0], %[rk1]\n\t" \
            "v_and_b32_e32 %[rk0], 3, %[rk0]\n\t" \
            "v_cmp_eq_u32_e64 %[m], 0, %[rk0]\n\t" \
             \
            "v_add_u32_e32 %[t], %[gap], %[lane]\n\t" \
            "v_add_u32_e32 %[bq], %[kc], %[lane]\n\t" \
            "v_lshlrev_b32_e32 %[t], 1, %[t]\n\t" \
            "v_lshlrev_b32_e32 %[bq], 1, %[bq]\n\t" \
            "v_and_b32_e32 %[t], 30, %[t]\n\t" \
            "v_and_b32_e32 %[bq], 30, %[bq]\n\t" \
            "v_lshrrev_b32_e32 %[qk], %[t], %[qk]\n\t" \
            "v_lshrrev_b32_e32 %[a0], %[bq], %[a0]\n\t" \
            "v_xor_b32_e32 %[qk], %[qk], %[a0]\n\t" \
            "v_and_b32_e32 %[qk], 3, %[qk]\n\t" \
            "v_cmp_eq_u32_e64 %[m2], 0, %[qk]\n\t" \
             \
            "v_add_u32_e32 %[t], %[fok], %[lane]\n\t" \
            "v_add_u32_e32 %[bq], %[t1], %[lane]\n\t" \
            "v_lshlrev_b32_e32 %[t], 1, %[t]\n\t" \
            "v_lshlrev_b32_e32 %[bq], 1, %[bq]\n\t" \
            "v_and_b32_e32 %[t], 30, %[t]\n\t" \
            "v_and_b32_e32 %[bq], 30, %[bq]\n\t" \
            "v_lshrrev_b32_e32 %[a1], %[t], %[a1]\n\t" \
            "v_lshrrev_b32_e32 %[aq], %[bq], %[aq]\n\t" \
            "v_xor_b32_e32 %[a1], %[a1], %[aq]\n\t" \
            "v_and_b32_e32 %[a1], 3, %[a1]\n\t" \
            "v_cmp_ne_u32_e32 vcc, 0, %[a1]\n\t" \
            "s_and_b64 %[m], %[m], %[seed]\n\t"              \
            "s_and_b64 %[m2], %[m2], %[seed]\n\t"            \
            "s_mov_b64 %[seed], vcc\n\t"                     \
             \
            "s_bcnt1_i32_b64 %[t2], %[m2]\n\t" \
            "s_mov_b64 vcc, %[m]\n\t" \
            "s_nop 0\n\t" \
            "v_mbcnt_lo_u32_b32 %[t], vcc_lo, 0\n\t" \
            "v_mbcnt_hi_u32_b32 %[t], vcc_hi, %[t]\n\t" \
            "s_mov_b64 vcc, %[m2]\n\t" \
            "s_nop 0\n\t" \
            "v_mbcnt_lo_u32_b32 %[bq], vcc_lo, 0\n\t" \
            "v_mbcnt_hi_u32_b32 %[bq], vcc_hi, %[bq]\n\t" \
            "v_add_u32_e32 %[t], %[t2], %[t]\n\t" \
            "v_sub_u32_e32 %[t], %[t], %[bq]\n\t" \
            "v_cmp_ge_u32_e32 vcc, %[kb], %[lane]\n\t" \
            "s_nop 1\n\t" \
            "v_cndmask_b32_e32 %[t], 0, %[t], vcc\n\t" \
            "s_nop 1\n\t" \
            "v_max_u32_dpp %[t], %[t], %[t] row_shr:1 row_mask:0xf bank_mask:0xf bound_ctrl:0\n\t" \
            "s_nop 1\n\t" \
            "v_max_u32_dpp %[t], %[t], %[t] row_shr:2 row_mask:0xf bank_mask:0xf bound_ctrl:0\n\t" \
            "s_nop 1\n\t" \
            "v_max_u32_dpp %[t], %[t], %[t] row_shr:4 row_mask:0xf bank_mask:0xf bound_ctrl:0\n\t" \
            "s_nop 1\n\t" \
            "v_max_u32_dpp %[t], %[t], %[t] row_shr:8 row_mask:0xf bank_mask:0xf bound_ctrl:0\n\t" \
            "s_nop 1\n\t" \
            "v_max_u32_dpp %[t], %[t], %[t] row_bcast:15 row_mask:0xa bank_mask:0xf\n\t" \
            "s_nop 1\n\t" \
            "v_max_u32_dpp %[t], %[t], %[t] row_bcast:31 row_mask:0xc bank_mask:0xf\n\t" \
            "s_nop 1\n\t" \
            "v_readlane_b32 %[t2], %[t], 63\n\t"             \
             \
            "s_mov_b64 vcc, %[seed]\n\t" \
            "s_lshl_b32 %[gap], vcc_lo, %[AW1]\n\t" \
            "s_lshr_b32 %[kb], vcc_lo, %[AW1C]\n\t" \
            "s_lshl_b32 %[kc], vcc_hi, %[AW1]\n\t" \
            "s_or_b32 %[kc], %[kc], %[kb]\n\t" \
            "s_lshr_b32 %[kb], vcc_hi, %[AW1C]\n\t" \
            "v_mov_b32_e32 %[rk0], %[gap]\n\t" \
            "v_mov_b32_e32 %[rk1], %[kc]\n\t" \
            "v_mov_b32_e32 %[qk], %[kb]\n\t" \
            "v_cmp_gt_u32_e32 vcc, 32, %[lane]\n\t" \
            "v_alignbit_b32 %[a0], %[rk1], %[rk0], %[lane]\n\t" \
            "v_alignbit_b32 %[a1], %[qk], %[rk1], %[lane]\n\t" \
            "v_cndmask_b32_e32 %[a0], %[a1], %[a0], vcc\n\t" \
            "v_and_b32_e32 %[a0], %[AWM], %[a0]\n\t" \
            "v_bcnt_u32_b32 %[a1], %[a0], 0\n\t" \
            "v_and_b32_e32 %[a0], %[ARM], %[a0]\n\t" \
            "v_cmp_lt_u32_e32 vcc, %[AM], %[a1]\n\t"             \
            "v_cmp_eq_u32_e64 %[m], 0, %[a0]\n\t"            \
            "s_nop 0\n\t" \
            "s_cmp_eq_u64 vcc, 0\n\t" \
            LZ_SC_WHY(9) "s_cbranch_scc1 Lsc_extgo_%=\n\t"                \
            "s_ff1_i32_b64 %[kb], vcc\n\t" \
            LZ_SC_WHY(9) "s_cmp_ge_u32 %[kb], 63\n\t" \
            "s_cbranch_scc1 Lsc_extgo_%=\n\t" \
            "s_add_i32 %[kb], %[kb], 1\n\t" \
            "s_bfm_b64 %[m2], %[kb], 0\n\t" \
            "s_and_b64 %[m], %[m], %[m2]\n\t"                \
            "s_mov_b32 %[kb], 0\n\t"                          \
            "s_mov_b32 %[kc], 0\n\t"                          \
            "s_cbranch_scc0 Lsc_sext_%=\n\t" \
            "s_flbit_i32_b64 %[kb], %[m]\n\t" \
            "s_sub_i32 %[kb], 64, %[kb]\n\t"                 \
            "s_bfm_b64 %[m2], %[kb], 0\n\t" \
            "s_and_b64 %[m2], %[m2], %[seed]\n\t" \
            "s_bcnt1_i32_b64 %[kc], %[m2]\n"                  \
            "Lsc_sext_%=:\n\t" \
             \
            "s_add_i32 %[cl], %[cl], %[t2]\n\t" \
            "s_add_i32 %[cl], %[cl], %[blen]\n\t" \
            "s_add_i32 %[cl], %[cl], %[kb]\n\t" \
            "s_sub_i32 %[cl], %[cl], %[kc]\n\t" \
            "s_add_i32 %[clit], %[clit], %[t0]\n\t" \
            "s_sub_i32 %[clit], %[clit], %[t2]\n\t" \
            "s_add_i32 %[clit], %[clit], %[kc]\n\t" \
            "s_add_i32 %[i], %[t1], %[kb]\n\t" \
            "s_add_i32 %[rend], %[fok], %[kb]\n\t" \
            "s_add_i32 %[ncm], %[ncm], 1\n\t" \
            "s_branch Lsc_top_%=\n" \
            "Lsc_sfalse_%=:\n\t" \
            LZ_SC_WHY(2) "s_bitset0_b64 %[m], %[t0]\n\t" \
            "s_cmp_eq_u64 %[m], 0\n\t" \
            "s_cbranch_scc1 Lsc_noseed_%=\n\t" \
            "s_ff1_i32_b64 %[t0], %[m]\n\t" \
            "s_branch Lsc_sdl_%=\n" \
            "Lsc_noseed_%=:\n\t" \
            "s_mov_b32 %[kind], 3\n\t" \
            "s_branch Lsc_end_%=\n" \
            "Lsc_anchor_%=:\n\t"                            \
            "s_ff1_i32_b64 %[t0], %[seed]\n\t" \
            "v_readlane_b32 %[t1], %[hq], %[t0]\n\t" \
            "s_mov_b32 %[kind], 2\n\t" \
            "s_branch Lsc_end_%=\n" \
            "Lsc_extgo_%=:\n\t"                             \
            "s_add_i32 %[cl], %[cl], %[t2]\n\t" \
            "s_add_i32 %[cl], %[cl], %[blen]\n\t" \
            "s_add_i32 %[clit], %[clit], %[t0]\n\t" \
            "s_sub_i32 %[clit], %[clit], %[t2]\n\t" \
            "s_mov_b32 %[i], %[t1]\n\t" \
            "s_mov_b32 %[rend], %[fok]\n\t" \
            "s_mov_b32 %[kind], 1\n" \
            "Lsc_end_%=:\n\t" \
            "s_waitcnt vmcnt(0) lgkmcnt(0)\n\t" \
            "s_nop 4" \
            : LZ_SC_WHY_OPERAND [i] "+s"(i), [rend] "+s"(r_end), [cl] "+s"(cl), [clit] "+s"(clit), [ncm] "=&s"(ncm), \
              [t0] "=&s"(t0), [t1] "=&s"(t1), [t2] "=&s"(t2), [kb] "=&s"(kb), [kc] "=&s"(kc), [gap] "=&s"(gap), [rec] "=&s"(rec), [cls] "=&s"(cls), \
              [fok] "=&s"(fok), [blen] "=&s"(blen), [anc] "=&s"(anc), [aent] "=&s"(aent), [kind] "=&s"(kind), [m] "=&s"(m), [seed] "=&s"(seed), [m2] "=&s"(m2), [pmk] "=&s"(pmk), \
              [rk0] "=&v"(rk0), [rk1] "=&v"(rk1), [qk] "=&v"(qk), [hq] "=&v"(hq), [a0] "=&v"(a0), [a1] "=&v"(a1), [aq] "=&v"(aq), [t] "=&v"(t), [bq] "=&v"(bq), \
              [w1] "=&v"(w1), [dumv] "=&v"(dumv) LZ_SC_CAT(F, XOUT) \
            : [ilim] "s"(ilim_u), [rlim] "s"(rlim_u), [qks] "s"(qks), [rks] "s"(rks), [qkl] "s"(qkl), [rt2] "s"(rt2), [qt2] "s"(qt2), [bkp] "s"(bkp), \
              [qend] "s"(qend), [wdum] "s"((int)SEED_BM_WORDS), [TB] "s"(tbits), [PB] "s"(pbits), [TAGM] "s"(tagm) LZ_SC_CAT(F, XIN), \
              [lane] "v"(lane), [ldsb] "v"(ldsb), [zero] "v"(zero), [one] "v"(one), \
              [MRD] "n"(MRD), [NT] "n"(NT), [WIN] "s"((int)WIN), [NR1] "n"(WIN - 64), [MSL] "n"(MSL), [MSL64] "n"(MSL + 64), \
              [C41M] "n"(3 * MRD + 1 - WIN - MSL), [C40M] "n"(MRD - MSL), [CQ64] "n"(MRD + 64), [C2MRD] "n"(2 * MRD), \
              [AW1] "n"(AW - 1), [AW1C] "n"(33 - AW), [AWM] "n"((1 << AW) - 1), [ARM] "n"(((1 << AR) - 1) << (AW - AR)), [AM] "n"(AM), [KS5] "n"(2 * MSL + 5), [KS] "n"(2 * MSL) \
            : "vcc", "scc", "memory");
        if constexpr (JOIN) {
            if constexpr (MSL == 9) { LZ_SC_ASM(LZ_NC_WORD9, J) }
            else if constexpr (MSL == 8) { LZ_SC_ASM(LZ_NC_WORD8, J) }
            else { LZ_SC_ASM(LZ_NC_WORD7, J) }
        } else {
            if constexpr (MSL == 9) { LZ_SC_ASM(LZ_NC_WORD9, P) }
            else if constexpr (MSL == 8) { LZ_SC_ASM(LZ_NC_WORD8, P) }
            else { LZ_SC_ASM(LZ_NC_WORD7, P) }
        }
#undef LZ_SC_ASM
        last_src = -1;
        Bf = seed; adv = t0; hqa = (u32)t1;
        round_no_seed = kind == 3;
        LZ_PSN(23, ncm);
#ifdef LZANI_PATH_STATS
        pw[why < 12 ? why : 0] += 1;
#endif
#undef LZ_SC_WHY
#undef LZ_SC_WHY_OPERAND
        return ncm;
    }
#undef LZ_NC_LOADS_F
#undef LZ_NC_LOADS_X
#undef LZ_NC_ROUND_X
#undef LZ_NC_ROUND_F
#undef LZ_NC_ASM
#undef LZ_NC_ASM_X
#undef LZ_NC_SPLITCHK
#undef LZ_NC_SPLITGEN
#undef LZ_NC_SPLITIN
#undef LZ_NC_WORD7
#undef LZ_NC_WORD7N
#undef LZ_NC_WORD9
#undef LZ_NC_WORD8
#undef LZ_NC_FTURN
#undef LZ_NC_FIX
#undef LZ_NC_SEEDS
#undef LZ_NC_COMMIT

    __device__ __forceinline__ bool find_event(int i, int n, bool trk, int r_end, int lit, int& adv, int& bpos, int& blen)
    {
        if (!FAST || !BK || P.mqd + P.mrd > 128)
            return find_event_round(i, n, trk, r_end, lit, adv, bpos, blen);
        last_src = -1;
        LZ_PS(0);
        const bool no_seed = round_no_seed;
        round_no_seed = false;
        const int nt = trk ? imin(imin(n, P.mqd - lit + 1), 64) : 0;
        if (q_head < q_cnt && __builtin_amdgcn_readlane(a_pos, q_head) < i) drop_before(i);
        const bool only = CHAIN && JOIN && refill_only;
        refill_only = false;
        if (only && q_head < q_cnt) { scan_pos = i; restart_at = i; }
        bool refill_now = only || scan_pos < i + nt;
        bool round_done = !trk;
        u32 rk0 = KM_INVALID, rk1 = KM_INVALID, qk = KM_INVALID;
        u64 seedmask = 0;
        const bool pre = CHAIN && pre_round;
        pre_round = false;
        if (pre) {
            seedmask = pre_seed; rk0 = pre_rk0; rk1 = pre_rk1; qk = pre_qk; round_done = true;
            if (seedmask) {
                const int ls = ctz64(seedmask);
                const int la = q_head < q_cnt ? __builtin_amdgcn_readlane(a_pos, q_head) - i : 64;
                if (ls < la) {
                    u64 d0, d1;
                    seed_candidates((u32)__builtin_amdgcn_readlane((int)qk, ls), lit + ls + P.mrd, rk0, rk1, d0, d1);
                    if (popc64(d0) + popc64(d1) == 1) {
                        const int idx = d0 ? ctz64(d0) : 64 + ctz64(d1);
                        adv = ls; bpos = r_end + idx; blen = wave_equal_len(bpos, i + ls, P.msl);
                        LZ_PS(1);
                        return true;
                    }
                }
            }
        }
        else if (__builtin_expect(!refill_now, 1)) {
            if (trk) { seedmask = track_round(i, nt, r_end, lit, rk0, rk1, qk); round_done = true; }
            if (__builtin_expect((seedmask == 0) & (lit + nt > P.mqd) & (q_head < q_cnt), 1)) {
                const int plen = len_at(q_head);
                if (__builtin_expect(plen > 0, 1)) {
                    adv = __builtin_amdgcn_readlane(a_pos, q_head) - i;
                    bpos = (int)((u32)__builtin_amdgcn_readlane((int)a_ref, q_head)); blen = plen;
                    last_src = q_head++;
                    LZ_PS(2);
                    return true;
                }
            }
        }
        int pos = i, guard = 0;
        bool merge_done = false;
        if (trk & refill_now & !only) {
            const u32 hqv = qkL[(u32)(i + lane)];
            LZ_PS(3);
            seedmask = no_seed ? 0 : track_round(i, nt, r_end, lit, rk0, rk1, qk);
            int known = JOIN ? nt : imin(nt, seedmask ? ctz64(seedmask) + 1 : 8);
            u64 lightmask = detect_steps(i, known);
            for (int it = 0; it < 130; ++it) {
                const int ls = seedmask ? ctz64(seedmask) : 64;
                const int la = lightmask ? ctz64(lightmask) : 64;
                const int l = imin(ls, la);
                if (l >= known && known < nt) { lightmask |= detect_steps(i, nt, known); known = nt; continue; }
                if (l >= 64) break;
                const int qp = i + l;
                int ap = 0, al = 0;
                if (la == l) {
                    lightmask &= lightmask - 1;
                    anchor_by_wave((u32)__builtin_amdgcn_readlane((int)hqv, l), qp, ap, al);
                }
                int sp = 0, sl = 0;
                if (ls == l) {
                    seedmask &= seedmask - 1;
                    const int ref_pred = r_end + lit + l;
                    u64 d0 = 0, d1 = 0;
                    const u32 qkl = (u32)__builtin_amdgcn_readlane((int)qk, l);
                    if (qkl != KM_INVALID) seed_candidates(qkl, lit + l + P.mrd, rk0, rk1, d0, d1);
                    while (d0 | d1) {
                        int idx;
                        if (d0) { idx = ctz64(d0); d0 &= d0 - 1; }
                        else { idx = 64 + ctz64(d1); d1 &= d1 - 1; }
                        seed_consider(r_end + idx, wave_equal_len(r_end + idx, qp, P.msl), ref_pred, sp, sl);
                    }
                }
                arbitrate(P, R.len, lit + l, ap, al, sp, sl);
                if (sl >= P.msl) { adv = l; bpos = sp; blen = sl; LZ_PS(4); return true; }
            }
            LZ_PS(5);
            if (lit + nt <= P.mqd) { adv = nt; return false; }
            pos = i + nt;
            if (q_head < q_cnt) drop_before(pos);
            if (scan_pos < pos) scan_pos = pos;
            refill_now = false;
            round_done = true; merge_done = true;
        }
        for (;;) {
            if (refill_now) {
                if (++guard > (1 << 24)) { LZ_GUARD_TRIP(7); break; }
                refill(pos);
                refill_now = false;
                if (only) { adv = 0; return false; }
            }
            if (!round_done) { seedmask = track_round(i, nt, r_end, lit, rk0, rk1, qk); round_done = true; }
            if (!merge_done) {
                merge_done = true;
                if (seedmask != 0 || (trk && lit + nt <= P.mqd)) {
                    for (int it = 0; it < 130; ++it) {
                        const int ls = seedmask ? ctz64(seedmask) : 64;
                        int la = 64;
                        if (q_head < q_cnt) la = imin(64, __builtin_amdgcn_readlane(a_pos, q_head) - i);
                        if (la >= nt) la = 64;
                        const int l = imin(ls, la);
                        if (l >= 64) break;
                        const int qp = i + l;
                        int ap = 0, al = 0, src = -1;
                        if (la == l) { anchor_of(q_head, qp, ap, al); src = q_head; ++q_head; }
                        int sp = 0, sl = 0;
                        if (ls == l) {
                            seedmask &= seedmask - 1;
                            const int ref_pred = r_end + lit + l;
                            u64 d0 = 0, d1 = 0;
                            const u32 qkl = (u32)__builtin_amdgcn_readlane((int)qk, l);
                            if (qkl != KM_INVALID) seed_candidates(qkl, lit + l + P.mrd, rk0, rk1, d0, d1);
                            while (d0 | d1) {
                                int idx;
                                if (d0) { idx = ctz64(d0); d0 &= d0 - 1; }
                                else { idx = 64 + ctz64(d1); d1 &= d1 - 1; }
                                seed_consider(r_end + idx, wave_equal_len(r_end + idx, qp, P.msl), ref_pred, sp, sl);
                            }
                        }
                        arbitrate(P, R.len, lit + l, ap, al, sp, sl);
                        if (sl >= P.msl) {
                            adv = l; bpos = sp; blen = sl;
                            if (src >= 0) note_src(src, ap, al, sp, sl);
                            LZ_PS(6);
                            return true;
                        }
                    }
                    if (trk && lit + nt <= P.mqd) { adv = nt; return false; }
                    pos = i + nt;
                }
            }
            if (__builtin_expect(q_head >= q_cnt, 0)) {
                if (pos >= i + n || scan_pos >= iend) break;
                refill_now = true;
                continue;
            }
            const int qp = __builtin_amdgcn_readlane(a_pos, q_head);
            const int plen = len_at(q_head);
            if (__builtin_expect(plen > 0, 1)) {
                adv = qp - i; bpos = (int)((u32)__builtin_amdgcn_readlane((int)a_ref, q_head)); blen = plen;
                last_src = q_head++;
                LZ_PS(7);
                return true;
            }
            int ap, al;
            anchor_of(q_head, qp, ap, al);
            ++q_head;
            if (__builtin_expect((al >= P.msl) & ((qp - i >= nt) | (ap != 0)), 1)) {
                adv = qp - i; bpos = ap; blen = al;
                note_src(q_head - 1, ap, al, ap, al);
                return true;
            }
            pos = qp + 1;
        }
        adv = n;
        return false;
    }
    __device__ __forceinline__ ExtMasks ext_scan(u64 prevB, u64 B, int n) const
    {
        bool b, q;
        ext_lane(prevB, B, lane, n, P.aw, P.am, P.ar, b, q);
        ExtMasks m;
        m.brk = wballot(b);
        m.qual = wballot(q);
        return m;
    }
    __device__ __forceinline__ int best_split(u64 Lm, u64 Rm, int to_scan) const
    {
        int key = -1;
        if (lane <= to_scan) key = (popc64(Lm & lowmask(lane)) + popc64(Rm >> lane)) * 128 + lane;
        if (to_scan == 64) key = imax(key, popc64(Lm) * 128 + 64);
        key = imax(key, __builtin_amdgcn_update_dpp(-1, key, 0x111, 0xF, 0xF, false));
        key = imax(key, __builtin_amdgcn_update_dpp(-1, key, 0x112, 0xF, 0xF, false));
        key = imax(key, __builtin_amdgcn_update_dpp(-1, key, 0x114, 0xF, 0xF, false));
        key = imax(key, __builtin_amdgcn_update_dpp(-1, key, 0x118, 0xF, 0xF, false));
        key = imax(key, __builtin_amdgcn_update_dpp(-1, key, 0x142, 0xA, 0xF, false));
        key = imax(key, __builtin_amdgcn_update_dpp(-1, key, 0x143, 0xC, 0xF, false));
        return __builtin_amdgcn_readlane(key, 63) & 127;
    }
};

__device__ __forceinline__ void join_candidates(const u32* __restrict__ tw, int kb, int dirbits, int posbits, u32 tagmask,
                                                const unsigned long long* __restrict__ keys, u32 n_keys,
                                                unsigned long long* __restrict__ cand_bits, int words, int lane)
{
    for (int k = lane; k < words; k += 64) cand_bits[k] = 0;
    const int tb = kb - dirbits;
    const u32 hmask = (u32)lowmask(kb), pmask = (u32)lowmask(posbits);
    u32* const bits32 = reinterpret_cast<u32*>(cand_bits);
    __builtin_amdgcn_fence(__ATOMIC_RELEASE, "agent");
    for (u32 k0 = 0; k0 < n_keys; k0 += 128) {
        unsigned long long e[2];
        u32 w[2];
#pragma unroll
        for (int c = 0; c < 2; ++c) { const u32 k = k0 + 64 * c + lane; e[c] = keys[k < n_keys ? k : n_keys - 1]; }
#pragma unroll
        for (int c = 0; c < 2; ++c) w[c] = tw[(((u32)(e[c] >> posbits)) & hmask) >> tb];
#pragma unroll
        for (int c = 0; c < 2; ++c) {
            const u32 hq = ((u32)(e[c] >> posbits)) & hmask, pos = (u32)e[c] & pmask;
            const u32 x = w[c] ^ rep4(0x80u | (hq & tagmask));
            const u32 z = (x - 0x01010101u) & ~x & 0x80808080u;
            if ((k0 + 64 * c + lane < n_keys) & ((z != 0) | (w[c] == TW_OVERFLOW))) atomicOr(&bits32[pos >> 5], 1u << (pos & 31));
        }
    }
    __builtin_amdgcn_fence(__ATOMIC_ACQ_REL, "agent");
}

struct PairArgs {
    GenomeTab G;
    Params P;
    IndexGeom geo;
    const u32* dirz;
    const u32* ent;
    u64 dir_stride, ent_stride;
    const u32* bk;
    u64 bk_stride;
    const u32* tw;
    u64 tw_stride;
    const u32* fl;
    u64 fl_stride;
    u32 fmask;
    const u32* ref_ids;
    const u64* row_off;
    const u32* query_ids;
    int* out;
    const u32* qorder;
    const u64* qcum;
    u32 qb[NQUEUES + 1];
    unsigned long long* cursor;
    const unsigned long long* skeys;
    const u64* soff;
    const u32* scnt;
    unsigned long long* cbits;
    u64 cbits_stride;
    u64 cb_e0;
    lzani_region* reg_out;
    unsigned long long* reg_count;
    unsigned long long reg_cap;
    const unsigned long long* torder;
};

__device__ __forceinline__ u32 xcc_id()
{
    u32 x;
    asm volatile("s_getreg_b32 %0, hwreg(HW_REG_XCC_ID)" : "=s"(x));
    return x & 7u;
}

template <bool FAST, bool NFREE, int DEFP, bool ALN, bool BK, int CAND, bool LFLT>
__device__ __forceinline__ void pair_body(const PairArgs& a, u32 lo, u32 j, int lane, u32* lds, const u32* flt)
{
    constexpr bool JOIN = CAND != 0;
    const Params Pk = DEFP ? folded_params(DEFP) : a.P;
    const u32 slot = a.qorder[lo];
    const u32 r = a.ref_ids[slot];
    const u64 e = a.row_off[slot] + j;
    const u32 q = a.query_ids ? a.query_ids[e] : j + (j >= r ? 1u : 0u);

    unsigned long long* cand_bits = nullptr;
    if (CAND == 2) cand_bits = a.cbits + (e - a.cb_e0) * a.cbits_stride;
    if (CAND == 1) {
        cand_bits = a.cbits + (u64)(blockIdx.x * 4 + (threadIdx.x >> 6)) * a.cbits_stride;
        join_candidates(a.tw + slot * a.tw_stride, a.geo.kb, a.geo.dirbits, a.geo.posbits, a.geo.tagmask,
                        a.skeys + a.soff[q], a.scnt[q], cand_bits, ((a.G.L[q] + Pk.mrd) >> 6) + 8, lane);
    }
    const int Lr = a.G.L[r], Lq = a.G.L[q];
    const u64 ro = a.G.nmoff[r], qo = a.G.nmoff[q];
    const int T = ref_text_len(Lr, Pk.mrd), D = Lq + Pk.mrd;
    IndexView iv;
    iv.dirz = a.dirz + slot * a.dir_stride;
    iv.ent = a.ent + slot * a.ent_stride;
    iv.kb = a.geo.kb; iv.dirbits = a.geo.dirbits; iv.posbits = a.geo.posbits; iv.tagmask = a.geo.tagmask;
    iv.bk = a.bk ? a.bk + slot * a.bk_stride : nullptr;
    iv.tw = a.tw ? a.tw + slot * a.tw_stride : nullptr;
    const bool nfree = NFREE ? true : !(a.G.hasN[r] | a.G.hasN[q]);
#if defined(LZANI_STAMPS) || defined(LZANI_PATH_STATS)
    constexpr int CHAIN = (FAST && BK && !ALN && !LFLT) ? chain_of(DEFP, NFREE) : 0;
#else
    constexpr int CHAIN = (FAST && BK && !ALN) ? chain_of(DEFP, NFREE) : 0;
#endif
    DevWave<FAST, BK, JOIN, CHAIN, LFLT> w{Pk, ref_view(a.G.t2 + 2 * ro, a.G.nm + ro, Lr, Pk.mrd, nfree),
                    qry_view(a.G.t2 + 2 * qo, a.G.nm + qo, Lq, Pk.mrd, nfree), iv, lane,
                    lds,
                    FAST ? a.G.kmS + 64 * ro : nullptr, FAST ? a.G.kmL + 64 * qo : nullptr,
                    FAST ? a.G.kmS + 64 * qo : nullptr, a.reg_out, a.reg_count, a.reg_cap, e};
    w.iend = D - Pk.msl;
    w.cand_bits = cand_bits;
    w.flt = flt; w.fmask = a.fmask;
    PairMachine<DevWave<FAST, BK, JOIN, CHAIN, LFLT>, ALN> m(w, Pk, T, D);
    int res[3];
#ifdef LZANI_STAMPS
    for (int k = 0; k < 8; ++k) w.acc[k] = 0;
    w.cur = 0;
    asm volatile("s_memtime %0\n\ts_waitcnt lgkmcnt(0)" : "=s"(w.t0) :: "memory");
#endif
#if defined(LZANI_EXP) && LZANI_EXP == 3
    res[0] = res[1] = res[2] = 0;
    if (!JOIN)
#endif
#ifdef LZANI_EXP_REFILLS
    {
        res[0] = res[1] = res[2] = 0;
        if constexpr (JOIN) {
            int guard = 0;
            while (w.scan_pos < w.iend && ++guard < 100000) { w.refill(w.scan_pos); res[0] += w.q_cnt; }
        }
    }
    if (!JOIN)
#endif
#ifdef LZANI_PHASE_TIME
    const unsigned long long pt_p0 = w.pt_now();
#endif
    m.run(res);
#ifdef LZANI_PHASE_TIME
    {
        const unsigned long long pt_all = w.pt_now() - pt_p0;
        atomicAdd(&g_phase_time[0], lane == 0 ? pt_all : 0ULL);
        atomicAdd(&g_phase_time[1], lane == 0 ? w.pt_chain : 0ULL);
        atomicAdd(&g_phase_time[2], lane == 0 ? w.pt_refill : 0ULL);
        atomicAdd(&g_phase_time[3], lane == 0 ? 1ULL : 0ULL);
    }
#endif
#ifdef LZANI_PATH_STATS
    w.flush_path_stats(g_path_stats, lane);
#endif
#ifdef LZANI_CHAIN_STATS
    w.flush_chain_stats(g_chain_stats, lane);
#endif
#ifdef LZANI_STAMPS
    w.stamp(0);
    for (int k = 0; k < 8; ++k) atomicAdd(&g_stamp_acc[k], lane == 0 ? w.acc[k] : 0ULL);
#endif
    int* o = a.out + 3 * e;
    o[0] = res[0]; o[1] = res[1]; o[2] = res[2];
}

__device__ __forceinline__ u32 row_of_ticket(const u64* __restrict__ qcum, u32 rb, u32 re, u64 tk)
{
    u32 lo = rb, hi = re;
    while (hi - lo > 1) {
        u32 mid = (lo + hi) >> 1;
        if (qcum[mid] <= tk) lo = mid; else hi = mid;
    }
    return lo;
}

#ifndef LZANI_WAVES_PER_SIMD
#define LZANI_WAVES_PER_SIMD 8
#endif
template <bool FAST, bool NFREE, int DEFP, bool ALN, bool BK, int CAND>
__device__ __forceinline__ void pairs_loop(const PairArgs& a)
{
    const int lane = threadIdx.x & 63;
    __shared__ u32 s_seed[4][SEED_LDS_WORDS];
    u32* const lds = s_seed[threadIdx.x >> 6];
    for (int k = lane; k < SEED_LDS_WORDS; k += 64) lds[k] = 0;
    u32 qx = xcc_id() % NQUEUES, dry = 0;
    for (;;) {
        unsigned long long t = 0;
        if (lane == 0) t = atomicAdd(&a.cursor[qx], 1ULL);
        const u32 tlo = __builtin_amdgcn_readfirstlane((u32)t);
        const u32 thi = __builtin_amdgcn_readfirstlane((u32)(t >> 32));
        const u32 rb = a.qb[qx], re = a.qb[qx + 1];
        const u64 tk = a.qcum[rb] + (((u64)thi << 32) | tlo);
        if (tk >= a.qcum[re]) {
            if (++dry >= NQUEUES) break;
            qx = (qx + 1) % NQUEUES;
            continue;
        }
        u64 tk2 = tk;
        if (CAND == 2 && a.torder) tk2 = a.qcum[0] + (u32)a.torder[tk - a.qcum[0]];
        const u32 lo = row_of_ticket(a.qcum, rb, re, tk2);
        pair_body<FAST, NFREE, DEFP, ALN, BK, CAND, false>(a, lo, (u32)(tk2 - a.qcum[lo]), lane, lds, nullptr);
    }
}
template <bool FAST, bool NFREE, int DEFP, bool ALN = false, bool BK = false, int CAND = 0>
__global__ void __launch_bounds__(256, LZANI_WAVES_PER_SIMD) k_pairs(PairArgs a)
{
    pairs_loop<FAST, NFREE, DEFP, ALN, BK, CAND>(a);
}

#ifndef LZANI_BLK_CHUNK
#define LZANI_BLK_CHUNK 256
#endif
enum { BLK_WAVES = 16, BLK_CHUNK = LZANI_BLK_CHUNK, BLK_CHUNK_MIN = 32 };
template <bool NFREE, bool DEFP>
__global__ void __launch_bounds__(64 * BLK_WAVES, 8) k_pairs_blk(PairArgs a, u32 fwords, u32 fold, u32* __restrict__ blkctr)
{
    extern __shared__ u32 s_dyn[];
    const int lane = threadIdx.x & 63;
    u32* const lds = s_dyn + (threadIdx.x >> 6) * SEED_LDS_WORDS;
    u32* const flt = s_dyn + BLK_WAVES * SEED_LDS_WORDS;
    u32* const ctl = s_dyn;
    for (int k = lane; k < SEED_LDS_WORDS; k += 64) lds[k] = 0;
    u32 qx = xcc_id() % NQUEUES, dry = 0, have_slot = 0xFFFFFFFFu;
    for (;;) {
        __syncthreads();
        const u32 rb = a.qb[qx], re = a.qb[qx + 1];
        const u64 base = a.qcum[rb], total = a.qcum[re] - base;
        if (threadIdx.x == 0) {
            const unsigned long long seen = __hip_atomic_load(&a.cursor[qx], __ATOMIC_RELAXED, __HIP_MEMORY_SCOPE_AGENT);
            const u64 left = total > seen ? total - seen : 0;
            u64 ch = left / (2 * (gridDim.x / NQUEUES + 1));
            ch = ch < BLK_CHUNK_MIN ? BLK_CHUNK_MIN : ch > BLK_CHUNK ? BLK_CHUNK : ch;
            const unsigned long long t = atomicAdd(&a.cursor[qx], (unsigned long long)ch);
            ctl[0] = (u32)t; ctl[1] = (u32)(t >> 32); ctl[2] = (u32)ch;
        }
        __syncthreads();
        const u64 t0 = ((u64)ctl[1] << 32) | ctl[0];
        const u64 chunk = ctl[2];
        if (t0 >= total) {
            if (++dry >= NQUEUES) break;
            qx = (qx + 1) % NQUEUES;
            continue;
        }
        const u64 t1 = t0 + chunk < total ? t0 + chunk : total;
        u32 lo = row_of_ticket(a.qcum, rb, re, base + t0);
        for (u64 cur = t0; cur < t1; ++lo) {
            const u64 row_end = a.qcum[lo + 1] - base;
            const u64 seg_end = row_end < t1 ? row_end : t1;
            if (seg_end <= cur) continue;
            const u32 slot = a.qorder[lo];
            if (slot != have_slot) {
                const u32* const gf = a.fl + (u64)slot * a.fl_stride;
                for (u32 k = threadIdx.x; k < fwords; k += 64 * BLK_WAVES) {
                    u32 v = gf[k];
                    for (u32 i = 1; i < (1u << fold); ++i) v |= gf[k + i * fwords];
                    flt[k] = v;
                }
                have_slot = slot;
            }
            if (threadIdx.x == 0) { blkctr[blockIdx.x] = 0; __threadfence(); }
            __syncthreads();
            if (threadIdx.x == 0) { ctl[0] = 0; ctl[1] = 0; ctl[2] = 0; }
            const u32 n_seg = (u32)(seg_end - cur);
            const u32 j0 = (u32)(base + cur - a.qcum[lo]);
            for (;;) {
                u32 k = 0;
                if (lane == 0) k = atomicAdd(&blkctr[blockIdx.x], 1u);
                k = __builtin_amdgcn_readfirstlane(k);
                if (k >= n_seg) break;
                pair_body<true, NFREE, DEFP, false, true, 0, true>(a, lo, j0 + k, lane, lds, flt);
            }
            __syncthreads();
            cur = seg_end;
        }
    }
}

}

#if defined(LZANI_RTC)
extern "C" __global__ void __launch_bounds__(256, LZANI_WAVES_PER_SIMD) lzani_rtc_pairs(lzani::PairArgs a)
{
    lzani::pairs_loop<true, (LZANI_RTC_NFREE) != 0, 9, false, true, LZANI_RTC_CAND>(a);
}
#endif
```

Before: 16.73 million.

## Derive query short-kmer seed words from packed 2-bit text instead of kmer array

For N-free chains with short seed length (msl ≤ 7), the query seed word is now extracted from the 2-bit packed query text with a 64-bit load and a funnel shift, instead of being read from the per-position qkS array. The inline-asm null/seed chains gain a form T that loads a dwordx2 from the text, decodes it with v_alignbit and a mask, and applies the N-free head validity check. This aims to cut the query-side kmer-array memory traffic, which is 16x larger than the packed text, at the cost of a few extra ALU ops and pinning v60–v63 as fixed registers. That pinning constrains occupancy assumptions, enforced by a static_assert on waves per SIMD.

Result: faster. 16.98 million (median of 6 runs) (+1.5%).

```diff
diff --git a/lz-ani_amd/csrc/lzani_core.h b/lz-ani_amd/csrc/lzani_core.h
--- a/lz-ani_amd/csrc/lzani_core.h
+++ b/lz-ani_amd/csrc/lzani_core.h
@@ -210,6 +210,15 @@
 LZ_HD bool kmer_valid_nfree_head(int L, int mrd, int p, int k)
 {
     return p + k <= (mrd == 0 ? 2 * L : L);
+}
+LZ_HD constexpr bool kms_is_text(int msl) { return msl >= 1 && msl <= 7; }
+LZ_HD u32 kms_from_syms(u32 syms, int msl)
+{
+    return syms & (u32)lowmask(2 * msl);
+}
+LZ_HD bool kms_valid_nfree_head(int L, int mrd, int p, int msl)
+{
+    return kmer_valid_nfree_head(L, mrd, p, msl);
 }
 LZ_HD void key_slot(const IndexView& I, u64 key, u32& bucket, u32& tag)
 {
diff --git a/lz-ani_amd/csrc/lzani_kernels_index.h b/lz-ani_amd/csrc/lzani_kernels_index.h
--- a/lz-ani_amd/csrc/lzani_kernels_index.h
+++ b/lz-ani_amd/csrc/lzani_kernels_index.h
@@ -15,7 +15,7 @@
     u32 a = KM_INVALID, b = KM_INVALID;
     if (kmer_at(R, p, mal, key)) a = kml_from_syms((u32)key, mal);
     if (kmer_at(R, p, msl, key)) {
-        b = (u32)key;
+        b = kms_from_syms((u32)key, msl);
         if (msl == 8 || msl == 9) {
             u32 h = (b * 0x9E3779B1u) >> 18;
             h = h == 0x3FFFu ? 0x3FFEu : h;
diff --git a/lz-ani_amd/csrc/lzani_kernels_pairs.h b/lz-ani_amd/csrc/lzani_kernels_pairs.h
--- a/lz-ani_amd/csrc/lzani_kernels_pairs.h
+++ b/lz-ani_amd/csrc/lzani_kernels_pairs.h
@@ -38,6 +38,13 @@
            NT = MQD + 1, WIN = MQD + MRD };
 };
 
+#ifdef LZANI_EXP_QCACHED
+#define LZ_QK_AT(i, lane) ((u32)(((i) & 0x3ff) + (lane)))
+#define LZ_QTEXT_OF(CP) false
+#else
+#define LZ_QK_AT(i, lane) ((u32)((i) + (lane)))
+#define LZ_QTEXT_OF(CP) (CP::NF && kms_is_text(CP::MSL))
+#endif
 #ifndef LZANI_STRETCH_DENSE
 #define LZANI_STRETCH_DENSE 0
 #endif
@@ -334,6 +341,21 @@
         }
     }
 
+    static constexpr bool QTEXT_KERNEL = CHAIN != 0 && LZ_QTEXT_OF(ChainP<CHAIN>);
+    __device__ __forceinline__ bool seed_word_from_text() const { return QTEXT_KERNEL; }
+    __device__ __forceinline__ u32 query_seed_word(int i, int ln) const
+    {
+#ifndef LZANI_EXP_QCACHED
+        if (seed_word_from_text()) {
+            const int p = uniform(i) + ln;
+            const u32a* const w = reinterpret_cast<const u32a*>(Q.t2) + ((u32)p >> 4);
+            const u32 syms = funnel32(w[1], w[0], ((u32)p & 15u) * 2u);
+            return kms_valid_nfree_head(Q.L, P.mrd, p, P.msl) ? kms_from_syms(syms, P.msl) : KM_INVALID;
+        }
+#endif
+        return qkS[LZ_QK_AT(i, ln)];
+    }
+
     __device__ __forceinline__ bool find_event_round(int i, int n, bool trk, int r_end, int lit,
                                                      int& ev_lane, int& bpos, int& blen) const
     {
@@ -349,7 +371,7 @@
         hq = lane < n ? hq : KM_INVALID;
         if (W > 0) {
             const int w0 = imin(lane, W - 1), w1 = imin(lane + 64, W - 1);
-            qk = qkS[(u32)(i + lane)];
+            qk = query_seed_word(i, lane);
             rk0 = rkS[(u32)(r_end + w0)];
             rk1 = rkS[(u32)(r_end + w1)];
             qk = lane < nt ? qk : KM_INVALID;
@@ -705,7 +727,7 @@
 #ifdef LZANI_PRIO
         __builtin_amdgcn_s_setprio(LZANI_PRIO);
 #endif
-        qk = qkS[(u32)(i + lane)];
+        qk = query_seed_word(i, lane);
         rk0 = rkS[(u32)(r_end + w0)];
         rk1 = rkS[(u32)(r_end + w1)];
 #ifdef LZANI_PRIO
@@ -739,7 +761,7 @@
         const int rlim = R.len - MSL + 1 - WIN;
         const u32 ldsb = (u32)(size_t)bitmap;
         const u32 zero = 0, one = 1;
-        const u32* const qks = uniform_ptr(qkS);
+        [[maybe_unused]] const u32* const qks = uniform_ptr(qkS);
         const u32* const rks = uniform_ptr(rkS);
         int code, ap, rec, t0, t1, t2, kb, kc, qh = q_head;
         u64 m, seed;
@@ -757,6 +779,15 @@
             qc_u = __builtin_amdgcn_readfirstlane(q_cnt); ilim_u = __builtin_amdgcn_readfirstlane(ilim); rlim_u = __builtin_amdgcn_readfirstlane(rlim);
         }
         u32 rk0, rk1, qk, a0, a1, aq, t, bq, w1, dumv, qkb, rk0b, rk1b;
+        constexpr bool QTEXT = LZ_QTEXT_OF(CP);
+        [[maybe_unused]] register u32 qkT asm("v60"), qkTh asm("v61"), qkbT asm("v62"), qkbTh asm("v63");
+        static_assert(!QTEXT || MRD >= 1, "form T states kms_valid_nfree_head for mrd >= 1 only (chain_params_ok)");
+#define LZ_NC_QOUT_K [qk] "=&v"(qk)
+#define LZ_NC_QOUTB_K [qkb] "=&v"(qkb)
+#define LZ_NC_QOUT_T [qk] "=&v"(qkT), [qkh] "=&v"(qkTh)
+#define LZ_NC_QOUTB_T [qkb] "=&v"(qkbT), [qkbh] "=&v"(qkbTh)
+#define LZ_NC_QIN_K [qks] "s"(qks),
+#define LZ_NC_QIN_T
 #ifdef LZANI_CHAIN_STATS
         int ncnt = 0;
 #define LZ_NC_COUNT "s_add_i32 %[ncnt], %[ncnt], 1\n\t"
@@ -773,14 +804,44 @@
 #else
 #define LZ_NC_NOSEED
 #endif
-#define LZ_NC_LOADS_X(I, R, QK, K0, K1) \
-            "v_add_lshl_u32 %[a0], %[lane], %[" I "], 2\n\t" \
+#ifdef LZANI_EXP_QCACHED
+#define LZ_NC_QCACHED "v_and_b32_e32 %[a0], 0xffc, %[a0]\n\t"
+#else
+#define LZ_NC_QCACHED
+#endif
+#define LZ_NC_CAT(F, X) LZ_NC_##X##_##F
+#define LZ_NC_QKP "v[60:61]"
+#define LZ_NC_QKBP "v[62:63]"
+#define LZ_NC_QADDR_K(I) "v_add_lshl_u32 %[a0], %[lane], %[" I "], 2\n\t" LZ_NC_QCACHED
+#define LZ_NC_QADDR_T(I) \
+            "v_add_u32_e32 %[a0], %[" I "], %[lane]\n\t" \
+            "v_lshrrev_b32_e32 %[a0], 2, %[a0]\n\t" \
+            "v_and_b32_e32 %[a0], -4, %[a0]\n\t"
+#define LZ_NC_QLOAD_K(QK, QP) "global_load_dword %[" QK "], %[a0], %[qks]\n\t"
+#define LZ_NC_QLOAD_T(QK, QP) "global_load_dwordx2 " QP ", %[a0], %[qt2]\n\t"
+#define LZ_NC_LOADS_X(QF, I, R, QK, QP, K0, K1) \
+            LZ_NC_CAT(QF, QADDR)(I) \
             "v_add_lshl_u32 %[a1], %[lane], %[" R "], 2\n\t" \
             "v_add_lshl_u32 %[aq], %[w1], %[" R "], 2\n\t" \
-            "global_load_dword %[" QK "], %[a0], %[qks]\n\t" \
+            LZ_NC_CAT(QF, QLOAD)(QK, QP) \
             "global_load_dword %[" K0 "], %[a1], %[rks]\n\t" \
             "global_load_dword %[" K1 "], %[aq], %[rks]\n\t"
-#define LZ_NC_LOADS_F LZ_NC_LOADS_X("i", "rend", "qk", "rk0", "rk1")
+#define LZ_NC_LOADS_F(QF) LZ_NC_LOADS_X(QF, "i", "rend", "qk", LZ_NC_QKP, "rk0", "rk1")
+#define LZ_NC_QPREF_K(I)
+#define LZ_NC_QDECF_K(I, QK, QH)
+#define LZ_NC_QDECG_K(I, QK, QH)
+#define LZ_NC_QPREF_T(I) "v_add_lshl_u32 %[aq], %[lane], %[" I "], 1\n\t"
+#define LZ_NC_QDECF_T(I, QK, QH) \
+            "v_alignbit_b32 %[" QK "], %[" QH "], %[" QK "], %[aq]\n\t" \
+            "v_and_b32_e32 %[" QK "], %[KMASK], %[" QK "]\n\t"
+#define LZ_NC_QDECG_T(I, QK, QH) \
+            "v_add_u32_e32 %[aq], %[" I "], %[lane]\n\t" \
+            "v_add_u32_e32 %[t], %[MRD], %[aq]\n\t" \
+            "v_lshlrev_b32_e32 %[aq], 1, %[aq]\n\t" \
+            "v_cmp_ge_i32_e32 vcc, %[qend], %[t]\n\t" \
+            "v_alignbit_b32 %[" QK "], %[" QH "], %[" QK "], %[aq]\n\t" \
+            "v_and_b32_e32 %[" QK "], %[KMASK], %[" QK "]\n\t" \
+            "v_cndmask_b32_e32 %[" QK "], -1, %[" QK "], vcc\n\t"
 #define LZ_NC_WORD7(A, T, K) \
             "v_lshrrev_b32_e32 %[" A "], 5, %[" K "]\n\t" \
             "v_lshlrev_b32_e32 %[" T "], %[" K "], %[one]\n\t" \
@@ -800,12 +861,13 @@
             "v_lshrrev_b32_e32 %[" T "], %[KS], %[" K "]\n\t" \
             "v_lshlrev_b32_e32 %[" T "], %[" T "], %[one]\n\t" \
             "v_lshl_add_u32 %[" A "], %[" A "], 2, %[ldsb]\n\t"
-#define LZ_NC_ROUND_X(WORD, WAIT, QK, K0, K1) \
+#define LZ_NC_ROUND_X(QDEC, WORD, WAIT, I, QK, QH, K0, K1) \
             WAIT "\n\t" \
             WORD("a0", "t", K0) \
             "ds_or_b32 %[a0], %[t]\n\t" \
             WORD("a1", "bq", K1) \
             "ds_or_b32 %[a1], %[bq]\n\t" \
+            QDEC(I, QK, QH) \
             WORD("aq", "t", QK) \
             "ds_read_b32 %[aq], %[aq]\n\t" \
             "ds_write_b32 %[a0], %[zero]\n\t" \
@@ -813,8 +875,8 @@
             "s_waitcnt lgkmcnt(2)\n\t" \
             "v_and_b32_e32 %[aq], %[aq], %[t]\n\t" \
             "v_cmp_ne_u32_e64 %[seed], 0, %[aq]\n\t"
-#define LZ_NC_ROUND_F(WORD) LZ_NC_ROUND_X(WORD, "s_waitcnt vmcnt(0)", "qk", "rk0", "rk1")
-#define LZ_NC_FTURN(WORDF, P, N, IC, IN, RN, CQ, C0, C1, NQ, N0, N1, SFX) \
+#define LZ_NC_ROUND_F(QF, WORD) LZ_NC_ROUND_X(LZ_NC_CAT(QF, QDECG), WORD, "s_waitcnt vmcnt(0)", "i", "qk", "qkh", "rk0", "rk1")
+#define LZ_NC_FTURN(QF, WORDF, P, N, IC, IN, RN, CQ, CQH, C0, C1, NQ, NQP, N0, N1, SFX) \
             "Lnc_fturn" SFX "_%=:\n\t" \
             "s_bitcmp0_b32 %[" P "], 15\n\t" \
             "s_cbranch_scc1 Lnc_fnogo" SFX "_%=\n\t" \
@@ -826,8 +888,9 @@
             "s_sub_i32 %[gap], %[ap], %[" IC "]\n\t" \
             "s_add_i32 %[" IN "], %[ap], %[t0]\n\t" \
             "s_add_i32 %[" RN "], %[bpos], %[t0]\n\t" \
-            LZ_NC_LOADS_X(IN, RN, NQ, N0, N1) \
-            LZ_NC_ROUND_X(WORDF, "s_waitcnt vmcnt(3)", CQ, C0, C1) \
+            LZ_NC_LOADS_X(QF, IN, RN, NQ, NQP, N0, N1) \
+            LZ_NC_CAT(QF, QPREF)(IC) \
+            LZ_NC_ROUND_X(LZ_NC_CAT(QF, QDECF), WORDF, "s_waitcnt vmcnt(3)", IC, CQ, CQH, C0, C1) \
             LZ_NC_SEEDS \
             "s_cbranch_scc1 Lnc_frec" SFX "_%=\n\t"          \
             "s_mov_b32 %[t2], %[qh]\n\t" \
@@ -884,8 +947,8 @@
             "s_cmp_lg_u32 %[tnt], 0\n\t" \
             "s_cbranch_scc1 Lnc_chk_%=\n\t"
 #define LZ_NC_SPLITIN , [tnt] "s"(tnt_u)
-#define LZ_NC_ASM(WORD, WORDF) LZ_NC_ASM_X(WORD, WORDF, "", "", )
-#define LZ_NC_ASM_X(WORD, WORDF, SPLCHK, SPLGEN, SPLIN) \
+#define LZ_NC_ASM(QF, WORD, WORDF) LZ_NC_ASM_X(QF, WORD, WORDF, "", "", )
+#define LZ_NC_ASM_X(QF, WORD, WORDF, SPLCHK, SPLGEN, SPLIN) \
         asm volatile( \
             LZ_NC_PRIO_ON \
             "s_mov_b32 %[code], 0\n\t" \
@@ -922,7 +985,7 @@
             "s_cmp_gt_i32 %[rend], %[rlim]\n\t" \
             "s_cbranch_scc1 Lnc_end_%=\n\t" \
             SPLCHK \
-            LZ_NC_LOADS_F \
+            LZ_NC_LOADS_F(QF) \
              \
              \
             "v_readlane_b32 %[blen], %[alen], %[qh]\n\t" \
@@ -986,7 +1049,7 @@
             "Lnc_ok_%=:\n\t" \
             "s_mov_b32 %[t2], 1\n" \
             "Lnc_chk_%=:\n\t" \
-            LZ_NC_ROUND_F(WORD) \
+            LZ_NC_ROUND_F(QF, WORD) \
             "s_mov_b32 %[code], 1\n\t" \
             LZ_NC_SEEDS \
             "s_cbranch_scc1 Lnc_sseed_%=\n"                  \
@@ -1030,14 +1093,14 @@
             "s_sub_i32 %[t2], %[qh], 1\n\t"                 \
             "v_readlane_b32 %[cls], %[alen], %[t2]\n"       \
             "Lnc_fstart_%=:\n\t" \
-            LZ_NC_LOADS_F \
-             \
-             \
-             \
-             \
-             \
-            LZ_NC_FTURN(WORDF, "cls", "blen", "i", "t1", "kb", "qk", "rk0", "rk1", "qkb", "rk0b", "rk1b", "") \
-            LZ_NC_FTURN(WORDF, "blen", "cls", "t1", "i", "rend", "qkb", "rk0b", "rk1b", "qk", "rk0", "rk1", "2") \
+            LZ_NC_LOADS_F(QF) \
+             \
+             \
+             \
+             \
+             \
+            LZ_NC_FTURN(QF, WORDF, "cls", "blen", "i", "t1", "kb", "qk", "qkh", "rk0", "rk1", "qkb", LZ_NC_QKBP, "rk0b", "rk1b", "") \
+            LZ_NC_FTURN(QF, WORDF, "blen", "cls", "t1", "i", "rend", "qkb", "qkbh", "rk0b", "rk1b", "qk", LZ_NC_QKP, "rk0", "rk1", "2") \
             "s_branch Lnc_fturn_%=\n" \
             "Lnc_fnogo2_%=:\n\t" \
             "s_mov_b32 %[i], %[t1]\n\t" \
@@ -1413,27 +1476,29 @@
               [code] "=&s"(code), [ap] "=&s"(ap), [bpos] "=&s"(bpos), [blen] "=&s"(blen), [lastb] "=&s"(last_cl), [lastlit] "=&s"(last_clit), [rec] "=&s"(rec), \
               [t0] "=&s"(t0), [t1] "=&s"(t1), [t2] "=&s"(t2), [kb] "=&s"(kb), [kc] "=&s"(kc), [m] "=&s"(m), [seed] "=&s"(seed), \
               [gap] "=&s"(gap), [cls] "=&s"(cls), [fok] "=&s"(fok), [atm] "=&s"(add_tm), [atl] "=&s"(add_tl), [atc] "=&s"(add_tc), [m2] "=&s"(m2), \
-              [rk0] "=&v"(rk0), [rk1] "=&v"(rk1), [qk] "=&v"(qk), [a0] "=&v"(a0), [a1] "=&v"(a1), [aq] "=&v"(aq), [t] "=&v"(t), [bq] "=&v"(bq), [w1] "=&v"(w1), [dumv] "=&v"(dumv), [qkb] "=&v"(qkb), [rk0b] "=&v"(rk0b), [rk1b] "=&v"(rk1b) \
-            : [qc] "s"(qc_u), [ilim] "s"(ilim_u), [rlim] "s"(rlim_u), [qks] "s"(qks), [rks] "s"(rks), [ocl] "s"(ocl_u), [oclit] "s"(oclit_u), \
+              [rk0] "=&v"(rk0), [rk1] "=&v"(rk1), LZ_NC_CAT(QF, QOUT), [a0] "=&v"(a0), [a1] "=&v"(a1), [aq] "=&v"(aq), [t] "=&v"(t), [bq] "=&v"(bq), [w1] "=&v"(w1), [dumv] "=&v"(dumv), LZ_NC_CAT(QF, QOUTB), [rk0b] "=&v"(rk0b), [rk1b] "=&v"(rk1b) \
+            : [qc] "s"(qc_u), [ilim] "s"(ilim_u), [rlim] "s"(rlim_u), LZ_NC_CAT(QF, QIN) [rks] "s"(rks), [ocl] "s"(ocl_u), [oclit] "s"(oclit_u), \
               [rt2] "s"(rt2), [qt2] "s"(qt2), [qend] "s"(qend), [wdum] "s"((int)SEED_BM_WORDS) SPLIN, \
               [apos] "v"(a_pos), [alen] "v"(a_len), [aref] "v"(a_ref), [aext] "v"(a_ext), [lane] "v"(lane), \
               [ldsb] "v"(ldsb), [zero] "v"(zero), [one] "v"(one), \
               [MQD] "n"(MQD), [MRD] "n"(MRD), [REG] "n"(REG), [AW] "n"(AW), [NT] "n"(NT), [WIN] "s"((int)WIN), [NR1] "n"(WIN - 64), [MSL] "n"(MSL), [MSL64] "n"(MSL + 64), [C41M] "n"(3 * MRD + 1 - WIN - MSL), [C40M] "n"(MRD - MSL), [CQ64] "n"(MRD + 64), [C2MRD] "n"(2 * MRD), \
-              [AW1] "n"(AW - 1), [AW1C] "n"(33 - AW), [AWM] "n"((1 << AW) - 1), [ARM] "n"(((1 << AR) - 1) << (AW - AR)), [AM] "n"(AM), [KS5] "n"(2 * MSL + 5), [KS] "n"(2 * MSL) \
+              [AW1] "n"(AW - 1), [AW1C] "n"(33 - AW), [AWM] "n"((1 << AW) - 1), [ARM] "n"(((1 << AR) - 1) << (AW - AR)), [AM] "n"(AM), [KS5] "n"(2 * MSL + 5), [KS] "n"(2 * MSL), [KMASK] "n"((1 << (2 * (MSL <= 7 ? MSL : 7))) - 1) \
             : "vcc", "scc", "memory");
 #ifdef LZANI_PHASE_TIME
         const unsigned long long pt_t0 = pt_now();
 #endif
         if constexpr (SPLITW) {
-            if constexpr (MSL == 9) { LZ_NC_ASM_X(LZ_NC_WORD9, LZ_NC_WORD9, LZ_NC_SPLITCHK, LZ_NC_SPLITGEN, LZ_NC_SPLITIN) }
-            else if constexpr (MSL == 8) { LZ_NC_ASM_X(LZ_NC_WORD8, LZ_NC_WORD8, LZ_NC_SPLITCHK, LZ_NC_SPLITGEN, LZ_NC_SPLITIN) }
-            else if constexpr (CP::NF) { LZ_NC_ASM_X(LZ_NC_WORD7, LZ_NC_WORD7N, LZ_NC_SPLITCHK, LZ_NC_SPLITGEN, LZ_NC_SPLITIN) }
-            else { LZ_NC_ASM_X(LZ_NC_WORD7, LZ_NC_WORD7, LZ_NC_SPLITCHK, LZ_NC_SPLITGEN, LZ_NC_SPLITIN) }
+            if constexpr (MSL == 9) { LZ_NC_ASM_X(K, LZ_NC_WORD9, LZ_NC_WORD9, LZ_NC_SPLITCHK, LZ_NC_SPLITGEN, LZ_NC_SPLITIN) }
+            else if constexpr (MSL == 8) { LZ_NC_ASM_X(K, LZ_NC_WORD8, LZ_NC_WORD8, LZ_NC_SPLITCHK, LZ_NC_SPLITGEN, LZ_NC_SPLITIN) }
+            else if constexpr (QTEXT) { LZ_NC_ASM_X(T, LZ_NC_WORD7, LZ_NC_WORD7N, LZ_NC_SPLITCHK, LZ_NC_SPLITGEN, LZ_NC_SPLITIN) qk = qkT; }
+            else if constexpr (CP::NF) { LZ_NC_ASM_X(K, LZ_NC_WORD7, LZ_NC_WORD7N, LZ_NC_SPLITCHK, LZ_NC_SPLITGEN, LZ_NC_SPLITIN) }
+            else { LZ_NC_ASM_X(K, LZ_NC_WORD7, LZ_NC_WORD7, LZ_NC_SPLITCHK, LZ_NC_SPLITGEN, LZ_NC_SPLITIN) }
         } else
-        if constexpr (MSL == 9) { LZ_NC_ASM(LZ_NC_WORD9, LZ_NC_WORD9) }
-        else if constexpr (MSL == 8) { LZ_NC_ASM(LZ_NC_WORD8, LZ_NC_WORD8) }
-        else if constexpr (CP::NF) { LZ_NC_ASM(LZ_NC_WORD7, LZ_NC_WORD7N) }
-        else { LZ_NC_ASM(LZ_NC_WORD7, LZ_NC_WORD7) }
+        if constexpr (MSL == 9) { LZ_NC_ASM(K, LZ_NC_WORD9, LZ_NC_WORD9) }
+        else if constexpr (MSL == 8) { LZ_NC_ASM(K, LZ_NC_WORD8, LZ_NC_WORD8) }
+        else if constexpr (QTEXT) { LZ_NC_ASM(T, LZ_NC_WORD7, LZ_NC_WORD7N) qk = qkT; }
+        else if constexpr (CP::NF) { LZ_NC_ASM(K, LZ_NC_WORD7, LZ_NC_WORD7N) }
+        else { LZ_NC_ASM(K, LZ_NC_WORD7, LZ_NC_WORD7) }
 #ifdef LZANI_PHASE_TIME
         pt_chain += pt_now() - pt_t0;
 #endif
@@ -1472,7 +1537,7 @@
         const int ilim = SPLITW ? imin(iend - NT, stop_i - (int)SPLIT_MARGIN) : iend - NT, rlim = R.len - MSL + 1 - WIN;
         const u32 ldsb = (u32)(size_t)bitmap;
         const u32 zero = 0, one = 1;
-        const u32* const qks = uniform_ptr(qkS);
+        [[maybe_unused]] const u32* const qks = uniform_ptr(qkS);
         const u32* const rks = uniform_ptr(rkS);
         const u32* const qkl = uniform_ptr(qkL);
         const u32* const rt2 = uniform_ptr(reinterpret_cast<const u32*>(R.t2));
@@ -1485,6 +1550,9 @@
         int ncm, t0, t1, t2, kb, kc, gap, rec, cls, fok, blen, anc, aent;
         u64 m, seed, m2, pmk;
         u32 rk0, rk1, qk, hq, a0, a1, aq, t, bq, w1, dumv;
+        constexpr bool QTEXT = LZ_QTEXT_OF(CP);
+        [[maybe_unused]] register u32 qkT asm("v60"), qkTh asm("v61");
+        static_assert(!QTEXT || MRD >= 1, "form T states kms_valid_nfree_head for mrd >= 1 only (chain_params_ok)");
         [[maybe_unused]] u64 cwa, cwb;
         [[maybe_unused]] u32 e0, e1, e2, e3, tagl;
         [[maybe_unused]] const unsigned long long* const cbp = JOIN ? reinterpret_cast<const unsigned long long*>(uniform_ptr(reinterpret_cast<const u32*>(cand_bits))) : nullptr;
@@ -1626,7 +1694,13 @@
 #define LZ_SC_J_XOUT , [cwa] "=&s"(cwa), [cwb] "=&s"(cwb), [e0] "=&s"(e0), [e1] "=&s"(e1), [e2] "=&s"(e2), [e3] "=&s"(e3), [tagl] "=&s"(tagl)
 #define LZ_SC_J_XIN , [cbp] "s"(cbp)
 #define LZ_SC_CAT(F, X) LZ_SC_##F##_##X
-#define LZ_SC_ASM(WORD, F) \
+#define LZ_SC_HQLOAD_K "global_load_dword %[hq], %[a0], %[qkl]\n\t"
+#define LZ_SC_HQLOAD_T \
+            "v_add_lshl_u32 %[t], %[lane], %[i], 2\n\t" \
+            "global_load_dword %[hq], %[t], %[qkl]\n\t"
+#define LZ_SC_QOUT_K [qk] "=&v"(qk)
+#define LZ_SC_QOUT_T [qk] "=&v"(qkT), [qkh] "=&v"(qkTh)
+#define LZ_SC_ASM(QF, WORD, F) \
         asm volatile( \
             "s_mov_b32 %[ncm], 0\n\t" "s_mov_b32 %[kind], 0\n\t" LZ_SC_WHY(10) \
             "v_add_u32_e32 %[w1], 64, %[lane]\n\t" \
@@ -1639,10 +1713,10 @@
             "s_cbranch_scc1 Lsc_end_%=\n\t" \
             LZ_SC_WHY(1) "s_cmp_gt_i32 %[rend], %[rlim]\n\t" \
             "s_cbranch_scc1 Lsc_end_%=\n\t" \
-            LZ_NC_LOADS_F \
-            "global_load_dword %[hq], %[a0], %[qkl]\n\t"     \
+            LZ_NC_LOADS_F(QF) \
+            LZ_SC_HQLOAD_##QF \
             "s_mov_b32 %[gap], %[NT]\n\t"                    \
-            LZ_NC_ROUND_F(WORD) \
+            LZ_NC_ROUND_F(QF, WORD) \
             LZ_NC_SEEDS \
             LZ_SC_WHY(2) "s_cbranch_scc0 Lsc_noseed_%=\n\t"               \
             LZ_NC_FIX \
@@ -1933,23 +2007,25 @@
             : LZ_SC_WHY_OPERAND [i] "+s"(i), [rend] "+s"(r_end), [cl] "+s"(cl), [clit] "+s"(clit), [ncm] "=&s"(ncm), \
               [t0] "=&s"(t0), [t1] "=&s"(t1), [t2] "=&s"(t2), [kb] "=&s"(kb), [kc] "=&s"(kc), [gap] "=&s"(gap), [rec] "=&s"(rec), [cls] "=&s"(cls), \
               [fok] "=&s"(fok), [blen] "=&s"(blen), [anc] "=&s"(anc), [aent] "=&s"(aent), [kind] "=&s"(kind), [m] "=&s"(m), [seed] "=&s"(seed), [m2] "=&s"(m2), [pmk] "=&s"(pmk), \
-              [rk0] "=&v"(rk0), [rk1] "=&v"(rk1), [qk] "=&v"(qk), [hq] "=&v"(hq), [a0] "=&v"(a0), [a1] "=&v"(a1), [aq] "=&v"(aq), [t] "=&v"(t), [bq] "=&v"(bq), \
+              [rk0] "=&v"(rk0), [rk1] "=&v"(rk1), LZ_SC_QOUT_##QF, [hq] "=&v"(hq), [a0] "=&v"(a0), [a1] "=&v"(a1), [aq] "=&v"(aq), [t] "=&v"(t), [bq] "=&v"(bq), \
               [w1] "=&v"(w1), [dumv] "=&v"(dumv) LZ_SC_CAT(F, XOUT) \
-            : [ilim] "s"(ilim_u), [rlim] "s"(rlim_u), [qks] "s"(qks), [rks] "s"(rks), [qkl] "s"(qkl), [rt2] "s"(rt2), [qt2] "s"(qt2), [bkp] "s"(bkp), \
+            : [ilim] "s"(ilim_u), [rlim] "s"(rlim_u), LZ_NC_CAT(QF, QIN) [rks] "s"(rks), [qkl] "s"(qkl), [rt2] "s"(rt2), [qt2] "s"(qt2), [bkp] "s"(bkp), \
               [qend] "s"(qend), [wdum] "s"((int)SEED_BM_WORDS), [TB] "s"(tbits), [PB] "s"(pbits), [TAGM] "s"(tagm) LZ_SC_CAT(F, XIN), \
               [lane] "v"(lane), [ldsb] "v"(ldsb), [zero] "v"(zero), [one] "v"(one), \
               [MRD] "n"(MRD), [NT] "n"(NT), [WIN] "s"((int)WIN), [NR1] "n"(WIN - 64), [MSL] "n"(MSL), [MSL64] "n"(MSL + 64), \
               [C41M] "n"(3 * MRD + 1 - WIN - MSL), [C40M] "n"(MRD - MSL), [CQ64] "n"(MRD + 64), [C2MRD] "n"(2 * MRD), \
-              [AW1] "n"(AW - 1), [AW1C] "n"(33 - AW), [AWM] "n"((1 << AW) - 1), [ARM] "n"(((1 << AR) - 1) << (AW - AR)), [AM] "n"(AM), [KS5] "n"(2 * MSL + 5), [KS] "n"(2 * MSL) \
+              [AW1] "n"(AW - 1), [AW1C] "n"(33 - AW), [AWM] "n"((1 << AW) - 1), [ARM] "n"(((1 << AR) - 1) << (AW - AR)), [AM] "n"(AM), [KS5] "n"(2 * MSL + 5), [KS] "n"(2 * MSL), [KMASK] "n"((1 << (2 * (MSL <= 7 ? MSL : 7))) - 1) \
             : "vcc", "scc", "memory");
         if constexpr (JOIN) {
-            if constexpr (MSL == 9) { LZ_SC_ASM(LZ_NC_WORD9, J) }
-            else if constexpr (MSL == 8) { LZ_SC_ASM(LZ_NC_WORD8, J) }
-            else { LZ_SC_ASM(LZ_NC_WORD7, J) }
+            if constexpr (MSL == 9) { LZ_SC_ASM(K, LZ_NC_WORD9, J) }
+            else if constexpr (MSL == 8) { LZ_SC_ASM(K, LZ_NC_WORD8, J) }
+            else if constexpr (QTEXT) { LZ_SC_ASM(T, LZ_NC_WORD7, J) }
+            else { LZ_SC_ASM(K, LZ_NC_WORD7, J) }
         } else {
-            if constexpr (MSL == 9) { LZ_SC_ASM(LZ_NC_WORD9, P) }
-            else if constexpr (MSL == 8) { LZ_SC_ASM(LZ_NC_WORD8, P) }
-            else { LZ_SC_ASM(LZ_NC_WORD7, P) }
+            if constexpr (MSL == 9) { LZ_SC_ASM(K, LZ_NC_WORD9, P) }
+            else if constexpr (MSL == 8) { LZ_SC_ASM(K, LZ_NC_WORD8, P) }
+            else if constexpr (QTEXT) { LZ_SC_ASM(T, LZ_NC_WORD7, P) }
+            else { LZ_SC_ASM(K, LZ_NC_WORD7, P) }
         }
 #undef LZ_SC_ASM
         last_src = -1;
@@ -1965,6 +2041,29 @@
     }
 #undef LZ_NC_LOADS_F
 #undef LZ_NC_LOADS_X
+#undef LZ_NC_CAT
+#undef LZ_NC_QKP
+#undef LZ_NC_QKBP
+#undef LZ_NC_QADDR_K
+#undef LZ_NC_QADDR_T
+#undef LZ_NC_QLOAD_K
+#undef LZ_NC_QLOAD_T
+#undef LZ_NC_QPREF_K
+#undef LZ_NC_QPREF_T
+#undef LZ_NC_QDECF_K
+#undef LZ_NC_QDECG_K
+#undef LZ_NC_QDECF_T
+#undef LZ_NC_QDECG_T
+#undef LZ_NC_QOUT_K
+#undef LZ_NC_QOUT_T
+#undef LZ_NC_QOUTB_K
+#undef LZ_NC_QOUTB_T
+#undef LZ_NC_QIN_K
+#undef LZ_NC_QIN_T
+#undef LZ_SC_HQLOAD_K
+#undef LZ_SC_HQLOAD_T
+#undef LZ_SC_QOUT_K
+#undef LZ_SC_QOUT_T
 #undef LZ_NC_ROUND_X
 #undef LZ_NC_ROUND_F
 #undef LZ_NC_ASM
@@ -2341,6 +2440,7 @@
 #ifndef LZANI_WAVES_PER_SIMD
 #define LZANI_WAVES_PER_SIMD 8
 #endif
+static_assert(LZANI_WAVES_PER_SIMD <= 8, "the null chain names v60 .. v63 (form T of the query words): below 64 VGPRs a wave its register pairs must move");
 template <bool FAST, bool NFREE, int DEFP, bool ALN, bool BK, int CAND>
 __device__ __forceinline__ void pairs_loop(const PairArgs& a)
 {
```
